# Matthew-Mosior/text-compression

Hardware: AMD Instinct MI355X
Metric: BWT+MTF+RLE encode MB/s on 1 GiB ACGTN (higher is better)
Workload: dtype u8; 1 GPU; 1 x 1073741824-byte iid ACGTN record(s) (splitmix64 counter generator), fused BWT->MTF->RLE encode, in/out resident in HBM; record_bytes=1073741824, records=1, parallelism=record-per-gpu x1

## Files before the change

### include/textcomp_debug.h

```cpp
#ifndef TEXTCOMP_DEBUG_H
#define TEXTCOMP_DEBUG_H
#include "textcomp.h"
#ifdef __cplusplus
extern "C" {
#endif
int tc_dbg_checksum64_dev(tc_ctx *ctx, const void *d_p, uint64_t bytes, uint64_t *out);
int tc_dbg_stream_bench(tc_ctx *ctx, uint64_t bytes, int width, int mode, int iters, double *gbps);
int tc_dbg_sort_bench(tc_ctx *ctx, uint64_t n, int key_bits, int iters, int check, double *ms_per_pass);
int tc_dbg_scatter_bench(tc_ctx *ctx, uint64_t n, uint32_t bins, uint32_t xrun, int iters, double *ms_per_pass);
int tc_dbg_dispatch_probe(tc_ctx *ctx, uint32_t grid, uint32_t lds_bytes, uint32_t spin_cycles, uint32_t *out6);
int tc_dbg_lcp_set_short_cap(tc_ctx *ctx, uint32_t cap);
int tc_dbg_msd_split_used(tc_ctx *ctx, uint32_t *used);
#ifdef __cplusplus
}
#endif
#endif
```

### text-compression_amd/csrc/tc_common.hpp

```cpp
#pragma once
#include <hip/hip_runtime.h>
#include <stdint.h>
#include <stdio.h>
#include <string.h>

#include <string>
#include <vector>

#include "textcomp.h"

typedef uint8_t u8;
typedef uint16_t u16;
typedef uint32_t u32;
typedef uint64_t u64;
typedef int16_t i16;
typedef int32_t i32;
typedef int64_t i64;

#define TC_WAVE 64

struct tc_ctx {
    int device = 0;
    hipStream_t stream = nullptr;
    char *ws = nullptr;
    size_t ws_cap = 0;
    size_t ws_off = 0;
    std::vector<hipMemGenericAllocationHandle_t> ws_chunks;
    size_t ws_chunk_bytes = 0, ws_mapped = 0;
    size_t ws_reserved = 0;
    u32 *d_err = nullptr;
    u64 *d_scalars = nullptr;
    u64 *h_scalars = nullptr;
    u8 *h_hdr = nullptr;
    hipEvent_t ev[8] = {};
    hipEvent_t pev[2 * 16] = {};
    int profile = 0;
    int coding = 0;
    int num_cus = 0;
    int reserved_cus = 0;
    void *hostpipe = nullptr;
    u32 stats_ws_grown = 0;
    u32 lcp_cap = 0;
    int msd_split_used = 0;
    int mtf_fastin_failed = 0;
    int live_comms = 0;
    int safe_tickets = 0;
    u32 ticket_fallbacks = 0;
    int pev_used = 0;
    std::string err;
    tc_stats stats = {};
};

struct TcFail {
    int code;
};

#define TC_HIP(ctx, expr)                                                                  \
    do {                                                                                   \
        hipError_t e__ = (expr);                                                           \
        if (e__ != hipSuccess) {                                                           \
            char b__[512];                                                                 \
            snprintf(b__, sizeof b__, "%s:%d: %s -> %s", __FILE__, __LINE__, #expr,        \
                     hipGetErrorString(e__));                                              \
            (ctx)->err = b__;                                                              \
            throw TcFail{e__ == hipErrorOutOfMemory ? TC_ERR_OOM : TC_ERR_HIP};            \
        }                                                                                  \
    } while (0)

#define TC_FAIL(ctx, code_, ...)                         \
    do {                                                 \
        char b__[512];                                   \
        snprintf(b__, sizeof b__, __VA_ARGS__);          \
        (ctx)->err = b__;                                \
        throw TcFail{code_};                             \
    } while (0)

#define TC_LAUNCH_CHECK(ctx) TC_HIP(ctx, hipGetLastError())

struct Arena {
    char *base;
    size_t off = 0;
    explicit Arena(char *b) : base(b) {}
    template <class T>
    T *get(size_t count) {
        size_t bytes = (count * sizeof(T) + 255) & ~size_t(255);
        T *p = base ? reinterpret_cast<T *>(base + off) : nullptr;
        off += bytes;
        return p;
    }
};

void tc_ws_reserve(tc_ctx *ctx, size_t bytes);
template <class F>
static inline void tc_ws_plan(tc_ctx *ctx, size_t base, F &&fn) {
    Arena dry(nullptr);
    fn(dry, true);
    tc_ws_reserve(ctx, base + dry.off);
    Arena A(ctx->ws + base);
    fn(A, false);
}
u32 tc_persistent_grid(tc_ctx *ctx, int blocks_per_cu);
template <class K>
static inline u32 tc_persistent_grid_for(tc_ctx *ctx, K kernel, int threads, int want_per_cu) {
    int occ = 0;
    if (hipOccupancyMaxActiveBlocksPerMultiprocessor(&occ, kernel, threads, 0) != hipSuccess || occ < 1) {
        (void)hipGetLastError();
        occ = 1;
    }
    return tc_persistent_grid(ctx, occ < want_per_cu ? occ : want_per_cu);
}
void *tc_chunked_alloc(tc_ctx *ctx, size_t bytes, int chunk_log2, void **handle);
void tc_chunked_free(void *handle);
void tc_sync_check(tc_ctx *ctx);

static inline u32 tc_cdiv(u64 a, u64 b) { return (u32)((a + b - 1) / b); }

#ifdef __HIPCC__

__device__ __forceinline__ u32 lane_id() { return __lane_id(); }

__device__ __forceinline__ u64 lanemask_lt() {
    return (1ull << lane_id()) - 1ull;
}

__device__ __forceinline__ u32 wave_incl_sum(u32 v) {
#pragma unroll
    for (int d = 1; d < 64; d <<= 1) {
        u32 t = __shfl_up(v, d, 64);
        if ((int)lane_id() >= d) v += t;
    }
    return v;
}
__device__ __forceinline__ u32 wave_incl_max(u32 v) {
#pragma unroll
    for (int d = 1; d < 64; d <<= 1) {
        u32 t = __shfl_up(v, d, 64);
        if ((int)lane_id() >= d) v = v > t ? v : t;
    }
    return v;
}
__device__ __forceinline__ u64 wave_incl_max64(u64 v) {
#pragma unroll
    for (int d = 1; d < 64; d <<= 1) {
        u64 t = __shfl_up(v, d, 64);
        if ((int)lane_id() >= d) v = v > t ? v : t;
    }
    return v;
}
__device__ __forceinline__ u32 wave_sum(u32 v) {
#pragma unroll
    for (int d = 32; d >= 1; d >>= 1) v += __shfl_xor(v, d, 64);
    return v;
}
__device__ __forceinline__ u64 wave_max64(u64 v) {
#pragma unroll
    for (int d = 32; d >= 1; d >>= 1) {
        u64 t = __shfl_xor(v, d, 64);
        v = v > t ? v : t;
    }
    return v;
}

template <int NT>
__device__ __forceinline__ u32 block_excl_sum(u32 v, u32 *smem, u32 *total) {
    const int w = threadIdx.x >> 6;
    u32 inc = wave_incl_sum(v);
    __syncthreads();
    if (lane_id() == 63) smem[w] = inc;
    __syncthreads();
    u32 base = 0, tot = 0;
#pragma unroll
    for (int i = 0; i < NT / 64; i++) {
        u32 s = smem[i];
        if (i < w) base += s;
        tot += s;
    }
    *total = tot;
    return base + inc - v;
}

template <int NT>
__device__ __forceinline__ u64 block_incl_max64(u64 v, u64 *smem, u64 *total) {
    const int w = threadIdx.x >> 6;
    u64 inc = wave_incl_max64(v);
    __syncthreads();
    if (lane_id() == 63) smem[w] = inc;
    __syncthreads();
    u64 base = 0, tot = 0;
#pragma unroll
    for (int i = 0; i < NT / 64; i++) {
        u64 s = smem[i];
        if (i < w) base = base > s ? base : s;
        tot = tot > s ? tot : s;
    }
    *total = tot;
    return inc > base ? inc : base;
}

#define LB_FLAG_AGG (1ull << 62)
#define LB_FLAG_INC (2ull << 62)
#define LB_VALUE(x) ((x) & ((1ull << 62) - 1))
#define LB_SPIN_LIMIT (1u << 24)

__device__ __forceinline__ void lb_store(u64 *p, u64 v) {
    __hip_atomic_store(p, v, __ATOMIC_RELAXED, __HIP_MEMORY_SCOPE_AGENT);
}
__device__ __forceinline__ u64 lb_load(const u64 *p) {
    return __hip_atomic_load(p, __ATOMIC_RELAXED, __HIP_MEMORY_SCOPE_AGENT);
}

struct OpSum {
    __device__ static u64 apply(u64 a, u64 b) { return a + b; }
    __device__ static u64 identity() { return 0; }
};
struct OpMax {
    __device__ static u64 apply(u64 a, u64 b) { return a > b ? a : b; }
    __device__ static u64 identity() { return 0; }
};
struct OpMaxPair {
    __device__ static u64 apply(u64 a, u64 b) {
        u64 ah = a >> 31, bh = b >> 31, al = a & 0x7fffffffull, bl = b & 0x7fffffffull;
        return ((ah > bh ? ah : bh) << 31) | (al > bl ? al : bl);
    }
    __device__ static u64 identity() { return 0; }
};

template <class Op>
__device__ __forceinline__ u64 lb_exclusive(u64 *status, u32 tile, u64 aggregate, u32 *err) {
    if (tile == 0) {
        if (lane_id() == 0) lb_store(&status[0], LB_FLAG_INC | aggregate);
        return Op::identity();
    }
    if (lane_id() == 0) lb_store(&status[tile], LB_FLAG_AGG | aggregate);
    u64 excl = Op::identity();
    i64 look = (i64)tile - 1;
    u32 spins = 0;
    while (true) {
        i64 idx = look - (i64)lane_id();
        u64 s = LB_FLAG_INC;
        if (idx >= 0) s = lb_load(&status[idx]);
        u64 invalid = __ballot((s >> 62) == 0);
        u64 incmask = __ballot((s >> 62) == 2);
        int first_inc = incmask ? __builtin_ctzll(incmask) : 64;
        if (invalid & (first_inc >= 63 ? ~0ull : ((2ull << first_inc) - 1ull))) {
            if (++spins > LB_SPIN_LIMIT) {
                if (lane_id() == 0) atomicOr(err, 1u);
                break;
            }
            __builtin_amdgcn_s_sleep(1);
            continue;
        }
        u64 v = ((int)lane_id() <= first_inc) ? LB_VALUE(s) : Op::identity();
#pragma unroll
        for (int d = 32; d >= 1; d >>= 1) v = Op::apply(v, __shfl_xor(v, d, 64));
        excl = Op::apply(excl, v);
        if (incmask) break;
        look -= 64;
    }
    if (lane_id() == 0) lb_store(&status[tile], LB_FLAG_INC | Op::apply(excl, aggregate));
    return excl;
}

__device__ __forceinline__ u64 lb_exclusive_last(u64 *status, u32 tile, u64 aggregate, u32 *err) {
    if (lane_id() == 0) lb_store(&status[tile], ((tile == 0 || aggregate != 0) ? LB_FLAG_INC : LB_FLAG_AGG) | aggregate);
    if (tile == 0) return 0;
    i64 look = (i64)tile - 1;
    u32 spins = 0;
    while (true) {
        const i64 idx = look - (i64)lane_id();
        u64 s = LB_FLAG_INC;
        if (idx >= 0) s = lb_load(&status[idx]);
        const u64 ends = __ballot((s >> 62) == 2 || ((s >> 62) == 1 && LB_VALUE(s) != 0));
        const u64 invalid = __ballot((s >> 62) == 0);
        const int first_end = ends ? __builtin_ctzll(ends) : 64;
        const u64 nearer = first_end >= 64 ? ~0ull : ((1ull << first_end) - 1ull);
        if (invalid & nearer) {
            if (++spins > LB_SPIN_LIMIT) {
                if (lane_id() == 0) atomicOr(err, 1u);
                return 0;
            }
            __builtin_amdgcn_s_sleep(1);
            continue;
        }
        if (ends) return LB_VALUE(__shfl(s, first_end, 64));
        look -= 64;
    }
}

__device__ __forceinline__ void lds_barrier() { asm volatile("s_waitcnt lgkmcnt(0)\n\ts_barrier" ::: "memory"); }

#endif
```

### text-compression_amd/csrc/tc_msd.hpp

```cpp
#pragma once
#include "tc_sa.hpp"

#ifndef MSD_NT
#define MSD_NT 1024
#endif
#ifndef MSD_ITEMS
#define MSD_ITEMS 8
#endif
#define MSD_TILE (MSD_NT * MSD_ITEMS)
#ifndef MSD_GROUP
#define MSD_GROUP 16
#endif
#define MSD_GLOG (MSD_GROUP == 32 ? 5 : MSD_GROUP == 16 ? 4 : 3)
#ifndef MSD_SUB
#define MSD_SUB 1
#endif
#ifndef MSD_BPC
#define MSD_BPC 1
#endif
#define MSD_LEVELS 3
#define MSDF_CAP_SMALL 2048
#ifndef MSDF_KO_NT
#define MSDF_KO_NT 256
#endif
#ifndef MSDF_BIG_NT
#define MSDF_BIG_NT 512
#endif
#ifndef MSDF_BIG_ITEMS
#define MSDF_BIG_ITEMS 12
#endif
#define MSDF_CAP_BIG (MSDF_BIG_NT * MSDF_BIG_ITEMS)

struct MsdLevel {
    const u32 *pstart;
    const u32 *pcnt;
    const u32 *tpre;
    u32 nparents;
    int shift;
    u32 *seg;
    u32 *cstart;
    u32 *ccnt;
    int aligned;
    u32 ntot;
    const u32 *cnt_in;
    u32 *flags;
    u64 *dbg;
};

#ifdef __HIPCC__

__device__ __forceinline__ u32 msd_tile_lo(u32 T, u32 b, u32 G) { return (u32)(((u64)T * b) / G); }
__device__ __forceinline__ u32 msd_block_of_tile(u32 T, u32 t, u32 G) {
    return (u32)((((u64)t + 1) * G - 1) / T);
}

__global__ void msd_root_kernel(u32 *pstart, u32 *pcnt, u32 N, u32 *maxchild) {
    pstart[0] = 0;
    pcnt[0] = N;
    *maxchild = 0;
}

__device__ __forceinline__ u32 msd_block_of_parent(const MsdLevel &L, u32 q, u32 G) {
    return (u32)(((u64)L.pstart[q] * G) / L.ntot);
}
__device__ __forceinline__ u32 msd_first_parent(const MsdLevel &L, u32 b, u32 G) {
    if (b == 0) return 0;
    if (b >= G) return L.nparents;
    u32 lo = 0, hi = L.nparents;
    while (lo < hi) {
        const u32 mid = (lo + hi) >> 1;
        if (msd_block_of_parent(L, mid, G) >= b) hi = mid; else lo = mid + 1;
    }
    return lo;
}
__device__ __forceinline__ void msd_block_range(const MsdLevel &L, u32 b, u32 G, u32 *t0, u32 *t1) {
    if (L.aligned) {
        *t0 = L.tpre[msd_first_parent(L, b, G)];
        *t1 = L.tpre[msd_first_parent(L, b + 1, G)];
    } else {
        const u32 T = L.tpre[L.nparents];
        *t0 = (u32)(((u64)T * b) / G);
        *t1 = (u32)(((u64)T * (b + 1)) / G);
    }
}

__global__ __launch_bounds__(1024) void msd_prep_kernel(const u32 *__restrict__ pcnt, u32 nparents,
                                                        u32 *__restrict__ tpre) {
    __shared__ u32 s_scan[1024 / 64 + 1];
    const u32 per = (nparents + 1023) / 1024;
    const u32 lo = threadIdx.x * per;
    u32 sum = 0;
    if (per == 64 && nparents == 65536u) {
        uint4 v[16];
        const uint4 *pv = reinterpret_cast<const uint4 *>(pcnt + lo);
#pragma unroll
        for (int i = 0; i < 16; i++) v[i] = pv[i];
        u32 t[64];
#pragma unroll
        for (int i = 0; i < 16; i++) {
            t[4 * i] = (v[i].x + MSD_TILE - 1) / MSD_TILE; t[4 * i + 1] = (v[i].y + MSD_TILE - 1) / MSD_TILE;
            t[4 * i + 2] = (v[i].z + MSD_TILE - 1) / MSD_TILE; t[4 * i + 3] = (v[i].w + MSD_TILE - 1) / MSD_TILE;
        }
#pragma unroll
        for (int i = 0; i < 64; i++) sum += t[i];
        u32 tot;
        u32 run = block_excl_sum<1024>(sum, s_scan, &tot);
        uint4 *ov = reinterpret_cast<uint4 *>(tpre + lo);
#pragma unroll
        for (int i = 0; i < 16; i++) {
            uint4 o;
            o.x = run; run += t[4 * i];
            o.y = run; run += t[4 * i + 1];
            o.z = run; run += t[4 * i + 2];
            o.w = run; run += t[4 * i + 3];
            ov[i] = o;
        }
        if (threadIdx.x == 0) tpre[nparents] = tot;
        return;
    }
    for (u32 i = 0; i < per; i++) {
        const u32 q = lo + i;
        if (q < nparents) sum += (pcnt[q] + MSD_TILE - 1) / MSD_TILE;
    }
    u32 tot;
    u32 run = block_excl_sum<1024>(sum, s_scan, &tot);
    for (u32 i = 0; i < per; i++) {
        const u32 q = lo + i;
        if (q < nparents) {
            tpre[q] = run;
            run += (pcnt[q] + MSD_TILE - 1) / MSD_TILE;
        }
    }
    if (threadIdx.x == 0) tpre[nparents] = tot;
}

__device__ __forceinline__ u32 msd_find_parent(const u32 *tpre, u32 nparents, u32 t) {
    u32 lo = 0, hi = nparents;
    while (hi - lo > 1) {
        const u32 mid = (lo + hi) >> 1;
        if (tpre[mid] <= t) lo = mid; else hi = mid;
    }
    return lo;
}

struct MsdTileInfo {
    u32 base;
    u32 valid;
    u32 q;
    u32 last;
};
struct MsdCur {
    u32 q, tq0, tq1, ps, pc;
};
__device__ __forceinline__ void msd_cur_init(const MsdLevel &L, MsdCur &c, u32 t) {
    c.q = msd_find_parent(L.tpre, L.nparents, t);
    c.tq0 = L.tpre[c.q]; c.tq1 = L.tpre[c.q + 1]; c.ps = L.pstart[c.q]; c.pc = L.pcnt[c.q];
}
__device__ __forceinline__ void msd_cur_info(const MsdLevel &L, MsdCur &c, u32 t, u32 t_end, MsdTileInfo *out) {
    if (t >= t_end) {
        out->base = 0; out->valid = 0; out->q = 0; out->last = 0;
        return;
    }
    if (t >= c.tq1) {
        u32 q = c.q + 1;
        while (L.tpre[q + 1] <= t) q++;
        c.q = q; c.tq0 = L.tpre[q]; c.tq1 = L.tpre[q + 1]; c.ps = L.pstart[q]; c.pc = L.pcnt[q];
    }
    const u32 off = (t - c.tq0) * MSD_TILE;
    out->base = c.ps + off;
    out->valid = c.pc - off < MSD_TILE ? c.pc - off : MSD_TILE;
    out->q = c.q;
    out->last = (t + 1 >= t_end || t + 1 >= c.tq1) ? 1u : 0u;
}

struct MsdTextDigit {
    const u8 *text;
    u32 n;
    u32 B, s;
    u16 lut[256];
    u32 hash_ok, hsh, tlo, thi;
};

#ifndef MSD_XCD_MAP
#define MSD_XCD_MAP 0
#endif
__device__ __forceinline__ u32 msd_logical_wg(u32 b, u32 G) {
    return (MSD_XCD_MAP && (G & 7u) == 0) ? (b & 7u) * (G >> 3) + (b >> 3) : b;
}

struct MsdJointRows {
    u8 row[256];
    u8 dig[128];
};
template <bool TEXT, bool JOINT, bool HI>
__device__ __forceinline__ void msd_count_body(const MsdLevel &L, const u64 *__restrict__ keys,
                                               const MsdTextDigit &td, u32 *__restrict__ joint_out,
                                               const MsdJointRows &jr) {
    static_assert(!HI || (!TEXT && JOINT), "the high halves serve the joint count of keys only");
    __shared__ u32 s_cnt[256];
    __shared__ u16 s_lut[TEXT ? 256 : 1];
    __shared__ u32 s_seg[4];
    __shared__ u32 s_joint[JOINT ? 32768 : 1];
    const u32 tid = threadIdx.x, G = gridDim.x, b = msd_logical_wg(blockIdx.x, G);
    if (tid < 256) s_cnt[tid] = 0;
    if (TEXT && tid < 256) s_lut[tid] = td.lut[tid];
    __shared__ u8 s_row[JOINT ? 256 : 1];
    if (JOINT) {
        for (u32 i = tid; i < 32768; i += MSD_NT) s_joint[i] = 0;
        if (tid < 256) s_row[tid] = jr.row[tid];
    }
    const u32 T = L.tpre[L.nparents];
    const u32 t0 = msd_tile_lo(T, b, G), t1 = msd_tile_lo(T, b + 1, G);
    if (t0 >= t1) return;
    u32 t = t0;
    u32 q = 0;
    if (tid == 0) q = msd_find_parent(L.tpre, L.nparents, t0);
    while (t < t1) {
        if (tid == 0) {
            while (L.tpre[q + 1] <= t) q++;
            const u32 tq0 = L.tpre[q], tq1 = L.tpre[q + 1];
            const u32 te = tq1 < t1 ? tq1 : t1;
            const u32 ps = L.pstart[q], pc = L.pcnt[q];
            const u32 lo = ps + (t - tq0) * MSD_TILE;
            const u64 hi = (u64)ps + (u64)(te - tq0) * MSD_TILE;
            s_seg[0] = q; s_seg[1] = lo; s_seg[2] = hi < (u64)ps + pc ? (u32)hi : ps + pc; s_seg[3] = te;
        }
        __syncthreads();
        const u32 sq = s_seg[0], lo = s_seg[1], hi = s_seg[2];
        t = s_seg[3];
        if (TEXT) {
            const bool words = td.s <= 5 && (u64)lo + 8 < td.n && ((((uintptr_t)td.text) + lo) & 15) == 0;
            u32 p = lo;
            if (words) {
                const u32 span = (u64)hi + 8 <= td.n ? hi - lo : td.n - 8 - lo;
                const u32 nfull = span / (16 * MSD_NT);
                const u32 *tw = reinterpret_cast<const u32 *>(td.text + lo);
                auto fetch = [&](u32 r, u32 *x) {
                    const u32 wi = (r * MSD_NT + tid) * 4;
#pragma unroll
                    for (int q = 0; q < 5; q++) x[q] = tw[wi + q];
                };
                auto tally = [&](const u32 *x) {
                    u32 cd[20];
                    if (td.hash_ok) {
#pragma unroll
                        for (int q = 0; q < 5; q++) {
                            const u32 y = __builtin_amdgcn_perm(td.thi, td.tlo, (x[q] >> td.hsh) & 0x07070707u);
#pragma unroll
                            for (int j = 0; j < 4; j++) cd[4 * q + j] = (y >> (8 * j)) & 255u;
                        }
                    } else {
#pragma unroll
                        for (int j = 0; j < 20; j++) cd[j] = s_lut[(x[j >> 2] >> (8 * (j & 3))) & 255u];
                    }
#pragma unroll
                    for (int k = 0; k < 16; k++) {
                        u32 g = 0;
#pragma unroll
                        for (int j = 0; j < 5; j++)
                            if (j < (int)td.s) g = g * td.B + cd[k + j];
                        atomicAdd(&s_cnt[g], 1u);
                    }
                };
                u32 r = 0;
                for (; r + 4 <= nfull; r += 4) {
                    u32 xa[5], xb[5], xc[5], xd[5];
                    fetch(r, xa); fetch(r + 1, xb); fetch(r + 2, xc); fetch(r + 3, xd);
                    tally(xa); tally(xb); tally(xc); tally(xd);
                }
                for (; r < nfull; r++) {
                    u32 x[5];
                    fetch(r, x);
                    tally(x);
                }
                p = lo + nfull * 16 * MSD_NT;
            }
            for (u64 i0 = (u64)p + tid; i0 < hi; i0 += MSD_NT) {
                u64 i = i0;
                u32 g = 0;
                for (u32 j = 0; j < td.s; j++, i++) g = g * td.B + (i < td.n ? (u32)s_lut[td.text[i]] : 0u);
                atomicAdd(&s_cnt[g], 1u);
            }
        } else {
            auto add_dd = [&](u32 dd) {
                if (JOINT) {
                    const u32 r = s_row[dd >> 8];
                    if (r != 0xffu) atomicAdd(&s_joint[(r << 8) | (dd & 255u)], 1u);
                    else {
                        atomicAdd(&s_cnt[dd >> 8], 1u);
                        atomicAdd(&joint_out[((size_t)sq * 256 + (dd >> 8)) * 256 + (dd & 255u)], 1u);
                    }
                } else {
                    atomicAdd(&s_cnt[dd >> 8], 1u);
                }
            };
            auto add = [&](u64 k) { add_dd((u32)(k >> (L.shift - 8)) & 0xffffu); };
            if (HI) {
                const u32 *khi = reinterpret_cast<const u32 *>(keys);
                const u32 hs = (u32)L.shift - 40u;
                auto add4 = [&](const uint4 v) {
                    add_dd((v.x >> hs) & 0xffffu); add_dd((v.y >> hs) & 0xffffu);
                    add_dd((v.z >> hs) & 0xffffu); add_dd((v.w >> hs) & 0xffffu);
                };
                const u32 a0 = (lo + 3u) & ~3u, a = a0 < hi ? a0 : hi;
                if (lo + tid < a) add_dd((khi[lo + tid] >> hs) & 0xffffu);
                const u32 nq = (hi - a) >> 2;
                const uint4 *q4 = reinterpret_cast<const uint4 *>(khi + a);
                u32 i = tid;
                for (; i + 3 * MSD_NT < nq; i += 4 * MSD_NT) {
                    const uint4 v0 = q4[i], v1 = q4[i + MSD_NT], v2 = q4[i + 2 * MSD_NT], v3 = q4[i + 3 * MSD_NT];
                    add4(v0); add4(v1); add4(v2); add4(v3);
                }
                for (; i < nq; i += MSD_NT) add4(q4[i]);
                const u32 p = a + 4 * nq + tid;
                if (p < hi) add_dd((khi[p] >> hs) & 0xffffu);
            } else {
                u32 p = lo + tid;
                for (; p + 3 * MSD_NT < hi; p += 4 * MSD_NT) {
                    const u64 k0 = keys[p], k1 = keys[p + MSD_NT], k2 = keys[p + 2 * MSD_NT], k3 = keys[p + 3 * MSD_NT];
                    add(k0); add(k1); add(k2); add(k3);
                }
                for (; p < hi; p += MSD_NT) add(keys[p]);
            }
        }
        __syncthreads();
        if (JOINT) {
            for (u32 w = tid; w < 32768; w += MSD_NT) {
                const u32 v = s_joint[w];
                if (v) {
                    atomicAdd(&joint_out[((size_t)sq * 256 + jr.dig[w >> 8]) * 256 + (w & 255u)], v);
                    atomicAdd(&s_cnt[jr.dig[w >> 8]], v);
                    s_joint[w] = 0;
                }
            }
            __syncthreads();
        }
        if (tid < 256) {
            L.seg[((size_t)sq + b) * 256 + tid] = s_cnt[tid];
            s_cnt[tid] = 0;
        }
    }
}
template <bool TEXT, bool JOINT>
__global__ __launch_bounds__(MSD_NT) void msd_count_kernel(MsdLevel L, const u64 *__restrict__ keys,
                                                           MsdTextDigit td, u32 *__restrict__ joint_out,
                                                           MsdJointRows jr) {
    msd_count_body<TEXT, JOINT, false>(L, keys, td, joint_out, jr);
}
__global__ __launch_bounds__(MSD_NT) void msd_count_hi_kernel(MsdLevel L, const u32 *__restrict__ khi,
                                                              MsdTextDigit td, u32 *__restrict__ joint_out,
                                                              MsdJointRows jr) {
    msd_count_body<false, true, true>(L, reinterpret_cast<const u64 *>(khi), td, joint_out, jr);
}

__global__ __launch_bounds__(256) void msd_scan_kernel(MsdLevel L, u32 G, u32 *maxchild) {
    __shared__ u32 s_scan[256 / 64 + 1];
    const u32 q = blockIdx.x, d = threadIdx.x;
    const u32 cnt = L.pcnt[q];
    const size_t c = (size_t)q * 256 + d;
    if (cnt == 0) {
        L.ccnt[c] = 0;
        L.cstart[c] = L.pstart[q];
        return;
    }
    if (L.aligned) {
        const u32 tot = L.cnt_in[c];
        u32 all;
        const u32 excl = block_excl_sum<256>(tot, s_scan, &all);
        const u32 start = L.pstart[q] + excl;
        L.cstart[c] = start;
        L.ccnt[c] = tot;
        L.seg[((size_t)q + msd_block_of_parent(L, q, G)) * 256 + d] = start;
        if (d == 0 && all != cnt) atomicOr(L.flags, 8u);
        if (maxchild) {
            u32 m = tot;
#pragma unroll
            for (int x = 32; x >= 1; x >>= 1) {
                const u32 o = __shfl_xor(m, x, 64);
                m = m > o ? m : o;
            }
            if ((d & 63) == 0 && m > MSDF_CAP_SMALL) atomicMax(maxchild, m);
        }
        return;
    }
    const u32 T = L.tpre[L.nparents];
    const u32 bf = msd_block_of_tile(T, L.tpre[q], G), bl = msd_block_of_tile(T, L.tpre[q + 1] - 1, G);
    u32 tot = 0;
#pragma unroll 8
    for (u32 b = bf; b <= bl; b++) {
        const u32 v = L.seg[((size_t)q + b) * 256 + d];
        tot += msd_tile_lo(T, b, G) < msd_tile_lo(T, b + 1, G) ? v : 0u;
    }
    u32 all;
    const u32 excl = block_excl_sum<256>(tot, s_scan, &all);
    u32 run = L.pstart[q] + excl;
    L.cstart[c] = run;
    L.ccnt[c] = tot;
#pragma unroll 8
    for (u32 b = bf; b <= bl; b++) {
        const size_t o = ((size_t)q + b) * 256 + d;
        const u32 v = L.seg[o];
        if (msd_tile_lo(T, b, G) >= msd_tile_lo(T, b + 1, G)) continue;
        L.seg[o] = run;
        run += v;
    }
    if (maxchild) {
        u32 m = tot;
#pragma unroll
        for (int x = 32; x >= 1; x >>= 1) {
            const u32 o = __shfl_xor(m, x, 64);
            m = m > o ? m : o;
        }
        if ((d & 63) == 0 && m > MSDF_CAP_SMALL) atomicMax(maxchild, m);
    }
}

typedef u32 msd_u32x4 __attribute__((ext_vector_type(4)));
template <bool KEYGEN, bool VALS, bool SPLIT>
__device__ __forceinline__ void msd_partition_body(const MsdLevel &L, const u64 *kin, const u32 *vin,
                                                   u64 *kout, u32 *vout, u32 *shi, u32 *slo, const u8 *text,
                                                   const RadixKeyGen &kg) {
    static_assert(!SPLIT || !VALS, "the split layout is the key-only levels'");
    __shared__ __attribute__((aligned(16))) u64 s_keys[MSD_TILE];
    __shared__ __attribute__((aligned(16))) u32 s_vals[VALS ? MSD_TILE : 4];
    __shared__ __attribute__((aligned(16))) u64 c_keys[256 * MSD_GROUP];
    __shared__ __attribute__((aligned(16))) u32 c_vals[VALS ? 256 * MSD_GROUP : 4];
    __shared__ u32 s_cnt[256 * MSD_SUB], s_dstart[256 * MSD_SUB], s_r[256], s_cur[256], s_ph[256];
    __shared__ u32 s_scan[16];
    __shared__ u64 s_lmask[4];
#ifdef MSD_PROFILE
    __shared__ u64 s_dbg[2];
    if (threadIdx.x == 0) { s_dbg[0] = 0; s_dbg[1] = 0; }
#endif
    __shared__ u16 s_live[256];
    __shared__ u16 s_klut[KEYGEN ? 256 : 1];
    constexpr bool KG_SPLIT = KEYGEN && !VALS && MSD_ITEMS == 8;
    __shared__ __attribute__((aligned(16))) u8 s_kr[KG_SPLIT ? MSD_TILE + 16 + 80 + 32 : 16];
    __shared__ __attribute__((aligned(16))) u8 s_kg8[KG_SPLIT ? MSD_TILE + 64 : 16];
    __shared__ u32 s_scan2[2];
    static_assert(MSD_GROUP == 8 || MSD_GROUP == 16 || MSD_GROUP == 32, "group = 8, 16 or 32 pairs");
    static_assert(((size_t)MSD_TILE * (VALS ? 12 : 8) + 256 * MSD_GROUP * (VALS ? 12 : 8) + 8192 + (KG_SPLIT ? 2 * MSD_TILE + 256 : 0)) * (VALS ? 1 : MSD_BPC) <= 163840, "LDS budget");
    __shared__ MsdTileInfo s_info[4];

    const u32 tid = threadIdx.x, G = gridDim.x, b = msd_logical_wg(blockIdx.x, G);
    if (KEYGEN && tid < 256) s_klut[tid] = kg.lut[tid];
    if (tid < 256) { s_r[tid] = 0; s_ph[tid] = 0; s_cur[tid] = 0; }
    for (u32 i = tid; i < 256 * MSD_SUB; i += MSD_NT) s_cnt[i] = 0;
    if (tid == 0) {
        u32 ta = 0, tb = 0;
        if (!(L.aligned && (*L.flags & 8u))) msd_block_range(L, b, G, &ta, &tb);
        s_scan2[0] = ta; s_scan2[1] = tb;
    }
    __syncthreads();
    const u32 t0 = s_scan2[0], t1 = s_scan2[1];
    if (t0 >= t1) return;
    MsdCur cs = {};
    if (tid == 0) {
        msd_cur_init(L, cs, t0);
        msd_cur_info(L, cs, t0, t1, &s_info[0]);
        msd_cur_info(L, cs, t0 + 1, t1, &s_info[1]);
        msd_cur_info(L, cs, t0 + 2, t1, &s_info[2]);
    }
    __syncthreads();

    constexpr int KG_PRE = 16, KG_SLOTS = MSD_TILE + KG_PRE + 80;
    u16 *k_c = reinterpret_cast<u16 *>(s_keys);
    u16 *k_g = k_c + KG_SLOTS;
    u8 *k_r = reinterpret_cast<u8 *>(k_g + KG_SLOTS);
    static_assert(KG_SLOTS * 5 <= MSD_TILE * 8, "key-generation image must fit under the staging keys");
    const u32 kg_units = KEYGEN ? (KG_PRE + MSD_TILE + kg.P * kg.s + kg.s + 15) / 16 : 0;

    u64 key[MSD_ITEMS];
    u32 val[MSD_ITEMS];
    msd_u32x4 raw = {0, 0, 0, 0}, nraw = {0, 0, 0, 0};
    auto kg_edge = [&](const MsdTileInfo ti) {
        return ti.base < (u32)KG_PRE || (u64)ti.base - KG_PRE + (u64)kg_units * 16 > (u64)kg.n_text ||
               ((((uintptr_t)text) + ti.base) & 15) != 0;
    };
    auto kg_load_plain = [&](const MsdTileInfo ti) {
        msd_u32x4 rw = {0, 0, 0, 0};
        if (tid < kg_units) {
            const i64 p0 = (i64)ti.base - KG_PRE + (i64)tid * 16;
            const i64 nt = (i64)kg.n_text;
            if (p0 >= 0 && p0 + 16 <= nt && ((((uintptr_t)text) + (u64)p0) & 15) == 0) {
                rw = *reinterpret_cast<const msd_u32x4 *>(text + p0);
            } else {
                u32 x[4] = {0, 0, 0, 0};
#pragma unroll 1
                for (int j = 0; j < 16; j++) {
                    const i64 pp = p0 + j;
                    const u32 c = (pp >= 0 && pp < nt) ? (u32)text[pp] : 0u;
                    x[j >> 2] |= c << (8 * (j & 3));
                }
                rw.x = x[0]; rw.y = x[1]; rw.z = x[2]; rw.w = x[3];
            }
        }
        return rw;
    };
    msd_u32x4 nk4[MSD_ITEMS / 2], nv4[MSD_ITEMS / 4];
    auto pof = [&](int k) -> u32 {
        return KEYGEN ? (u32)k * MSD_NT + tid : (u32)(k >> 2) * (4 * MSD_NT) + 4 * tid + (u32)(k & 3);
    };
    auto tile_safe = [&](const MsdTileInfo x) { return x.valid != 0 && (u64)x.base + MSD_TILE <= (u64)L.ntot; };
    auto load_plain = [&](const MsdTileInfo f) {
#pragma unroll
        for (int k = 0; k < MSD_ITEMS; k++) {
            const u32 p = pof(k);
            key[k] = 0;
            val[k] = 0;
            if (p < f.valid) {
                if (SPLIT) key[k] = (u64)shi[f.base + p] << 32 | slo[f.base + p];
                else key[k] = kin[f.base + p];
                if (VALS) val[k] = vin[f.base + p];
            }
        }
    };
    auto prefetch = [&](const MsdTileInfo cur_ti, const MsdTileInfo nx) {
        if (KEYGEN) {
            const bool use = nx.valid != 0 && !kg_edge(nx);
            const u32 base = use ? nx.base : (cur_ti.base >= (u32)KG_PRE && !kg_edge(cur_ti) ? cur_ti.base : 0u);
            const u32 unit = tid < kg_units ? tid : kg_units - 1;
            const u8 *src = use || base ? text + ((u64)base - KG_PRE + (u64)unit * 16)
                                        : reinterpret_cast<const u8 *>((((uintptr_t)text) + 15) & ~(uintptr_t)15);
            asm volatile("global_load_dwordx4 %0, %1, off" : "=v"(nraw) : "v"(src) : "memory");
        } else {
            const bool safe = tile_safe(nx);
            const u32 nb = safe ? nx.base : 0u;
            const u32 nv = safe ? nx.valid : (L.ntot < (u32)MSD_TILE ? L.ntot & ~3u : (u32)MSD_TILE);
#pragma unroll
            for (int g = 0; g < MSD_ITEMS / 4; g++) {
                u32 gs = (u32)g * (4 * MSD_NT) + 4 * tid;
                gs = gs < nv ? gs : 0u;
                const u32 *vp = vin + nb + gs;
                if (SPLIT) {
                    const u32 *hp = shi + nb + gs, *lp = slo + nb + gs;
                    asm volatile("global_load_dwordx4 %0, %1, off" : "=v"(nk4[2 * g]) : "v"(hp) : "memory");
                    asm volatile("global_load_dwordx4 %0, %1, off" : "=v"(nk4[2 * g + 1]) : "v"(lp) : "memory");
                } else {
                    const u64 *kp = kin + nb + gs;
                    asm volatile("global_load_dwordx4 %0, %1, off" : "=v"(nk4[2 * g]) : "v"(kp) : "memory");
                    asm volatile("global_load_dwordx4 %0, %1, off" : "=v"(nk4[2 * g + 1]) : "v"(kp + 2) : "memory");
                }
                if (VALS) asm volatile("global_load_dwordx4 %0, %1, off" : "=v"(nv4[g]) : "v"(vp) : "memory");
            }
        }
    };
    auto land = [&]() {
        if (KEYGEN) {
            asm volatile("s_waitcnt vmcnt(0)" : "+v"(nraw) : : "memory");
        } else {
            static_assert(MSD_ITEMS == 4 || MSD_ITEMS == 8, "land() lists the prefetch registers");
            if (!VALS) {
                if (MSD_ITEMS == 8)
                    asm volatile("s_waitcnt vmcnt(0)"
                                 : "+v"(nk4[0]), "+v"(nk4[1]), "+v"(nk4[MSD_ITEMS / 2 - 2]), "+v"(nk4[MSD_ITEMS / 2 - 1])
                                 :
                                 : "memory");
                else
                    asm volatile("s_waitcnt vmcnt(0)" : "+v"(nk4[0]), "+v"(nk4[1]) : : "memory");
            } else if (MSD_ITEMS == 8)
                asm volatile("s_waitcnt vmcnt(0)"
                             : "+v"(nk4[0]), "+v"(nk4[1]), "+v"(nk4[MSD_ITEMS / 2 - 2]), "+v"(nk4[MSD_ITEMS / 2 - 1]), "+v"(nv4[0]),
                               "+v"(nv4[MSD_ITEMS / 4 - 1])
                             :
                             : "memory");
            else
                asm volatile("s_waitcnt vmcnt(0)" : "+v"(nk4[0]), "+v"(nk4[1]), "+v"(nv4[0]) : : "memory");
        }
    };
    const u32 B = kg.B;
    (void)B;
    auto gen_group = [&](u8 *k_r, u8 *k_g8, u32 grp) {
        const u32 *rp = reinterpret_cast<const u32 *>(k_r + KG_PRE + 8 * grp);
        const u32 x0 = rp[0], x1 = rp[1], x2 = rp[2];
        u32 c[10];
        if (kg.hash_ok) {
            const u32 y0 = __builtin_amdgcn_perm(kg.thi, kg.tlo, (x0 >> kg.hsh) & 0x07070707u);
            const u32 y1 = __builtin_amdgcn_perm(kg.thi, kg.tlo, (x1 >> kg.hsh) & 0x07070707u);
            const u32 y2 = __builtin_amdgcn_perm(kg.thi, kg.tlo, (x2 >> kg.hsh) & 0x07070707u);
#pragma unroll
            for (int j = 0; j < 4; j++) {
                c[j] = (y0 >> (8 * j)) & 255u;
                c[4 + j] = (y1 >> (8 * j)) & 255u;
            }
            c[8] = y2 & 255u;
            c[9] = (y2 >> 8) & 255u;
        } else {
#pragma unroll
        for (int j = 0; j < 4; j++) {
            c[j] = (u32)s_klut[(x0 >> (8 * j)) & 255u];
            c[4 + j] = (u32)s_klut[(x1 >> (8 * j)) & 255u];
        }
        c[8] = (u32)s_klut[x2 & 255u];
        c[9] = (u32)s_klut[(x2 >> 8) & 255u];
        }
        u32 lo = 0, hi = 0;
#pragma unroll
        for (int j = 0; j < 8; j++) {
            const u32 g = kg.s == 3 ? (c[j] * B + c[j + 1]) * B + c[j + 2] : kg.s == 2 ? c[j] * B + c[j + 1] : c[j];
            if (j < 4) lo |= g << (8 * j);
            else hi |= g << (8 * (j - 4));
        }
        *reinterpret_cast<uint2 *>(k_g8 + 8 * grp) = make_uint2(lo, hi);
    };
    auto kg_fast = [&](const MsdTileInfo x) { return KEYGEN && kg.s <= 3 && MSD_ITEMS == 8 && x.valid != 0 && !kg_edge(x); };
    auto seg_init = [&](u32 qq) {
        const u32 sb = L.seg[((size_t)qq + b) * 256 + tid];
        s_cur[tid] = sb & ~(u32)(MSD_GROUP - 1);
        s_ph[tid] = sb & (MSD_GROUP - 1);
        s_r[tid] = sb & (MSD_GROUP - 1);
        const u64 m = __ballot(L.ccnt[(size_t)qq * 256 + tid] != 0);
        if ((tid & 63) == 0) s_lmask[tid >> 6] = m;
    };
    if (tid < 256) seg_init(s_info[0].q);
    auto detach = [&]() {
        if (KEYGEN) {
            asm volatile("" : "+v"(raw) : : "memory");
        } else if (!VALS) {
            asm volatile("" : "+v"(key[0]), "+v"(key[1]), "+v"(key[2]), "+v"(key[3]) : : "memory");
            if (MSD_ITEMS == 8)
                asm volatile("" : "+v"(key[MSD_ITEMS - 4]), "+v"(key[MSD_ITEMS - 3]), "+v"(key[MSD_ITEMS - 2]), "+v"(key[MSD_ITEMS - 1]) : : "memory");
        } else {
            asm volatile("" : "+v"(key[0]), "+v"(key[1]), "+v"(key[2]), "+v"(key[3]), "+v"(val[0]), "+v"(val[1]), "+v"(val[2]), "+v"(val[3]) : : "memory");
            if (MSD_ITEMS == 8)
                asm volatile("" : "+v"(key[MSD_ITEMS - 4]), "+v"(key[MSD_ITEMS - 3]), "+v"(key[MSD_ITEMS - 2]), "+v"(key[MSD_ITEMS - 1]),
                                  "+v"(val[MSD_ITEMS - 4]), "+v"(val[MSD_ITEMS - 3]), "+v"(val[MSD_ITEMS - 2]), "+v"(val[MSD_ITEMS - 1]) : : "memory");
        }
    };
    if (KEYGEN) {
        if (!kg_edge(s_info[0])) raw = kg_load_plain(s_info[0]);
    } else {
        load_plain(s_info[0]);
    }
    detach();
    if (KG_SPLIT && kg_fast(s_info[0])) {
        if (tid < kg_units) *reinterpret_cast<uint4 *>(s_kr + tid * 16) = make_uint4(raw.x, raw.y, raw.z, raw.w);
        __syncthreads();
        gen_group(s_kr, s_kg8, tid);
        if (tid < 3) gen_group(s_kr, s_kg8, MSD_NT + tid);
    }

    for (u32 t = t0; t < t1; t++) {
        const u32 slot = (t - t0) & 3u;
        const MsdTileInfo ti = s_info[slot];
#ifdef MSD_PROFILE
        u64 tq[8];
        tq[0] = __builtin_readcyclecounter();
#endif
        if (tid == 0) msd_cur_info(L, cs, t + 3, t1, &s_info[(slot + 3) & 3u]);
        __syncthreads();
#ifdef MSD_PROFILE
        const u64 t_b0 = __builtin_readcyclecounter();
#endif
        const MsdTileInfo nx = s_info[(slot + 1) & 3u];
        prefetch(ti, nx);
        if (KEYGEN && kg_edge(ti)) {
            raw = kg_load_plain(ti);
            detach();
        }
        if (!KEYGEN && t != t0 && !tile_safe(ti)) {
            load_plain(ti);
            detach();
        }
        const bool fastkg = KEYGEN && kg.s <= 3 && MSD_ITEMS == 8 && !kg_edge(ti);
        if (fastkg) {
            u8 *kr = KG_SPLIT ? s_kr : k_r;
            u8 *k_g8 = KG_SPLIT ? s_kg8 : reinterpret_cast<u8 *>(k_c);
            if (!KG_SPLIT) {
                if (tid < kg_units) *reinterpret_cast<uint4 *>(kr + tid * 16) = make_uint4(raw.x, raw.y, raw.z, raw.w);
                __syncthreads();
                gen_group(kr, k_g8, tid);
                if (tid < 3) gen_group(kr, k_g8, MSD_NT + tid);
                __syncthreads();
            }
            {
                const u32 *gp = reinterpret_cast<const u32 *>(k_g8 + 8 * tid);
                u32 D[8];
#pragma unroll
                for (int i = 0; i < 8; i++) D[i] = gp[i];
                const u32 *rq = reinterpret_cast<const u32 *>(kr + KG_PRE + 8 * tid - 4);
                const u32 r0 = rq[0], r1 = rq[1], r2 = rq[2];
                const u32 PR[2] = {__builtin_amdgcn_alignbyte(r1, r0, 3), __builtin_amdgcn_alignbyte(r2, r1, 3)};
                auto pick2 = [&](u32 X, int bx, u32 Y, int by, bool upper) -> u32 {
                    const u32 sel = upper ? ((u32)(4 + bx) << 24) | ((u32)by << 16) : ((u32)(4 + bx) << 8) | (u32)by;
                    return __builtin_amdgcn_perm(X, Y, sel);
                };
                auto build = [&](auto S) {
                    constexpr int SS = decltype(S)::value;
#pragma unroll
                    for (int k = 0; k < 8; k++) {
                        const int j0 = k, j1 = k + SS, j2 = k + 2 * SS, j3 = k + 3 * SS, j4 = k + 4 * SS, j5 = k + 5 * SS, j6 = k + 6 * SS;
                        const u32 hA = pick2(D[j0 >> 2], j0 & 3, D[j1 >> 2], j1 & 3, true);
                        const u32 hB = pick2(D[j2 >> 2], j2 & 3, D[j3 >> 2], j3 & 3, false);
                        const u32 lA = pick2(D[j4 >> 2], j4 & 3, D[j5 >> 2], j5 & 3, true);
                        const u32 lB = pick2(D[j6 >> 2], j6 & 3, PR[k >> 2], k & 3, false);
                        const u32 hi = __builtin_amdgcn_perm(hA, hB, 0x07060100u);
                        const u32 lo = __builtin_amdgcn_perm(lA, lB, 0x07060100u);
                        key[k] = ((u64)hi << 32) | (u64)lo;
                    }
                };
                if (kg.s == 3) build(std::integral_constant<int, 3>{});
                else if (kg.s == 2) build(std::integral_constant<int, 2>{});
                else build(std::integral_constant<int, 1>{});
            }
            if (!KG_SPLIT) __syncthreads();
        } else if (KEYGEN) {
            const i64 nt = (i64)kg.n_text;
            if (tid < kg_units) {
                const i64 p0 = (i64)ti.base - KG_PRE + (i64)tid * 16;
                const u32 xx[4] = {raw.x, raw.y, raw.z, raw.w};
                u32 cw[8];
                const bool inside = p0 >= 0 && p0 + 16 <= nt;
#pragma unroll
                for (int j = 0; j < 16; j += 2) {
                    const u32 ba = (xx[j >> 2] >> (8 * (j & 3))) & 255u, bb = (xx[(j + 1) >> 2] >> (8 * ((j + 1) & 3))) & 255u;
                    u32 ca = s_klut[ba], cb = s_klut[bb];
                    if (!inside) {
                        const i64 pa = p0 + j, pb = p0 + j + 1;
                        if (pa < 0 || pa >= nt) ca = 0;
                        if (pb < 0 || pb >= nt) cb = 0;
                    }
                    cw[j >> 1] = ca | (cb << 16);
                }
                uint4 *dc = reinterpret_cast<uint4 *>(k_c + tid * 16);
                dc[0] = make_uint4(cw[0], cw[1], cw[2], cw[3]);
                dc[1] = make_uint4(cw[4], cw[5], cw[6], cw[7]);
                *reinterpret_cast<uint4 *>(k_r + tid * 16) = make_uint4(raw.x, raw.y, raw.z, raw.w);
            }
            __syncthreads();
            const u32 gslots = KG_PRE + MSD_TILE + kg.P * kg.s;
            const u32 B = kg.B;
            if (kg.s == 3) {
                for (u32 x = tid; x < gslots; x += MSD_NT) k_g[x] = (u16)((k_c[x] * B + k_c[x + 1]) * B + k_c[x + 2]);
            } else {
                for (u32 x = tid; x < gslots; x += MSD_NT) {
                    u32 g = 0;
                    for (u32 j = 0; j < kg.s; j++) g = g * B + k_c[x + j];
                    k_g[x] = (u16)g;
                }
            }
            __syncthreads();
#pragma unroll
            for (int k = 0; k < MSD_ITEMS; k++) {
                const u32 p = k * MSD_NT + tid;
                if (p < ti.valid) {
                    const u32 x = KG_PRE + p;
                    u64 kk = 0;
#pragma unroll
                    for (int f = 0; f < 7; f++)
                        if (f < (int)kg.P) kk |= (u64)k_g[x + f * kg.s] << (56 - 8 * f);
                    key[k] = kk | (u64)k_r[x - 1];
                }
            }
            __syncthreads();
        }
#ifdef MSD_PROFILE
        tq[1] = __builtin_readcyclecounter();
#endif
        u32 dig[MSD_ITEMS], rnk[MSD_ITEMS];
#pragma unroll
        for (int k = 0; k < MSD_ITEMS; k++) {
            const u32 p = pof(k);
            dig[k] = (u32)(key[k] >> L.shift) & 255u;
            if (p < ti.valid) rnk[k] = atomicAdd(&s_cnt[dig[k] * MSD_SUB + (tid % MSD_SUB)], 1u);
        }
#ifdef MSD_PROFILE
        const u64 t_s1 = __builtin_readcyclecounter();
        if ((tid & 63) == 0) {
            atomicMax((unsigned long long *)&s_dbg[0], (unsigned long long)(t_s1 - t_b0));
            atomicMax((unsigned long long *)&s_dbg[1], (unsigned long long)(tq[1] - t_b0));
        }
#endif
        __syncthreads();
#ifdef MSD_PROFILE
        tq[2] = __builtin_readcyclecounter();
        if (b == 0 && L.dbg && (tid == 0 || tid == MSD_NT - 64)) L.dbg[tid == 0 ? 8 : 9] += t_s1 - tq[1];
        if (b == 0 && L.dbg && tid == 0) { L.dbg[10] += s_dbg[0]; L.dbg[11] += s_dbg[1]; s_dbg[0] = 0; s_dbg[1] = 0; }
#endif
        {
            constexpr u32 NC = 256 * MSD_SUB;
            if (tid < NC) {
                const u32 c = s_cnt[tid];
                const u32 inc = wave_incl_sum(c);
                if ((tid & 63) == 63) s_scan[tid >> 6] = inc;
                s_dstart[tid] = inc - c;
            }
            __syncthreads();
            if (tid < NC) {
                u32 base = 0;
                for (u32 i = 0; i < (tid >> 6); i++) base += s_scan[i];
                s_dstart[tid] += base;
            }
            if (tid < 256) {
                const u32 w = tid >> 6;
                const u64 mine = s_lmask[w];
                if ((mine >> (tid & 63)) & 1ull) {
                    u32 pos = (u32)__popcll(mine & ((1ull << (tid & 63)) - 1ull));
                    for (u32 i = 0; i < w; i++) pos += (u32)__popcll(s_lmask[i]);
                    s_live[pos] = (u16)tid;
                }
            }
        }
        __syncthreads();
#ifdef MSD_PROFILE
        tq[3] = __builtin_readcyclecounter();
#endif
#pragma unroll
        for (int k = 0; k < MSD_ITEMS; k++) {
            const u32 p = pof(k);
            if (p < ti.valid) {
                const u32 o = s_dstart[dig[k] * MSD_SUB + (tid % MSD_SUB)] + rnk[k];
                s_keys[o] = key[k];
                if (VALS) s_vals[o] = KEYGEN ? ti.base + (fastkg ? 8 * tid + k : p) : val[k];
            }
        }
#ifdef MSD_PROFILE
        tq[4] = __builtin_readcyclecounter();
#endif
        land();
#ifdef MSD_PROFILE
        tq[5] = __builtin_readcyclecounter();
#endif
        const bool kg_next = KG_SPLIT && kg_fast(nx);
        if (KEYGEN) {
            raw = nraw;
            if (kg_next && tid < kg_units) *reinterpret_cast<uint4 *>(s_kr + tid * 16) = make_uint4(raw.x, raw.y, raw.z, raw.w);
        } else {
#pragma unroll
            for (int k = 0; k < MSD_ITEMS; k++) {
                if (SPLIT) {
                    const msd_u32x4 h4 = nk4[2 * (k >> 2)], l4 = nk4[2 * (k >> 2) + 1];
                    const u32 h = (k & 3) == 0 ? h4.x : (k & 3) == 1 ? h4.y : (k & 3) == 2 ? h4.z : h4.w;
                    const u32 l = (k & 3) == 0 ? l4.x : (k & 3) == 1 ? l4.y : (k & 3) == 2 ? l4.z : l4.w;
                    key[k] = (u64)h << 32 | l;
                } else {
                    const msd_u32x4 q4 = nk4[k >> 1];
                    key[k] = (k & 1) ? ((u64)q4.w << 32 | q4.z) : ((u64)q4.y << 32 | q4.x);
                }
                if (VALS) {
                    const msd_u32x4 v4 = nv4[k >> 2];
                    val[k] = (k & 3) == 0 ? v4.x : (k & 3) == 1 ? v4.y : (k & 3) == 2 ? v4.z : v4.w;
                }
            }
        }
        __syncthreads();
#ifdef MSD_PROFILE
        tq[6] = __builtin_readcyclecounter();
#endif
        if (kg_next) {
            gen_group(s_kr, s_kg8, tid);
            if (tid < 3) gen_group(s_kr, s_kg8, MSD_NT + tid);
        }
        {
            constexpr u32 NG = MSD_NT / MSD_GROUP;
            const u32 lg = tid / MSD_GROUP, l = tid % MSD_GROUP;
            const u32 nlive = (u32)(__popcll(s_lmask[0]) + __popcll(s_lmask[1]) + __popcll(s_lmask[2]) + __popcll(s_lmask[3]));
            for (u32 j = lg; j < nlive; j += NG) {
                const u32 d = s_live[j];
                u32 c = 0;
#pragma unroll
                for (int x = 0; x < MSD_SUB; x++) c += s_cnt[d * MSD_SUB + x];
                if (c == 0) continue;
                const u32 r = s_r[d], ds = s_dstart[d * MSD_SUB], cur = s_cur[d], ph = s_ph[d];
                const u32 ng = (r + c) >> MSD_GLOG;
                for (u32 k = 0; k < ng; k++) {
                    const u32 e = k * MSD_GROUP + l;
                    u64 kk;
                    u32 vv = 0;
                    if (e < r) {
                        kk = c_keys[d * MSD_GROUP + e];
                        if (VALS) vv = c_vals[d * MSD_GROUP + e];
                    } else {
                        kk = s_keys[ds + e - r];
                        if (VALS) vv = s_vals[ds + e - r];
                    }
                    if (k > 0 || l >= ph) {
                        if (KEYGEN && SPLIT) {
                            shi[cur + e] = (u32)(kk >> 32);
                            slo[cur + e] = (u32)kk;
                        } else {
                            kout[cur + e] = kk;
                        }
                        if (VALS) vout[cur + e] = vv;
                    }
                }
                const u32 newr = ng ? ((r + c) & (MSD_GROUP - 1)) : r + c;
                if (ng) {
                    if (l < newr) {
                        const u32 o = ds + (ng * MSD_GROUP - r) + l;
                        c_keys[d * MSD_GROUP + l] = s_keys[o];
                        if (VALS) c_vals[d * MSD_GROUP + l] = s_vals[o];
                    }
                } else if (l >= r && l < newr) {
                    c_keys[d * MSD_GROUP + l] = s_keys[ds + l - r];
                    if (VALS) c_vals[d * MSD_GROUP + l] = s_vals[ds + l - r];
                }
                if (l == 0) {
                    s_r[d] = newr;
                    if (ng) {
                        s_cur[d] = cur + ng * MSD_GROUP;
                        s_ph[d] = 0;
                    }
#pragma unroll
                    for (int x = 0; x < MSD_SUB; x++) s_cnt[d * MSD_SUB + x] = 0;
                }
            }
        }
#ifdef MSD_PROFILE
        tq[7] = __builtin_readcyclecounter();
        if (b == 0 && tid == 0 && L.dbg) {
            L.dbg[0] += tq[1] - tq[0]; L.dbg[2] += tq[2] - tq[1]; L.dbg[3] += tq[3] - tq[2]; L.dbg[4] += tq[4] - tq[3];
            L.dbg[5] += tq[5] - tq[4]; L.dbg[6] += tq[6] - tq[5]; L.dbg[7] += tq[7] - tq[6]; L.dbg[1] += 1;
        }
#endif
        if (ti.last) {
            __syncthreads();
            for (u32 x = tid; x < 256 * MSD_GROUP; x += MSD_NT) {
                const u32 d = x / MSD_GROUP, j = x % MSD_GROUP;
                if (j >= s_ph[d] && j < s_r[d]) {
                    const u32 pos = s_cur[d] + j;
                    if (KEYGEN && SPLIT) {
                        const u64 kk = c_keys[x];
                        shi[pos] = (u32)(kk >> 32);
                        slo[pos] = (u32)kk;
                    } else {
                        kout[pos] = c_keys[x];
                    }
                    if (VALS) vout[pos] = c_vals[x];
                }
            }
            __syncthreads();
            if (t + 1 < t1 && tid < 256) seg_init(s_info[(slot + 1) & 3u].q);
        }
    }
}
template <bool KEYGEN, bool VALS = true>
__global__ __launch_bounds__(MSD_NT) void msd_partition_kernel(MsdLevel L, const u64 *kin, const u32 *vin,
                                                               u64 *kout, u32 *vout, const u8 *text,
                                                               RadixKeyGen kg) {
    msd_partition_body<KEYGEN, VALS, false>(L, kin, vin, kout, vout, nullptr, nullptr, text, kg);
}
template <bool KEYGEN>
__global__ __launch_bounds__(MSD_NT) void msd_partition_split_kernel(MsdLevel L, u32 *khi, u32 *klo, u64 *kout,
                                                                     const u8 *text, RadixKeyGen kg) {
    msd_partition_body<KEYGEN, false, true>(L, nullptr, nullptr, kout, nullptr, khi, klo, text, kg);
}
static inline size_t msd_split_npad(size_t N) { return (N + 31) & ~(size_t)31; }

struct MsdFinishLut {
    u32 a[256];
    u32 w[256];
    u32 c[256];
};
#define MSDK_BPC 1024
__global__ __launch_bounds__(256) void msd_finish_lut_kernel(const u32 *__restrict__ cnt, MsdFinishLut *out) {
    __shared__ u64 s_x[257];
    __shared__ u64 s_tot;
    const u32 t = threadIdx.x;
    s_x[t] = cnt[t];
    __syncthreads();
    if (t == 0) {
        u64 run = 0;
        for (int i = 0; i < 256; i++) { const u64 c = s_x[i]; s_x[i] = run; run += c; }
        s_x[256] = run;
        s_tot = run ? run : 1;
    }
    __syncthreads();
    const u64 tot = s_tot;
    const u32 lo = (u32)(s_x[t] * (u64)(MSDK_BPC * 64 - 1) / tot), hi = t == 255 ? (u32)(MSDK_BPC * 64 - 1) : (u32)(s_x[t + 1] * (u64)(MSDK_BPC * 64 - 1) / tot);
    out->a[t] = lo;
    out->w[t] = hi - lo;
    const u64 c16 = s_x[t] * 65536ull / tot;
    out->c[t] = c16 > 65535 ? 65535u : (u32)c16;
}


struct MsdFinishArgs {
    const u64 *keys;
    const u32 *vals;
    const u32 *pcnt;
    const u32 *cstart;
    const u32 *ccnt;
    u32 *sa_out;
    u8 *L;
    u32 *out_slot, *out_idx, *out_grp;
    u32 *rcount;
    u32 rcap;
    u32 *counters;
    u64 *kout;
    u32 *whole_list;
    u32 whole_cap;
    u32 *out_khi;
    const MsdFinishLut *lut;
};

#define MSDW_NT 512
__global__ __launch_bounds__(MSDW_NT) void msd_whole_kernel(MsdFinishArgs a) {
    __shared__ u32 s_o;
    const u32 tid = threadIdx.x;
    const u32 nlist = a.counters[2] < a.whole_cap ? a.counters[2] : a.whole_cap;
    for (u32 e = blockIdx.x; e < nlist; e += gridDim.x) {
        const u32 start = a.whole_list[2 * e], tot = a.whole_list[2 * e + 1];
        for (u32 base = 0; base < tot; base += MSDW_NT * 4) {
            const u32 cnt = tot - base < MSDW_NT * 4 ? tot - base : MSDW_NT * 4;
            const u32 reg = (e + base / (MSDW_NT * 4)) % FIN_REGIONS;
            const u32 rbase = reg * a.rcap;
            __syncthreads();
            if (tid == 0) s_o = atomicAdd(a.rcount + reg * FIN_RSTRIDE, cnt);
            __syncthreads();
            const u32 o0 = s_o;
            for (u32 i = tid; i < cnt; i += MSDW_NT) {
                const u32 p = start + base + i;
                const u64 k = a.keys[p];
                const u32 v = a.vals[p];
                a.sa_out[p] = v;
                a.L[p] = (u8)(k & 0xff);
                a.kout[p] = k;
                if (o0 + i < a.rcap) {
                    a.out_slot[rbase + o0 + i] = p;
                    a.out_idx[rbase + o0 + i] = v;
                    a.out_grp[rbase + o0 + i] = start;
                }
            }
        }
    }
}

template <int MSDF_NT, int MSDF_ITEMS, int MSDF_CH, int MSDF_XB, bool SORTEDKEYS, bool VALS = true>
__global__ __launch_bounds__(MSDF_NT) void msd_finish_kernel(MsdFinishArgs a) {
    constexpr u32 MSDF_TILE = MSDF_NT * MSDF_ITEMS;
    constexpr u32 BINS_PER_CHILD = 256u << MSDF_XB;
    constexpr u32 MAXBINS = MSDF_CH * BINS_PER_CHILD;
    constexpr int BPT = MAXBINS / MSDF_NT;
    static_assert(BPT * MSDF_NT == MAXBINS && BPT % 2 == 0, "bins must divide among the threads in pairs");
    static_assert(MSDF_TILE < 65536, "16-bit bin counters");
    __shared__ u32 s_off[MAXBINS / 2 + 2];
    __shared__ u32 s_low[MSDF_TILE];
    __shared__ u32 s_idx[VALS ? MSDF_TILE : 4];
    __shared__ __attribute__((aligned(16))) u8 s_L[MSDF_TILE + 8];
    __shared__ u32 s_cc[256], s_cs[256];
    __shared__ u32 s_chunk[5];
    __shared__ u32 s_scan[MSDF_NT / 64 + 1];
    const u32 q = blockIdx.x;
    if (a.pcnt[q] == 0 || (a.counters[1] & 8u)) return;
    const u32 tid = threadIdx.x, l = tid & 63;
    for (u32 i = tid; i < 256; i += MSDF_NT) {
        s_cc[i] = a.ccnt[(size_t)q * 256 + i];
        s_cs[i] = a.cstart[(size_t)q * 256 + i];
    }
    const u32 region = blockIdx.x % FIN_REGIONS;
    u32 *rctr = a.rcount + region * FIN_RSTRIDE;
    const u32 rbase = region * a.rcap;
    __shared__ u32 s_aw[256];
    __shared__ u16 s_cq[256];
    const bool use_lut = a.lut != nullptr;
    if (use_lut)
        for (u32 i = tid; i < 256; i += MSDF_NT) {
            s_aw[i] = a.lut->a[i] | (a.lut->w[i] << 16);
            s_cq[i] = (u16)a.lut->c[i];
        }
    auto bin_of = [&](u64 key, u32 c0) -> u32 {
        if (use_lut) {
            const u32 aw = s_aw[(u32)(key >> 32) & 255u];
            const u32 c = s_cq[(u32)(key >> 24) & 255u];
            const u32 inner = ((aw & 0xffffu) + ((u32)__umul24(aw >> 16, c) >> 16)) >> (8 - MSDF_XB);
            return (((u32)(key >> 40) & 255u) - c0) * BINS_PER_CHILD + inner;
        }
        return ((u32)(key >> (32 - MSDF_XB)) & ((0x10000u << MSDF_XB) - 1u)) - c0 * BINS_PER_CHILD;
    };
    auto off_at = [&](u32 bin) { return (s_off[bin >> 1] >> (16 * (bin & 1))) & 0xffffu; };
    u32 ch = 0;
    while (true) {
        __syncthreads();
        if (tid == 0) {
            while (ch < 256 && s_cc[ch] == 0) ch++;
            u32 c0 = ch, tot = 0, span = 0;
            if (ch < 256 && s_cc[ch] > MSDF_TILE) {
                if (SORTEDKEYS) {
                    const u32 e = atomicAdd(&a.counters[2], 1u);
                    if (e < a.whole_cap) {
                        a.whole_list[2 * e] = s_cs[ch];
                        a.whole_list[2 * e + 1] = s_cc[ch];
                    }
                    atomicOr(&a.counters[1], e < a.whole_cap ? 2u : 4u);
                } else {
                    atomicOr(&a.counters[1], 4u);
                }
                ch++;
                span = 1;
            } else {
                while (ch < 256 && span < MSDF_CH && tot + s_cc[ch] <= MSDF_TILE) {
                    tot += s_cc[ch];
                    ch++;
                    span++;
                }
            }
            s_chunk[0] = c0; s_chunk[1] = span; s_chunk[2] = c0 < 256 ? s_cs[c0] : 0; s_chunk[3] = tot; s_chunk[4] = ch;
        }
        __syncthreads();
        const u32 c0 = s_chunk[0], span = s_chunk[1], start = s_chunk[2], tot = s_chunk[3];
        ch = s_chunk[4];
        if (c0 >= 256) break;
        if (tot == 0) continue;
        const u32 nbins = span * BINS_PER_CHILD;
        const u32 lsh = (u32)((uintptr_t)(a.L + start) & 3u);
        for (u32 i = tid; i <= nbins / 2; i += MSDF_NT) s_off[i] = 0;
        __syncthreads();
        u64 key[MSDF_ITEMS];
        u32 val[MSDF_ITEMS], pos[MSDF_ITEMS];
        const u64 *kp = a.keys + start;
        const u32 *vp = a.vals + start;
#pragma unroll
        for (int k = 0; k < MSDF_ITEMS; k++) {
            const u32 i = k * MSDF_NT + tid;
            if (i < tot) {
                key[k] = kp[i];
                if (VALS) val[k] = vp[i];
            }
        }
#pragma unroll
        for (int k = 0; k < MSDF_ITEMS; k++) {
            const u32 i = k * MSDF_NT + tid;
            if (i < tot) {
                const u32 bin = bin_of(key[k], c0);
                pos[k] = atomicAdd(&s_off[bin >> 1], (bin & 1) ? 0x10000u : 1u);
            }
        }
        __syncthreads();
        {
            const u32 w0 = tid * (BPT / 2);
            u32 wv[BPT / 2], sum = 0;
#pragma unroll
            for (int j = 0; j < BPT / 2; j++) {
                wv[j] = (w0 + j) * 2 < nbins ? s_off[w0 + j] : 0u;
                sum += (wv[j] & 0xffffu) + (wv[j] >> 16);
            }
            u32 all;
            u32 ex = block_excl_sum<MSDF_NT>(sum, s_scan, &all);
#pragma unroll
            for (int j = 0; j < BPT / 2; j++) {
                const u32 lo = wv[j] & 0xffffu, hi = wv[j] >> 16;
                if ((w0 + j) * 2 < nbins) s_off[w0 + j] = ex | ((ex + lo) << 16);
                ex += lo + hi;
            }
            if (tid == 0) s_off[nbins / 2] = tot;
        }
        __syncthreads();
#pragma unroll
        for (int k = 0; k < MSDF_ITEMS; k++) {
            const u32 i = k * MSDF_NT + tid;
            if (i < tot) {
                const u32 bin = bin_of(key[k], c0);
                pos[k] = ((pos[k] >> (16 * (bin & 1))) & 0xffffu) + off_at(bin);
                s_low[pos[k]] = (u32)(key[k] >> 8);
            }
        }
        __syncthreads();
#pragma unroll
        for (int k = 0; k < MSDF_ITEMS; k++) {
            if (k * MSDF_NT < tot) {
                const u32 i = k * MSDF_NT + tid;
                const bool in = i < tot;
                u32 s = 0, e = 0, lt = 0, eq = 0;
                const u32 mine = (u32)(key[k] >> 8);
                if (in) {
                    const u32 bin = bin_of(key[k], c0);
                    s = off_at(bin);
                    e = off_at(bin + 1);
                }
                for (u32 u = s; __any(u < e); u++) {
                    if (u < e) {
                        const u32 y = s_low[u];
                        lt += y < mine;
                        eq += y == mine;
                    }
                }
                u32 rank = s + lt;
                const bool td = in && eq > 1;
                const u64 tb = __ballot(td);
                if (tb) {
                    if (td)
                        for (u32 u = s; u < pos[k]; u++) rank += s_low[u] == mine;
                    u32 base = 0;
                    if (l == 0) base = atomicAdd(rctr, (u32)__popcll(tb));
                    base = __shfl(base, 0, 64);
                    if (td) {
                        const u32 o = base + (u32)__popcll(tb & lanemask_lt());
                        if (o < a.rcap) {
                            a.out_slot[rbase + o] = start + rank;
                            a.out_idx[rbase + o] = VALS ? val[k] : mine;
                            if (!VALS) a.out_khi[rbase + o] = (u32)(key[k] >> 40);
                            a.out_grp[rbase + o] = start + s + lt;
                        }
                    }
                }
                if (in) {
                    if (VALS) s_idx[rank] = val[k];
                    s_L[rank + (VALS ? 0u : lsh)] = (u8)(key[k] & 0xff);
                    if (SORTEDKEYS) a.kout[start + rank] = key[k];
                }
            }
        }
        __syncthreads();
        if (VALS) {
            for (u32 i = tid; i < tot; i += MSDF_NT) {
                a.sa_out[start + i] = s_idx[i];
                a.L[start + i] = s_L[i];
            }
        } else {
            const u32 sh = lsh, nw = (sh + tot + 3u) >> 2;
            u8 *Lw = a.L + (start - sh);
            const u32 *sw = reinterpret_cast<const u32 *>(s_L);
            for (u32 w = tid; w < nw; w += MSDF_NT) {
                const u32 lo = 4u * w, hi = lo + 4u;
                if (lo >= sh && hi <= sh + tot) {
                    reinterpret_cast<u32 *>(Lw)[w] = sw[w];
                } else {
                    for (u32 q = lo; q < hi; q++)
                        if (q >= sh && q < sh + tot) Lw[q] = s_L[q];
                }
            }
        }
    }
}

template <int CH>
__global__ __launch_bounds__(256, 6) void msd_finish_ko_kernel(MsdFinishArgs a, const MsdFinishLut *__restrict__ lut) {
    constexpr u32 NT = 256, ITEMS = 8, TILE = NT * ITEMS, MAXBINS = CH * MSDK_BPC;
    constexpr int BPT = MAXBINS / NT;
    static_assert(CH == 3, "the chunk's live children are c0, l1, l2");
    static_assert(TILE == MSDF_CAP_SMALL && TILE <= 2048 && MAXBINS <= 4096 && BPT * NT == MAXBINS && BPT % 4 == 0,
                  "chunk of the small instance; bin | byte | slot in one word; whole 16-byte groups of bins per thread");
    __shared__ __attribute__((aligned(16))) u32 s_off[MAXBINS + 4];
    __shared__ u32 s_low[TILE + 4];
    __shared__ __attribute__((aligned(16))) u8 s_L[TILE + 8];
    __shared__ u32 s_aw[256];
    __shared__ u16 s_c[256];
    __shared__ u32 s_live[256 + 4];
    __shared__ u32 s_scan[NT / 64 + 1];
    const u32 q = blockIdx.x;
    if (a.pcnt[q] == 0 || (a.counters[1] & 8u)) return;
    const u32 tid = threadIdx.x, l = tid & 63;
    u32 nlive;
    {
        const u32 c = a.ccnt[(size_t)q * 256 + tid];
        s_aw[tid] = lut->a[tid] | (lut->w[tid] << 16);
        s_c[tid] = (u16)lut->c[tid];
        const u64 m = __ballot(c != 0);
// ... 220 lines not shown
```

### text-compression_amd/csrc/tc_sa_host.hpp

```cpp
#pragma once
#include <chrono>

#include "tc_sa_plan.hpp"

#ifndef SA_KDIR_BITS
#define SA_KDIR_BITS 26
#endif
struct SaBuffers {
    u64 *k0, *k1;
    u32 *v0, *v1;
    u32 *isa;
    u32 *v2;
    u32 *act[2][4];
    u64 *sk[2];
    u32 *sv[2];
    u32 *t_idx, *t_rank;
    u64 *t_bits;
    u32 *t_dir;
    u32 *t_bsum;
    u32 *fin_rc;
    u32 *kdir;
    u64 sparse_cap;
    u32 *hist;
    u64 *rstatus;
    u64 *gstatus;
    u32 *counts;
    u32 *msd_pstart[MSD_LEVELS + 1], *msd_pcnt[MSD_LEVELS + 1];
    u32 *msd_tpre[MSD_LEVELS], *msd_seg[MSD_LEVELS];
    u32 *msd_joint;
    u32 msd_grid;
    TiedTable tp;
    SegBuffers seg;
    u32 *chain_ref, *chain_code, *chain_summ;
};

static inline u64 msd_min_n() { return (u64)env_int("TC_SA_MSD_MIN_LOG2", 27) >= 40 ? ~0ull : 1ull << env_int("TC_SA_MSD_MIN_LOG2", 27); }
static inline bool msd_wanted(u64 N) { return env_int("TC_SA_MSD", 1) != 0 && N >= msd_min_n() && N >= 1024; }

static size_t sa_carve(Arena &A, u64 N, SaBuffers &b, bool own_v1) {
    b.k0 = A.get<u64>(N + 32);
    b.k1 = A.get<u64>(N);
    b.v0 = A.get<u32>(N);
    b.v1 = own_v1 ? A.get<u32>(N) : nullptr;
    b.isa = A.get<u32>(N + 1);
    b.v2 = A.get<u32>(N);
    b.sparse_cap = N / 8 + 1024;
    for (int s = 0; s < 2; s++) {
        for (int q = 0; q < 3; q++) b.act[s][q] = A.get<u32>(N);
        b.act[s][3] = A.get<u32>(b.sparse_cap);
        b.sk[s] = A.get<u64>(b.sparse_cap);
        b.sv[s] = A.get<u32>(b.sparse_cap);
    }
    b.t_idx = A.get<u32>(b.sparse_cap);
    b.t_rank = A.get<u32>(b.sparse_cap);
    b.t_bits = A.get<u64>(N / 64 + 2);
    b.t_dir = A.get<u32>(N / 64 + 2);
    b.t_bsum = A.get<u32>(N / 64 / BDIR_TILE + 2);
    b.fin_rc = A.get<u32>(FIN_REGIONS * FIN_RSTRIDE + 128);
    b.kdir = A.get<u32>(((size_t)1 << SA_KDIR_BITS) + 2 + ((size_t)1 << SA_KDIR_BITS) / KDF_CHUNK + 64);
    b.hist = A.get<u32>(RDX_MAX_PASSES * RDX_BINS);
    b.rstatus = A.get<u64>(radix_status_words(N));
    b.gstatus = A.get<u64>(2 * (size_t)tc_cdiv(N, GRP_TILE) + 4);
    b.counts = A.get<u32>(260);
    {
        SegBuffers &g = b.seg;
        g.cap_runs = (size_t)(N / SEG_CAP + 2);
        g.cap_tiles = (size_t)(N / SEG_PT + 2) + g.cap_runs;
        g.segbits = A.get<u64>(seg_bit_words(N));
        g.ybits = A.get<u64>(seg_bit_words(N));
        for (int q = 0; q < 2; q++) {
            g.lstart[q] = A.get<u32>(g.cap_runs);
            g.lsize[q] = A.get<u32>(g.cap_runs);
            g.ltbase[q] = A.get<u32>(g.cap_runs);
            g.lshift[q] = A.get<u32>(g.cap_runs);
        }
        g.tile_seg = A.get<u32>(g.cap_tiles);
        g.hist = A.get<u32>(g.cap_runs * 256);
        g.mm = A.get<u32>(g.cap_runs * 2);
        g.counters = A.get<u32>(64);
    }
    for (int l = 0; l <= MSD_LEVELS; l++) b.msd_pstart[l] = b.msd_pcnt[l] = nullptr;
    if (msd_wanted(N)) {
        b.msd_grid = 256 * MSD_BPC;
        size_t np = 1;
        for (int l = 0; l <= MSD_LEVELS; l++, np *= 256) {
            b.msd_pstart[l] = A.get<u32>(np);
            b.msd_pcnt[l] = A.get<u32>(np);
            if (l < MSD_LEVELS) {
                b.msd_tpre[l] = A.get<u32>(np + 1);
                b.msd_seg[l] = A.get<u32>((np + b.msd_grid) * 256);
            }
        }
        b.msd_joint = A.get<u32>((size_t)256 * 256 * 256);
        b.tp.key = A.get<u64>((size_t)1 << TP_SLOT_BITS);
        b.tp.grp = A.get<u32>((size_t)1 << TP_SLOT_BITS);
        b.tp.cnt = A.get<u32>((size_t)1 << TP_SLOT_BITS);
        b.tp.bloom = A.get<u32>(((size_t)1 << TP_BLOOM_LOG2) / 32);
    }
    b.chain_ref = A.get<u32>(N + 1);
    b.chain_code = A.get<u32>(N + 1);
    b.chain_summ = A.get<u32>(chain_summ_words());
    return A.off;
}

enum SaSlot {
    SA_SLOT_PRIMARY = 0,
    SA_SLOT_ACTIVE = 1,
    SA_SLOT_PROBE = 11,
    SA_SLOT_TIED = 12,
    SA_SLOT_DROPPED = 13,
    SA_SLOT_SAMPLE = 14,
    SA_SLOT_MAXCHILD = 15,
    SA_SLOT_SEG = 24,
    SA_SLOT_ERR = 62,
    SA_SLOT_MSD_PROF = 64,
    SA_SLOT_MSDK_PROF = 112,
};
static inline u32 sa_slot_lo(const tc_ctx *ctx, int slot) { return (u32)(ctx->h_scalars[slot] & 0xffffffffu); }
static inline u32 sa_slot_hi(const tc_ctx *ctx, int slot) { return (u32)(ctx->h_scalars[slot] >> 32); }
static inline u32 *sa_dev_slot(tc_ctx *ctx, int slot) { return reinterpret_cast<u32 *>(ctx->d_scalars + slot); }

#ifdef SEG_PROFILE
static void seg_profile_dump(tc_ctx *ctx, u32 m) {
    u64 h[16];
    TC_HIP(ctx, hipStreamSynchronize(ctx->stream));
    TC_HIP(ctx, hipMemcpyFromSymbol(h, HIP_SYMBOL(seg_prof), sizeof h));
    const double w = (double)(h[7] | 1);
    fprintf(stderr, "seg_small: %llu members, %llu windows (that sort), mid members per window %.0f | cycles per window: bits %.0f attr+masks %.0f (prefix) %.0f image %.0f tiny+compact %.0f tiny store %.0f network %.0f store %.0f\n",
            (unsigned long long)m, (unsigned long long)h[7], h[8] / w, h[0] / w, h[1] / w, 0.0, h[2] / w, h[3] / w, h[4] / w, h[5] / w, h[6] / w);
    memset(h, 0, sizeof h);
    TC_HIP(ctx, hipMemcpyToSymbol(HIP_SYMBOL(seg_prof), h, sizeof h));
}
#else
static inline void seg_profile_dump(tc_ctx *, u32) {}
#endif

static void seg_sort_pairs(tc_ctx *ctx, SegBuffers &g, u64 *kx, u32 *vx, u64 *ky, u32 *vy, u32 m, int rbits) {
    hipStream_t s = ctx->stream;
    const u32 nwords = (u32)seg_bit_words(m);
    TC_HIP(ctx, hipMemsetAsync(g.ybits, 0, (size_t)nwords * sizeof(u64), s));
    TC_HIP(ctx, hipMemsetAsync(g.counters, 0, 8 * sizeof(u32), s));
    u32 igrid = tc_cdiv((u64)nwords * 64, 256);
    if (igrid > 16384) igrid = 16384;
    seg_init_kernel<<<igrid, 256, 0, s>>>(kx, m, g.segbits, nwords, g.lstart[0], g.lsize[0], g.ltbase[0], g.lshift[0],
                                          (u32)(rbits > 8 ? rbits - 8 : 0), g.counters, (u32)g.cap_runs);
    TC_LAUNCH_CHECK(ctx);
    const int nlev = 8;
    int cur = 0;
    for (int L = 0;; L++) {
        TC_HIP(ctx, hipMemcpyAsync(&ctx->h_scalars[SA_SLOT_SEG], g.counters + 2 * cur, 2 * sizeof(u32), hipMemcpyDeviceToHost, s));
        TC_HIP(ctx, hipStreamSynchronize(s));
        const u32 S = sa_slot_lo(ctx, SA_SLOT_SEG), T = sa_slot_hi(ctx, SA_SLOT_SEG);
        if (S == 0) break;
        if (L >= nlev) TC_FAIL(ctx, TC_ERR_INTERNAL, "segmented sort: %u runs still unsorted after %d levels", S, nlev);
        if (S > g.cap_runs || T > g.cap_tiles) TC_FAIL(ctx, TC_ERR_INTERNAL, "segmented sort: %u long runs / %u tiles exceed the tables", S, T);
        const int nxt = cur ^ 1;
        TC_HIP(ctx, hipMemsetAsync(g.hist, 0, (size_t)S * 256 * sizeof(u32), s));
        seg_mm_init_kernel<<<tc_cdiv(S, 256), 256, 0, s>>>(g.mm, S);
        TC_LAUNCH_CHECK(ctx);
        TC_HIP(ctx, hipMemsetAsync(g.counters + 2 * nxt, 0, 2 * sizeof(u32), s));
        u32 wgrid = tc_cdiv(S, 4);
        if (wgrid > 8192) wgrid = 8192;
        seg_tilemap_kernel<<<wgrid, 256, 0, s>>>(g.lsize[cur], g.ltbase[cur], S, g.tile_seg, (u32)g.cap_tiles);
        TC_LAUNCH_CHECK(ctx);
        seg_count_kernel<<<T, 256, 0, s>>>(kx, ky, g.lstart[cur], g.lsize[cur], g.ltbase[cur], g.lshift[cur], g.tile_seg, g.counters + 2 * cur, g.hist, g.mm);
        TC_LAUNCH_CHECK(ctx);
        seg_scan_kernel<<<wgrid, 256, 0, s>>>(g.lstart[cur], g.lsize[cur], g.lshift[cur], g.counters + 2 * cur, g.hist, g.mm, g.segbits, 0,
                                              g.lstart[nxt], g.lsize[nxt], g.ltbase[nxt], g.lshift[nxt], g.counters + 2 * nxt, (u32)g.cap_runs);
        TC_LAUNCH_CHECK(ctx);
        seg_scatter_kernel<<<T, 256, 0, s>>>(kx, vx, ky, vy, g.lstart[cur], g.lsize[cur], g.ltbase[cur], g.lshift[cur], g.tile_seg, g.counters + 2 * cur,
                                             g.hist, g.mm, g.ybits);
        TC_LAUNCH_CHECK(ctx);
        cur = nxt;
    }
    seg_small_kernel<<<tc_cdiv(m, SEG_SPAN), SEG_NT, 0, s>>>(kx, vx, ky, vy, m, g.segbits, g.ybits);
    TC_LAUNCH_CHECK(ctx);
    seg_profile_dump(ctx, m);
}

static void sa_choose_config(const u32 *counts, u64 n, int forced_fields, SaConfig &c) {
    u32 sig = 0;
    double H = 0;
    for (int v = 0; v < 256; v++) {
        c.lut[v] = 0;
        if (counts[v]) {
            c.lut[v] = (u16)(++sig);
            double p = (double)counts[v] / (double)n;
            H -= p * log2(p);
        }
    }
    c.sigma_text = sig;
    c.B = sig + 1;
    if (c.B <= 16) {
        c.w = 8;
        c.s = 1;
        u32 pw = c.B;
        while (pw * c.B <= 256) {
            pw *= c.B;
            c.s++;
        }
    } else {
        c.s = 1;
        c.w = (u32)ceil_log2_u64(c.B);
    }
    u32 pmax = 56 / c.w;
    double need = (double)ceil_log2_u64(n + 1) + 8.0;
    double per_field = H * c.s;
    u32 P = pmax;
    if (per_field > 1e-9) {
        double pf = ceil(need / per_field);
        if (pf < (double)pmax) P = (u32)pf;
    }
    if (P < 1) P = 1;
    if (forced_fields > 0) P = (u32)forced_fields;
    if (P > pmax) P = pmax;
    c.P = P;
    c.h0 = P * c.s;
    c.entropy = H;
}

static void sa_run(tc_ctx *ctx, SaBuffers &b, const u8 *d_text, u64 n, u32 *d_sa, u8 *d_L,
                   u64 *primary, u32 *counts256_out);

struct TicketTrip {};
__global__ void err_or_kernel(u32 *err, u32 bits) { atomicOr(err, bits); }
static void ticket_check(tc_ctx *ctx) {
    if (env_int("TC_DBG_TICKET_TRIP", 0) != 0) {
        err_or_kernel<<<1, 1, 0, ctx->stream>>>(ctx->d_err, 2u);
        TC_LAUNCH_CHECK(ctx);
    }
    TC_HIP(ctx, hipMemcpyAsync(&ctx->h_scalars[SA_SLOT_ERR], ctx->d_err, sizeof(u32), hipMemcpyDeviceToHost,
                               ctx->stream));
    TC_HIP(ctx, hipStreamSynchronize(ctx->stream));
    if (sa_slot_lo(ctx, SA_SLOT_ERR) & 2u) throw TicketTrip{};
}

static void sa_build(tc_ctx *ctx, Arena &A, const u8 *d_text, u64 n, u32 *d_sa, u8 *d_L,
                     u64 *primary, u32 *counts256_out, bool dry) {
    const u64 N = n + 1;
    SaBuffers b;
    sa_carve(A, N, b, d_sa == nullptr);
    if (dry) return;
    try {
        sa_run(ctx, b, d_text, n, d_sa, d_L, primary, counts256_out);
    } catch (const TicketTrip &) {
        tc_memset_async(ctx, ctx->d_err, 0, sizeof(u32));
        ctx->safe_tickets = 1;
        ctx->ticket_fallbacks++;
        sa_run(ctx, b, d_text, n, d_sa, d_L, primary, counts256_out);
    }
    ctx->stats.ticket_fallbacks = ctx->ticket_fallbacks;
}

struct SaRun {
    tc_ctx *ctx;
    SaBuffers &b;
    const u8 *text;
    u64 n, N;
    int rbits;
    u32 *d_sa;
    u32 *sa;
    u8 *d_L;
    SaKnobs K;
    SaConfig cfg;
    int rshift;
    u64 bin_min;
    u64 *part_act1;
    bool part_act1_ok;
    u64 m = 0;
    u64 h_start = 0;
    const u64 *skeys = nullptr;
    const u64 *tkeys = nullptr;
    int tkeys_shift = 0;
    bool isa_ready = false;
    bool dense = false;
    RankLookup rl = {};
    std::chrono::steady_clock::time_point trace_t0;

    hipStream_t stream() const { return ctx->stream; }
    tc_stats &st() const { return ctx->stats; }
};

template <class X>
static inline void sa_fill(const SaConfig &c, X &x) {
    x.B = c.B; x.w = c.w; x.s = c.s; x.P = c.P;
    memcpy(x.lut, c.lut, sizeof x.lut);
}
static inline void sa_fill(const SaConfig &c, MsdTextDigit &x) {
    x.B = c.B; x.s = c.s;
    memcpy(x.lut, c.lut, sizeof x.lut);
}
static RadixKeyGen sa_keygen(const SaRun &R) {
    RadixKeyGen kg;
    sa_fill(R.cfg, kg);
    kg.n_text = (u32)R.n;
    kg.hash_ok = 0; kg.hsh = 0; kg.tlo = 0; kg.thi = 0;
    return kg;
}
static RadixBuffers sa_radix_buffers(const SaRun &R, u64 *keys, u64 *keys_alt, u32 *vals, u32 *vals_alt) {
    RadixBuffers rb;
    rb.keys = keys; rb.keys_alt = keys_alt; rb.vals = vals; rb.vals_alt = vals_alt;
    rb.hist = R.b.hist; rb.status = R.b.rstatus; rb.status_cap = radix_status_words(R.N);
    return rb;
}
static RadixBuffers sa_sparse_buffers(const SaRun &R) {
    return sa_radix_buffers(R, R.b.sk[0], R.b.sk[1], R.b.sv[0], R.b.sv[1]);
}

static void sa_trace_buffers(const SaRun &R) {
    if (R.K.trace != 2) return;
    fprintf(stderr, "textcomp: buffers text %p k0 %p k1 %p v0 %p v1 %p sa %p L %p\n", (const void *)R.text, (void *)R.b.k0,
            (void *)R.b.k1, (void *)R.b.v0, (void *)R.b.v1, (void *)R.d_sa, (void *)R.d_L);
}
static void sa_trace_step(SaRun &R, const char *what, u64 count) {
    if (!R.K.trace) return;
    (void)hipStreamSynchronize(R.stream());
    auto t1 = std::chrono::steady_clock::now();
    fprintf(stderr, "textcomp:   %-28s %10llu  %8.3f ms\n", what, (unsigned long long)count,
            std::chrono::duration<double, std::milli>(t1 - R.trace_t0).count());
    R.trace_t0 = t1;
}
static void sa_trace_tied_checksums(SaRun &R, u32 fm) {
    if (R.K.trace < 2 || fm == 0) return;
    tc_ctx *ctx = R.ctx;
    std::vector<u32> hk(fm), hh(fm), hs(fm), hg(fm);
    tc_d2h(ctx, hk.data(), R.b.act[0][1], fm * sizeof(u32));
    tc_d2h(ctx, hh.data(), R.b.act[0][3], fm * sizeof(u32));
    tc_d2h(ctx, hs.data(), R.b.act[0][0], fm * sizeof(u32));
    tc_d2h(ctx, hg.data(), R.b.act[0][2], fm * sizeof(u32));
    TC_HIP(ctx, hipStreamSynchronize(R.stream()));
    u64 a1 = 0, a2 = 0, a3 = 0, a4 = 0;
    for (u32 i = 0; i < fm; i++) { a1 += hk[i]; a2 += hh[i]; a3 += hs[i]; a4 += hg[i]; }
    fprintf(stderr, "textcomp: tied members: sum klo %llx khi %llx slot %llx grp %llx\n", (unsigned long long)a1, (unsigned long long)a2, (unsigned long long)a3, (unsigned long long)a4);
    for (u32 i = 0; i < fm && i < 6; i++) fprintf(stderr, "textcomp:   member %u: klo %08x khi %06x slot %u grp %u\n", i, hk[i], hh[i], hs[i], hg[i]);
}
static void sa_trace_group_sizes(SaRun &R, int cur, u32 mm) {
    if (!R.K.trace) return;
    tc_ctx *ctx = R.ctx;
    u64 *gh = reinterpret_cast<u64 *>(R.b.hist);
    tc_memset_async(ctx, gh, 0, 32 * sizeof(u64));
    group_size_hist_kernel<<<tc_cdiv(mm, 256), 256, 0, R.stream()>>>(R.b.act[cur][0], R.b.act[cur][2], mm, gh);
    u64 hh32[32];
    tc_d2h(ctx, hh32, gh, sizeof hh32);
    (void)hipStreamSynchronize(R.stream());
    fprintf(stderr, "textcomp:   members by group size 2^c:");
    for (int c = 0; c < 32; c++) if (hh32[c]) fprintf(stderr, " %d:%.1f%%", c, 100.0 * (double)hh32[c] / (double)mm);
    fprintf(stderr, "\n");
    R.trace_t0 = std::chrono::steady_clock::now();
}
static void sa_trace_chain_tables(SaRun &R, int cur, u32 mm, u32 hh, const ChainDims &cd, const u64 *chain_path, const u64 *chain_sign) {
    if (!R.K.trace) return;
    tc_ctx *ctx = R.ctx;
    unsigned long long *dg = reinterpret_cast<unsigned long long *>(R.b.hist);
    tc_memset_async(ctx, dg, 0, 8 * sizeof(u64));
    chain_diag_kernel<<<4096, 256, 0, R.stream()>>>(R.b.act[cur][1], R.b.act[cur][2], mm, chain_path, chain_sign, R.b.chain_code, dg);
    u64 hd[8];
    tc_d2h(ctx, hd, dg, sizeof hd);
    (void)hipStreamSynchronize(R.stream());
    fprintf(stderr, "textcomp:   chain tables (h = %u, %u x %u cells of %u rows, %s ranks): members %u, on path %llu, k = 0: %llu, largest k %llu\n",
            hh, cd.nb, cd.h, cd.bk, R.dense ? "dense" : "sparse", mm, (unsigned long long)hd[0], (unsigned long long)hd[1], (unsigned long long)hd[2]);
    R.trace_t0 = std::chrono::steady_clock::now();
}
#ifdef MSDK_PROFILE
static void msdk_profile_dump(tc_ctx *ctx) {
    u64 h[10];
    tc_d2h(ctx, h, ctx->d_scalars + SA_SLOT_MSDK_PROF, sizeof h);
    TC_HIP(ctx, hipStreamSynchronize(ctx->stream));
    const double c = (double)(h[8] | 1);
    fprintf(stderr, "finish (key-only): chunks %llu, keys per chunk %.0f | cycles per chunk: land %.0f B %.0f zero+B %.0f bins+B %.0f scan+B %.0f scatter+B %.0f walk+prefetch+rank+B %.0f copy-out %.0f\n",
            (unsigned long long)h[8], h[9] / c, h[0] / c, h[1] / c, h[2] / c, h[3] / c, h[4] / c, h[5] / c, h[6] / c, h[7] / c);
    tc_memset_async(ctx, ctx->d_scalars + SA_SLOT_MSDK_PROF, 0, sizeof h);
}
#else
static inline void msdk_profile_dump(tc_ctx *) {}
#endif
#ifdef MSD_PROFILE
static void msd_profile_dump(tc_ctx *ctx) {
    u64 h[48];
    tc_d2h(ctx, h, ctx->d_scalars + SA_SLOT_MSD_PROF, sizeof h);
    TC_HIP(ctx, hipStreamSynchronize(ctx->stream));
    for (int l = 0; l < MSD_LEVELS; l++)
        fprintf(stderr, "msd level %d: tiles %llu | cursor+B0 %llu keygen/S1+B1 %llu S2 %llu S3 %llu land %llu B3 %llu S4 %llu (cycles per tile)\n", l + 1,
                (unsigned long long)h[16 * l + 1], (unsigned long long)(h[16 * l] / (h[16 * l + 1] | 1)), (unsigned long long)(h[16 * l + 2] / (h[16 * l + 1] | 1)),
                (unsigned long long)(h[16 * l + 3] / (h[16 * l + 1] | 1)), (unsigned long long)(h[16 * l + 4] / (h[16 * l + 1] | 1)), (unsigned long long)(h[16 * l + 5] / (h[16 * l + 1] | 1)),
                (unsigned long long)(h[16 * l + 6] / (h[16 * l + 1] | 1)), (unsigned long long)(h[16 * l + 7] / (h[16 * l + 1] | 1)));
    for (int l = 0; l < MSD_LEVELS; l++)
        fprintf(stderr, "   level %d, S1 alone per tile: wave 0 %llu, last wave %llu cycles; slowest wave B0 -> before B1 %llu, B0 -> prefetch issued %llu\n", l + 1,
                (unsigned long long)(h[16 * l + 8] / (h[16 * l + 1] | 1)), (unsigned long long)(h[16 * l + 9] / (h[16 * l + 1] | 1)),
                (unsigned long long)(h[16 * l + 10] / (h[16 * l + 1] | 1)), (unsigned long long)(h[16 * l + 11] / (h[16 * l + 1] | 1)));
    tc_memset_async(ctx, ctx->d_scalars + SA_SLOT_MSD_PROF, 0, sizeof h);
}
#else
static inline void msd_profile_dump(tc_ctx *) {}
#endif

static void sa_run_group(SaRun &R, bool init, GroupArgs ga) {
    tc_ctx *ctx = R.ctx;
    hipStream_t s = R.stream();
    const u32 gtiles = tc_cdiv(R.N, GRP_TILE);
    u32 tiles = tc_cdiv(ga.count, GRP_TILE);
    tc_memset_async(ctx, R.b.gstatus, 0, (2 * (size_t)gtiles + 4) * sizeof(u64));
    ga.text = R.text; ga.sa = R.sa; ga.L = R.d_L;
    ga.status_max = R.b.gstatus; ga.status_sum = R.b.gstatus + gtiles;
    ga.ticket = reinterpret_cast<u32 *>(R.b.gstatus + 2 * (size_t)gtiles);
    ga.scalars = ctx->d_scalars; ga.err = ctx->d_err;
    u32 grid = init ? tc_persistent_grid_for(ctx, group_kernel<true>, GRP_NT, 2)
                    : tc_persistent_grid_for(ctx, group_kernel<false>, GRP_NT, 2);
    if (grid > tiles) grid = tiles;
    if (init) group_kernel<true><<<grid, GRP_NT, 0, s>>>(ga);
    else group_kernel<false><<<grid, GRP_NT, 0, s>>>(ga);
    TC_LAUNCH_CHECK(ctx);
}
static u64 sa_fetch_m(SaRun &R) {
    tc_d2h(R.ctx, R.ctx->h_scalars, R.ctx->d_scalars, 2 * sizeof(u64));
    TC_HIP(R.ctx, hipStreamSynchronize(R.stream()));
    return R.ctx->h_scalars[SA_SLOT_ACTIVE];
}
static void sa_apply_pairs(SaRun &R, const u64 *pairs, u32 count, u64 *part) {
    tc_ctx *ctx = R.ctx;
    hipStream_t s = R.stream();
    u32 *cursor = R.b.hist;
    rank_cursor_kernel<<<1, 256, 0, s>>>(cursor, R.rshift);
    TC_LAUNCH_CHECK(ctx);
    rank_bin_kernel<<<tc_cdiv(count, RBIN_TILE), RBIN_NT, 0, s>>>(pairs, count, R.rshift, cursor, part, R.N);
    TC_LAUNCH_CHECK(ctx);
    rank_scatter_kernel<<<tc_cdiv(R.N, RSCAT_NT * RSCAT_ITEMS), RSCAT_NT, 0, s>>>(part, R.N, R.rshift, cursor, R.b.isa);
    TC_LAUNCH_CHECK(ctx);
}

static RadixBuffers sa_build_keys_and_sort(SaRun &R, const RadixPlan &plan, bool sa_in_alt_at_end) {
    tc_ctx *ctx = R.ctx;
    SaBuffers &b = R.b;
    const SaConfig &cfg = R.cfg;
    hipStream_t s = R.stream();
    const u32 n = (u32)R.n;
    KeyBuildParams kp;
    sa_fill(cfg, kp);
    kp.plan.npass = plan.npass;
    for (int p = 0; p < plan.npass; p++) {
        kp.plan.shift[p] = plan.shift[p];
        kp.plan.mask[p] = plan.mask[p];
    }
    tc_memset_async(ctx, b.hist, 0, sizeof(u32) * RDX_MAX_PASSES * RDX_BINS);
    bool onehist = cfg.w == 8 && plan.npass < RDX_MAX_PASSES && R.K.kb_onehist != 0;
    for (int p = 0; p < plan.npass; p++)
        if (plan.mask[p] != 255u || plan.shift[p] % 8 != 0) onehist = false;
    const u32 kgrid = tc_cdiv(R.N, SA_TILE);
    const bool fuse = onehist && RDX_TILE == SA_TILE && R.K.keygen_fused != 0;
    R.st().keygen_fused = fuse ? 1u : 0u;
    const RadixKeyGen kg = sa_keygen(R);
    if (fuse) {
        u32 ggrid = tc_cdiv(R.N, 256 * 16 * 4);
        if (ggrid > 2048) ggrid = 2048;
        if (cfg.s == 3) ghist_kernel<3><<<ggrid, 256, 0, s>>>(R.text, n, kp, b.hist);
        else ghist_kernel<0><<<ggrid, 256, 0, s>>>(R.text, n, kp, b.hist);
        TC_LAUNCH_CHECK(ctx);
        keyhist_fix_kernel<<<1, 256, 0, s>>>(R.text, n, kp, b.hist);
    } else if (onehist) {
        if (cfg.s == 3 && cfg.P == 6) keybuild_kernel<true, 3, 6><<<kgrid, SA_NT, 0, s>>>(R.text, n, kp, b.k0, b.hist);
        else if (cfg.s == 3 && cfg.P == 5) keybuild_kernel<true, 3, 5><<<kgrid, SA_NT, 0, s>>>(R.text, n, kp, b.k0, b.hist);
        else keybuild_kernel<true, 0, 0><<<kgrid, SA_NT, 0, s>>>(R.text, n, kp, b.k0, b.hist);
        TC_LAUNCH_CHECK(ctx);
        keyhist_fix_kernel<<<1, 256, 0, s>>>(R.text, n, kp, b.hist);
    } else {
        keybuild_kernel<false, 0, 0><<<kgrid, SA_NT, 0, s>>>(R.text, n, kp, b.k0, b.hist);
    }
    TC_LAUNCH_CHECK(ctx);
    const bool even = plan.npass % 2 == 0;
    const bool start_in_sa = sa_in_alt_at_end ? !even : even;
    RadixBuffers rb = start_in_sa ? sa_radix_buffers(R, b.k0, b.k1, R.sa, b.v0) : sa_radix_buffers(R, b.k0, b.k1, b.v0, R.sa);
    ctx->pev_used = 0;
    const bool xcd_group = !ctx->safe_tickets && R.K.xcd_group != 0;
    radix_sort_pairs(ctx, rb, (u32)R.N, plan, true, true, true,
                     R.text, fuse ? &kg : nullptr, xcd_group);
    if (xcd_group) ticket_check(ctx);
    return rb;
}

static bool sa_alphabet(SaRun &R, u32 *counts256_out, u64 *primary) {
    tc_ctx *ctx = R.ctx;
    hipStream_t s = R.stream();
    tc_memset_async(ctx, R.b.counts, 0, 256 * sizeof(u32));
    {
        u32 grid = tc_cdiv(R.n, 256 * 64);
        if (grid > 2048) grid = 2048;
        if (grid < 1) grid = 1;
        hist256_kernel<<<grid, 256, 0, s>>>(R.text, R.n, R.b.counts);
        TC_LAUNCH_CHECK(ctx);
    }
    u32 counts[256];
    tc_d2h(ctx, counts, R.b.counts, sizeof counts);
    TC_HIP(ctx, hipStreamSynchronize(s));
    if (counts256_out) memcpy(counts256_out, counts, sizeof counts);
    sa_choose_config(counts, R.n, R.K.fields, R.cfg);
    if (R.cfg.sigma_text != 1 || R.n == 0) return false;
    unary_sa_kernel<<<tc_cdiv(R.N, 256), 256, 0, s>>>(R.text, (u32)R.n, R.sa, R.d_L);
    TC_LAUNCH_CHECK(ctx);
    *primary = R.n;
    tc_stats &st = R.st();
    st.sigma = 2; st.rounds = 0; st.radix_launches = 0; st.ms_radix = 0;
    return true;
}


static void sa_sample(SaRun &R, int topbits) {
    tc_ctx *ctx = R.ctx;
    sample_dup_kernel<<<1, 1024, 0, R.stream()>>>(R.text, (u32)R.n, sa_keygen(R), topbits, sa_dev_slot(ctx, SA_SLOT_SAMPLE));
    TC_LAUNCH_CHECK(ctx);
    tc_d2h(ctx, &ctx->h_scalars[SA_SLOT_SAMPLE], ctx->d_scalars + SA_SLOT_SAMPLE, sizeof(u64));
    TC_HIP(ctx, hipStreamSynchronize(R.stream()));
    R.st().sample_dups = sa_slot_lo(ctx, SA_SLOT_SAMPLE);
}

struct Round0Out {
    bool msd, msd_big, keyonly;
    int tb;
    FinishArgs fa;
    const u64 *keys;
    const u64 *keys_sorted;
    int npass;
};
static void sa_round0_begin(SaRun &R, int tb, Round0Out &o) {
    tc_ctx *ctx = R.ctx;
    SaBuffers &b = R.b;
    const int keybits = (int)(R.cfg.P * R.cfg.w);
    FinishArgs &fa = o.fa;
    o.tb = tb;
    o.keys_sorted = nullptr;
    fa.N = (u32)R.N; fa.tshift = 64 - tb;
    fa.lshift = 64 - keybits; fa.lbits = keybits - tb;
    fa.sa_out = R.sa; fa.L = R.d_L;
    fa.out_slot = b.act[1][0]; fa.out_idx = b.act[1][1]; fa.out_grp = b.act[1][2];
    fa.act_cap = (u32)R.N; fa.counters = sa_dev_slot(ctx, SA_SLOT_TIED);
    fa.rcount = b.fin_rc; fa.rcap = (u32)(R.N / FIN_REGIONS);
    fa.fix_cap = (u32)(b.sparse_cap - 1024);
    fa.ovbits = b.act[1][0];
    tc_memset_async(ctx, ctx->d_scalars + SA_SLOT_TIED, 0, 2 * sizeof(u64));
    tc_memset_async(ctx, b.fin_rc, 0, (FIN_REGIONS * FIN_RSTRIDE + 128) * sizeof(u32));
}

static Round0Out sa_round0_lsd(SaRun &R, const Round0Plan &pl) {
    Round0Out o;
    o.msd = o.msd_big = o.keyonly = false;
    sa_round0_begin(R, pl.topbits, o);
    R.st().msd_path = 0;
    RadixPlan plan;
    plan.add_range(64 - pl.topbits, 64);
    RadixBuffers rb = sa_build_keys_and_sort(R, plan, true);
    o.npass = plan.npass;
    o.keys = rb.keys;
    o.fa.keys = rb.keys; o.fa.sa_in = rb.vals;
    const u32 waves = tc_cdiv(R.N, 64 * FIN_WPW);
    finish_kernel<<<tc_cdiv(waves, FIN_NT / 64), FIN_NT, 0, R.stream()>>>(o.fa);
    TC_LAUNCH_CHECK(R.ctx);
    return o;
}

static Round0Out sa_round0_msd(SaRun &R, const Round0Plan &pl, bool keyonly) {
    tc_ctx *ctx = R.ctx;
    SaBuffers &b = R.b;
    const SaConfig &cfg = R.cfg;
    hipStream_t s = R.stream();
    tc_stats &st = R.st();
    const u32 n = (u32)R.n, N = (u32)R.N;
    Round0Out o;
    o.msd = true; o.msd_big = pl.msd_big; o.keyonly = keyonly;
    sa_round0_begin(R, 8 * MSD_LEVELS, o);
    u32 *counters = o.fa.counters;
    RadixKeyGen kg = sa_keygen(R);
    radix_keygen_hash(kg);
    if (R.K.keygen_hash == 0) kg.hash_ok = 0;
    MsdTextDigit td;
    sa_fill(cfg, td);
    td.text = R.text; td.n = n;
    td.hash_ok = kg.hash_ok; td.hsh = kg.hsh; td.tlo = kg.tlo; td.thi = kg.thi;
    u32 G = b.msd_grid < (u32)ctx->num_cus * MSD_BPC ? b.msd_grid : (u32)ctx->num_cus * MSD_BPC;
    if (ctx->reserved_cus > 0 && G > (u32)(ctx->num_cus - ctx->reserved_cus) * MSD_BPC)
        G = (u32)(ctx->num_cus - ctx->reserved_cus) * MSD_BPC;
    if (R.K.msd_grid > 0 && (u32)R.K.msd_grid < G) G = (u32)R.K.msd_grid;
    u32 *maxchild = sa_dev_slot(ctx, SA_SLOT_MAXCHILD);
    msd_root_kernel<<<1, 1, 0, s>>>(b.msd_pstart[0], b.msd_pcnt[0], N, maxchild);
    TC_LAUNCH_CHECK(ctx);
    u64 *kbuf[2] = {b.k0, b.k1};
    u32 *vbuf[2] = {keyonly ? nullptr : b.v0, keyonly ? nullptr : R.sa};
    st.msd_keyonly = keyonly ? 1u : 0u;
    ctx->pev_used = 0;
    st.keygen_fused = 1;
    MsdJointRows jr;
    u32 nrows = 0;
    {
        memset(jr.row, 0xff, sizeof jr.row);
        memset(jr.dig, 0, sizeof jr.dig);
        u32 nd = 1;
        for (u32 j = 0; j < cfg.s; j++) nd *= cfg.B;
        for (u32 d = 0; d < nd && d < 256; d++) {
            bool real = true;
            for (u32 v = d, j = 0; j < cfg.s; j++, v /= cfg.B) real = real && (v % cfg.B) != 0;
            if (real) {
                if (nrows < 128) { jr.row[d] = (u8)nrows; jr.dig[nrows] = (u8)d; }
                nrows++;
            }
        }
    }
    const bool joint = R.K.msd_joint != 0 && nrows <= 128;
    const bool split = keyonly && joint && R.K.msd_split != 0 && MSD_LEVELS == 3;
    u32 *khi = reinterpret_cast<u32 *>(b.k0), *klo = khi + msd_split_npad(N);
    ctx->msd_split_used = split ? 1 : 0;
    if (joint) tc_memset_async(ctx, b.msd_joint, 0, (size_t)256 * 256 * 256 * sizeof(u32));
    u32 np = 1;
    for (int l = 0; l < MSD_LEVELS; l++, np *= 256) {
        MsdLevel ML;
        ML.pstart = b.msd_pstart[l]; ML.pcnt = b.msd_pcnt[l]; ML.tpre = b.msd_tpre[l];
        ML.nparents = np; ML.shift = 56 - 8 * l; ML.seg = b.msd_seg[l];
        ML.cstart = b.msd_pstart[l + 1]; ML.ccnt = b.msd_pcnt[l + 1];
        ML.aligned = (joint && l == MSD_LEVELS - 1) ? 1 : 0;
        ML.ntot = N; ML.cnt_in = b.msd_joint; ML.flags = counters + 1;
        ML.dbg = ctx->d_scalars + SA_SLOT_MSD_PROF + 16 * l;
        const u64 *kin = l ? kbuf[(l - 1) & 1] : nullptr;
        const u32 *vin = l ? vbuf[(l - 1) & 1] : nullptr;
        msd_prep_kernel<<<1, 1024, 0, s>>>(ML.pcnt, np, b.msd_tpre[l]);
        TC_LAUNCH_CHECK(ctx);
        if (l == 0) msd_count_kernel<true, false><<<G, MSD_NT, 0, s>>>(ML, nullptr, td, nullptr, jr);
        else if (ML.aligned) {  }
        else if (joint && l == MSD_LEVELS - 2 && split) msd_count_hi_kernel<<<G, MSD_NT, 0, s>>>(ML, khi, td, b.msd_joint, jr);
        else if (joint && l == MSD_LEVELS - 2) msd_count_kernel<false, true><<<G, MSD_NT, 0, s>>>(ML, kin, td, b.msd_joint, jr);
        else msd_count_kernel<false, false><<<G, MSD_NT, 0, s>>>(ML, kin, td, nullptr, jr);
        TC_LAUNCH_CHECK(ctx);
        msd_scan_kernel<<<np, 256, 0, s>>>(ML, G, l == MSD_LEVELS - 1 ? maxchild : nullptr);
        TC_LAUNCH_CHECK(ctx);
        const bool ev = ctx->profile && ctx->pev_used < 16;
        if (ev) TC_HIP(ctx, hipEventRecord(ctx->pev[2 * ctx->pev_used], s));
        if (split && l <= 1) {
            if (l == 0) msd_partition_split_kernel<true><<<G, MSD_NT, 0, s>>>(ML, khi, klo, nullptr, R.text, kg);
            else msd_partition_split_kernel<false><<<G, MSD_NT, 0, s>>>(ML, khi, klo, kbuf[1], R.text, kg);
        } else if (keyonly) {
            if (l == 0) msd_partition_kernel<true, false><<<G, MSD_NT, 0, s>>>(ML, nullptr, nullptr, kbuf[0], nullptr, R.text, kg);
            else msd_partition_kernel<false, false><<<G, MSD_NT, 0, s>>>(ML, kin, nullptr, kbuf[l & 1], nullptr, R.text, kg);
        } else if (l == 0) msd_partition_kernel<true><<<G, MSD_NT, 0, s>>>(ML, nullptr, nullptr, kbuf[0], vbuf[0], R.text, kg);
        else msd_partition_kernel<false><<<G, MSD_NT, 0, s>>>(ML, kin, vin, kbuf[l & 1], vbuf[l & 1], R.text, kg);
        TC_LAUNCH_CHECK(ctx);
        if (ev) {
            TC_HIP(ctx, hipEventRecord(ctx->pev[2 * ctx->pev_used + 1], s));
            ctx->pev_used++;
        }
    }
    o.keys = kbuf[(MSD_LEVELS - 1) & 1];
    MsdFinishArgs mf;
    mf.keys = o.keys; mf.vals = vbuf[(MSD_LEVELS - 1) & 1];
    mf.pcnt = b.msd_pcnt[MSD_LEVELS - 1];
    mf.cstart = b.msd_pstart[MSD_LEVELS]; mf.ccnt = b.msd_pcnt[MSD_LEVELS];
    mf.sa_out = R.sa; mf.L = R.d_L;
    mf.out_slot = o.fa.out_slot; mf.out_idx = o.fa.out_idx; mf.out_grp = o.fa.out_grp;
    mf.rcount = o.fa.rcount; mf.rcap = o.fa.rcap; mf.counters = counters;
    mf.kout = kbuf[MSD_LEVELS & 1];
    o.keys_sorted = mf.kout;
    mf.whole_list = b.msd_seg[MSD_LEVELS - 1];
    mf.whole_cap = 1u << 20;
    mf.out_khi = b.v0;
    MsdFinishLut *flut = reinterpret_cast<MsdFinishLut *>(b.msd_seg[MSD_LEVELS - 1] + 2 * (size_t)mf.whole_cap);
    msd_finish_lut_kernel<<<1, 256, 0, s>>>(b.msd_pcnt[1], flut);
    TC_LAUNCH_CHECK(ctx);
    mf.lut = R.K.msd_finish_lut != 0 ? flut : nullptr;
    if (pl.msd_big && keyonly) {
        msd_finish_kernel<MSDF_BIG_NT, MSDF_BIG_ITEMS, 1, 5, true, false><<<np / 256, MSDF_BIG_NT, 0, s>>>(mf);
    } else if (pl.msd_big) {
        msd_finish_kernel<MSDF_BIG_NT, MSDF_BIG_ITEMS, 1, 5, true><<<np / 256, MSDF_BIG_NT, 0, s>>>(mf);
        TC_LAUNCH_CHECK(ctx);
        msd_whole_kernel<<<1024, MSDW_NT, 0, s>>>(mf);
    } else if (keyonly && R.K.msd_finish_ko != 0) {
        msd_finish_ko_kernel<3><<<np / 256, 256, 0, s>>>(mf, flut);
        msdk_profile_dump(ctx);
    } else if (keyonly) {
        msd_finish_kernel<MSDF_KO_NT, MSDF_CAP_SMALL / MSDF_KO_NT, 4, 1, false, false><<<np / 256, MSDF_KO_NT, 0, s>>>(mf);
    } else {
        msd_finish_kernel<256, 8, 4, 1, false><<<np / 256, 256, 0, s>>>(mf);
    }
    TC_LAUNCH_CHECK(ctx);
    o.npass = MSD_LEVELS;
    st.msd_path = 1;
    msd_profile_dump(ctx);
    return o;
}

static bool sa_keyonly_recover(SaRun &R, u32 fm, u32 flags) {
    tc_ctx *ctx = R.ctx;
    SaBuffers &b = R.b;
    const SaConfig &cfg = R.cfg;
    hipStream_t s = R.stream();
    const u32 n = (u32)R.n;
    bool ok = fm <= TP_MAX_TIED && (u64)fm + 1024 <= b.sparse_cap && !(flags & 2u);
    if (ok) sa_trace_tied_checksums(R, fm);
    if (ok && fm > 0) {
        tc_memset_async(ctx, b.tp.key, 0, sizeof(u64) << TP_SLOT_BITS);
        tc_memset_async(ctx, b.tp.cnt, 0, sizeof(u32) << TP_SLOT_BITS);
        tc_memset_async(ctx, b.tp.bloom, 0, ((size_t)1 << TP_BLOOM_LOG2) / 8);
        u32 *d_total = sa_dev_slot(ctx, SA_SLOT_PROBE);
        tc_memset_async(ctx, d_total, 0, sizeof(u64));
        tied_table_kernel<<<tc_cdiv(fm, 256), 256, 0, s>>>(b.act[0][1], b.act[0][3], b.act[0][2], fm, cfg.B, cfg.s, cfg.P, b.tp);
        TC_LAUNCH_CHECK(ctx);
        const RadixKeyGen kgp = sa_keygen(R);
        u32 pgrid = (u32)ctx->num_cus * 3;
        if (pgrid > tc_cdiv(n, TPK_TILE)) pgrid = tc_cdiv(n, TPK_TILE);
        switch (cfg.s) {
#define TC_PROBE(S) case S: tied_probe_kernel<S><<<pgrid, TPK_NT, 0, s>>>(R.text, n, kgp, b.tp, b.act[0][0], b.act[0][1], b.act[0][2], d_total, fm); break;
            TC_PROBE(1) TC_PROBE(2) TC_PROBE(3) TC_PROBE(4) TC_PROBE(5) TC_PROBE(6) TC_PROBE(7) TC_PROBE(8)
#undef TC_PROBE
            default: TC_FAIL(ctx, TC_ERR_INTERNAL, "key-only levels: %u symbols per field", cfg.s);
        }
        TC_LAUNCH_CHECK(ctx);
        tc_d2h(ctx, &ctx->h_scalars[SA_SLOT_PROBE], ctx->d_scalars + SA_SLOT_PROBE, sizeof(u64));
        TC_HIP(ctx, hipStreamSynchronize(s));
        ok = sa_slot_lo(ctx, SA_SLOT_PROBE) == fm;
    }
    if (R.K.trace)
        fprintf(stderr, "textcomp: key-only levels: %u tied suffixes %s (the pass over the text met %u)\n", fm,
                ok ? "found again in the text" : "-- NOT recoverable: the levels run again with suffix starts", sa_slot_lo(ctx, SA_SLOT_PROBE));
    return ok;
}

static void sa_tier2_fix(SaRun &R, const FinishArgs &fa, u32 &fm, u32 &flags, u32 &fm_dropped) {
    tc_ctx *ctx = R.ctx;
    hipStream_t s = R.stream();
    const u32 fm_lean = fm;
    u32 *flagword = sa_dev_slot(ctx, SA_SLOT_TIED) + 1;
    u32 *ndropped = sa_dev_slot(ctx, SA_SLOT_DROPPED);
    tc_memset_async(ctx, flagword, 0, sizeof(u32));
    tc_memset_async(ctx, ndropped, 0, sizeof(u64));
    tc_memset_async(ctx, fa.ovbits, 0, ((size_t)tc_cdiv(R.N, 64) + 1) * sizeof(u64));
    const u32 fwaves = tc_cdiv(R.N, 64 * FIX_WIN);
    finish_fix_kernel<<<tc_cdiv(fwaves, FIN_NT / 64), FIN_NT, 0, s>>>(fa);
    TC_LAUNCH_CHECK(ctx);
    if (fm_lean) {
        finish_filter_kernel<<<tc_cdiv(fm_lean, 256) < 4096u ? tc_cdiv(fm_lean, 256) : 4096u, 256, 0, s>>>(fa.out_slot, fm_lean, fa.ovbits, ndropped);
        TC_LAUNCH_CHECK(ctx);
    }
    tc_d2h(ctx, &ctx->h_scalars[SA_SLOT_TIED], ctx->d_scalars + SA_SLOT_TIED, 2 * sizeof(u64));
    TC_HIP(ctx, hipStreamSynchronize(s));
    fm = sa_slot_lo(ctx, SA_SLOT_TIED);
    flags = sa_slot_hi(ctx, SA_SLOT_TIED);
    fm_dropped = sa_slot_lo(ctx, SA_SLOT_DROPPED);
}

static void sa_order_tied(SaRun &R, u32 fm, u32 slot_bits) {
    tc_ctx *ctx = R.ctx;
    SaBuffers &b = R.b;
    hipStream_t s = R.stream();
    if (fm <= SEG_W && R.K.tiny != 0) {
        tied_small_kernel<0><<<1, SEG_NT, 0, s>>>(b.act[0][0], b.act[0][1], b.act[0][2], fm, nullptr, nullptr, nullptr);
        TC_LAUNCH_CHECK(ctx);
        return;
    }
    pack_active_kernel<<<tc_cdiv(fm, 256), 256, 0, s>>>(b.act[0][0], b.act[0][2], fm, b.sk[0]);
    TC_LAUNCH_CHECK(ctx);
    TC_HIP(ctx, hipMemcpyAsync(b.sv[0], b.act[0][1], fm * sizeof(u32), hipMemcpyDeviceToDevice, s));
    RadixPlan ps;
    ps.add_range(32, 32 + (int)slot_bits);
    RadixBuffers rs = sa_sparse_buffers(R);
    radix_sort_pairs(ctx, rs, fm, ps, false, false);
    unpack_active_kernel<<<tc_cdiv(fm, 256), 256, 0, s>>>(rs.keys, fm, b.act[0][0], b.act[0][2]);
    TC_LAUNCH_CHECK(ctx);
    TC_HIP(ctx, hipMemcpyAsync(b.act[0][1], rs.vals, fm * sizeof(u32), hipMemcpyDeviceToDevice, s));
}

static void sa_key_round(SaRun &R, u64 *kall) {
    tc_ctx *ctx = R.ctx;
    SaBuffers &b = R.b;
    hipStream_t s = R.stream();
    tc_stats &st = R.st();
    const u32 mm = (u32)R.m;
    key_round_kernel<<<tc_cdiv(mm, 256), 256, 0, s>>>(b.act[0][0], b.act[0][2], kall, mm, b.sk[0], b.sv[0]);
    TC_LAUNCH_CHECK(ctx);
    seg_sort_pairs(ctx, b.seg, b.sk[0], b.sv[0], b.sk[1], b.sv[1], mm, 32);
    key_round_store_kernel<<<tc_cdiv(mm, 256), 256, 0, s>>>(b.sk[0], b.act[0][0], mm, kall);
    TC_LAUNCH_CHECK(ctx);
    GroupArgs gk = {};
    gk.keys = b.sk[0]; gk.count = mm; gk.vals = b.sv[0]; gk.vals_are_idx = 0; gk.norank = 1;
    gk.in_slot = b.act[0][0]; gk.in_idx = b.act[0][1];
    gk.out_slot = b.act[1][0]; gk.out_idx = b.act[1][1]; gk.out_grp = b.act[1][2];
    sa_run_group(R, false, gk);
    const u64 m2 = sa_fetch_m(R);
    for (int q = 0; q < 3; q++)
        if (m2) TC_HIP(ctx, hipMemcpyAsync(b.act[0][q], b.act[1][q], m2 * sizeof(u32), hipMemcpyDeviceToDevice, s));
    st.m[st.rounds] = R.m; st.key_bytes[st.rounds] = 8; st.passes[st.rounds] = 1; st.h[st.rounds] = (u32)R.h_start;
    st.rounds++;
    st.seg_rounds++;
    if (R.K.trace)
        fprintf(stderr, "textcomp: key round: %u members of whole buckets ordered by the key's remaining 32 bits, %llu stay tied\n", mm, (unsigned long long)m2);
    R.m = m2;
    R.h_start = R.cfg.h0;
}

enum Round0Result {
    R0_ACCEPTED,
    R0_GIVE_WAY,
    R0_NEED_STARTS,
};
static Round0Result sa_round0_collect(SaRun &R, Round0Out &o, bool keyround, bool &many_ties) {
    tc_ctx *ctx = R.ctx;
    SaBuffers &b = R.b;
    hipStream_t s = R.stream();
    tc_stats &st = R.st();
    FinishArgs &fa = o.fa;
    u32 *roff = b.fin_rc + FIN_REGIONS * FIN_RSTRIDE;
    finish_regions_kernel<<<1, 64, 0, s>>>(fa.rcount, fa.rcap, roff, fa.counters);
    TC_LAUNCH_CHECK(ctx);
    if (o.msd && o.keyonly)
        finish_compact_kernel<<<1024, 256, 0, s>>>(roff, fa.rcap, b.act[1][0], b.act[1][1], b.act[1][2],
                                                  b.act[0][0], b.act[0][1], b.act[0][2], b.v0, b.act[0][3], (u32)b.sparse_cap);
    else
        finish_compact_kernel<<<1024, 256, 0, s>>>(roff, fa.rcap, b.act[1][0], b.act[1][1], b.act[1][2],
                                                  b.act[0][0], b.act[0][1], b.act[0][2]);
    TC_LAUNCH_CHECK(ctx);
    fa.out_slot = b.act[0][0]; fa.out_idx = b.act[0][1]; fa.out_grp = b.act[0][2];
    tc_d2h(ctx, &ctx->h_scalars[SA_SLOT_TIED], ctx->d_scalars + SA_SLOT_TIED, sizeof(u64));
    TC_HIP(ctx, hipStreamSynchronize(s));
    u32 fm = sa_slot_lo(ctx, SA_SLOT_TIED), over = sa_slot_hi(ctx, SA_SLOT_TIED);
    if (R.K.trace)
        fprintf(stderr, "textcomp: round 0 %s way%s: tied %u, flags 0x%x (1 over-long bucket left to the fix pass, 2 whole buckets tied, 4 bucket above the finish chunk, 8 joint counts off)\n",
                o.msd ? "MSD" : "LSD", o.msd && o.msd_big ? " (big finish)" : "", fm, over);
    if (o.msd && (over & (4u | 8u))) return R0_GIVE_WAY;
    if (o.msd && o.keyonly && !sa_keyonly_recover(R, fm, over)) return R0_NEED_STARTS;
    u32 slot_bits = (u32)R.rbits, fm_dropped = 0;
    if (!o.msd && (over & 1u) && fm <= fa.fix_cap && R.K.tier2 != 0) {
        sa_tier2_fix(R, fa, fm, over, fm_dropped);
        slot_bits = (u32)R.rbits + 1;
    }
    if (o.msd && !o.msd_big && fm > (1u << 18)) return R0_GIVE_WAY;
    if ((over & 1u) || fm > b.sparse_cap - 1024) {
        if (!o.msd && fm > b.sparse_cap - 1024) many_ties = true;
        return R0_GIVE_WAY;
    }
    R.m = fm - fm_dropped;
    if (over & 2u) R.h_start = (u64)(o.tb / (int)R.cfg.w) * R.cfg.s;
    if (o.msd && o.msd_big) {
        R.skeys = o.keys_sorted;
    } else {
        R.tkeys = o.keys;
        R.tkeys_shift = 64 - o.tb;
    }
    st.finish_pass = 1;
    st.rounds = 1;
    st.m[0] = R.N; st.key_bytes[0] = 8; st.passes[0] = (u32)o.npass; st.h[0] = 0;
    if (R.m > 0) sa_order_tied(R, fm, slot_bits);
    if (o.msd && o.msd_big && (over & 2u) && keyround && R.m >= (u64)R.K.seg_min && R.K.seg != 0)
        sa_key_round(R, const_cast<u64 *>(o.keys_sorted));
    return R0_ACCEPTED;
}

static bool sa_round0(SaRun &R, bool &hopeless, bool &many_ties) {
    SaConfig &cfg = R.cfg;
    Round0In in;
    in.entropy = cfg.entropy; in.w = cfg.w; in.s = cfg.s; in.P = cfg.P;
    in.N = R.N;
    in.msd_carved = R.b.msd_pstart[0] != nullptr && msd_wanted(R.N);
    in.want_sa = R.d_sa != nullptr;
    in.sample_dups = 0;
    in.msd_levels = MSD_LEVELS; in.cap_small = MSDF_CAP_SMALL; in.cap_big = MSDF_CAP_BIG;
    in.samp_n = SAMP_N; in.tied_max = TP_MAX_TIED;
    Round0Plan pl;
    sa_round0_depth(in, R.K, pl);
    const bool finish_fits = (int)(cfg.P * cfg.w) - pl.topbits <= 32;
    if (finish_fits && R.n >= (1u << 20) && R.K.sample != 0) {
        sa_sample(R, pl.topbits);
        hopeless = R.st().sample_dups > SAMP_N / 10;
    }
    if (!finish_fits || hopeless) return false;
    in.sample_dups = R.st().sample_dups;
    sa_round0_plan(in, R.K, pl);
    if (pl.P != cfg.P) {
        cfg.P = pl.P;
        cfg.h0 = cfg.P * cfg.s;
        R.h_start = cfg.h0;
    }
    Round0Result res = R0_GIVE_WAY;
    if (pl.try_msd) {
        Round0Out o = sa_round0_msd(R, pl, pl.keyonly);
        res = sa_round0_collect(R, o, pl.keyround, many_ties);
        if (res == R0_NEED_STARTS) {
            o = sa_round0_msd(R, pl, false);
            res = sa_round0_collect(R, o, pl.keyround, many_ties);
        }
    }
    if (res == R0_GIVE_WAY) {
        R.ctx->msd_split_used = 0;
        Round0Out o = sa_round0_lsd(R, pl);
        res = sa_round0_collect(R, o, pl.keyround, many_ties);
    }
    return res == R0_ACCEPTED;
}

static void sa_full_path(SaRun &R, u32 P_full, bool hopeless, bool many_ties) {
    SaBuffers &b = R.b;
    SaConfig &cfg = R.cfg;
    tc_stats &st = R.st();
    cfg.P = P_full;
    if ((hopeless || st.finish_pass == 0) && R.K.fields == 0 && R.K.deep != 0 && R.K.finish != 0)
        cfg.P = 56 / cfg.w;
    cfg.h0 = cfg.P * cfg.s;
    R.h_start = cfg.h0;
    RadixPlan plan;
    plan.add_range(64 - (int)(cfg.P * cfg.w), 64);
    RadixBuffers rb = sa_build_keys_and_sort(R, plan, false);
    R.skeys = rb.keys;
    GroupArgs g0 = {};
    g0.keys = R.skeys; g0.count = (u32)R.N; g0.vals = R.sa;
    g0.out_slot = b.act[0][0]; g0.out_idx = b.act[0][1]; g0.out_grp = b.act[0][2]; g0.out_tpos = b.act[0][3];
    const bool ties = hopeless || many_ties;
    if (ties) { g0.isa = b.isa; R.isa_ready = true; }
    const bool g0_pairs = ties && R.N >= R.bin_min && R.part_act1_ok;
    if (g0_pairs) g0.pairs = rb.keys_alt;
    sa_run_group(R, true, g0);
    if (g0_pairs) sa_apply_pairs(R, rb.keys_alt, (u32)R.N, R.part_act1);
    R.m = sa_fetch_m(R);
    st.rounds = 1;
    st.m[0] = R.N; st.key_bytes[0] = 8; st.passes[0] = (u32)plan.npass; st.h[0] = 0;
}

static void sa_rank_accel(SaRun &R) {
    tc_ctx *ctx = R.ctx;
    SaBuffers &b = R.b;
    hipStream_t s = R.stream();
    RankLookup &rl = R.rl;
    const u64 N = R.N;
    const u32 nwords = (u32)(N / 64 + 1);
    const u32 nb = tc_cdiv(nwords, BDIR_TILE);
    bitdir_sum_kernel<<<nb, 256, 0, s>>>(b.t_bits, nwords, b.t_bsum);
    TC_LAUNCH_CHECK(ctx);
    bitdir_spine_kernel<<<1, 1024, 0, s>>>(b.t_bsum, nb);
    TC_LAUNCH_CHECK(ctx);
    bitdir_down_kernel<<<nb, 256, 0, s>>>(b.t_bits, nwords, b.t_bsum, b.t_dir);
    TC_LAUNCH_CHECK(ctx);
    rl.t_bits = b.t_bits; rl.t_dir = b.t_dir;
    const u64 *dkeys = R.tkeys ? R.tkeys : ((R.skeys == b.k0 || R.skeys == b.k1) ? R.skeys : nullptr);
    if (!dkeys) return;
    int kb = R.tkeys ? (64 - R.tkeys_shift < SA_KDIR_BITS ? 64 - R.tkeys_shift : SA_KDIR_BITS) : SA_KDIR_BITS;
    while (kb > 16 && (1ull << kb) > N / 16) kb--;
    if (R.K.kdir_search != 0) {
        kdir_build_kernel<<<tc_cdiv((1ull << kb) + 1, 256), 256, 0, s>>>(dkeys, (u32)N, kb, b.kdir);
        TC_LAUNCH_CHECK(ctx);
    } else {
        const u64 entries = (1ull << kb) + 1;
        const u32 nbk = tc_cdiv(entries, KDF_CHUNK);
        u32 *bmin = b.kdir + ((size_t)1 << SA_KDIR_BITS) + 2;
        tc_memset_async(ctx, b.kdir, 0xff, entries * sizeof(u32));
        kdir_mark_kernel<<<tc_cdiv(N, 256), 256, 0, s>>>(dkeys, (u32)N, kb, b.kdir);
        TC_LAUNCH_CHECK(ctx);
        kdir_fill_min_kernel<<<nbk, 256, 0, s>>>(b.kdir, entries, bmin);
        TC_LAUNCH_CHECK(ctx);
        kdir_fill_spine_kernel<<<1, 1024, 0, s>>>(bmin, nbk);
        TC_LAUNCH_CHECK(ctx);
        kdir_fill_apply_kernel<<<nbk, 256, 0, s>>>(b.kdir, entries, bmin);
        TC_LAUNCH_CHECK(ctx);
    }
    rl.kdir = b.kdir; rl.kdir_bits = kb;
}

static void sa_rank_tables(SaRun &R) {
    tc_ctx *ctx = R.ctx;
    SaBuffers &b = R.b;
    hipStream_t s = R.stream();
    RankLookup &rl = R.rl;
    const u64 m = R.m, N = R.N;
    R.dense = m > b.sparse_cap - 1024 || R.K.dense != 0;
    sa_fill(R.cfg, rl);
    rl.text = R.text; rl.n = (u32)R.n; rl.N = (u32)N; rl.h0 = R.cfg.h0;
    if (R.dense && !R.skeys) TC_FAIL(ctx, TC_ERR_INTERNAL, "dense mode needs the sorted keys");
    if (R.dense) {
        if (!R.isa_ready) {
            GroupArgs gi = {};
            gi.keys = R.skeys; gi.count = (u32)N; gi.vals = R.sa;
            gi.isa = b.isa; gi.isa_only = 1;
            u64 *kfree = R.skeys == b.k0 ? b.k1 : b.k0;
            const bool gi_pairs = N >= R.bin_min && R.part_act1_ok && (R.skeys == b.k0 || R.skeys == b.k1);
            if (gi_pairs) gi.pairs = kfree;
            sa_run_group(R, true, gi);
            if (gi_pairs) sa_apply_pairs(R, kfree, (u32)N, R.part_act1);
        }
        rl.isa = b.isa;
        return;
    }
    rl.skeys = R.skeys; rl.tkeys = R.tkeys; rl.tshift = R.tkeys_shift; rl.sa = R.sa; rl.t_idx = b.t_idx; rl.t_rank = b.t_rank; rl.t_n = (u32)m;
    if (m == 0) return;
    const u32 mm = (u32)m;
    if (m <= SEG_W && R.K.tiny != 0) {
        tied_small_kernel<1><<<1, SEG_NT, 0, s>>>(b.act[0][0], b.act[0][1], b.act[0][2], mm, b.t_idx, b.t_rank, b.act[0][3]);
        TC_LAUNCH_CHECK(ctx);
        return;
    }
    widen_u32_kernel<<<tc_cdiv(mm, 256), 256, 0, s>>>(b.act[0][1], b.sk[0], mm);
    TC_LAUNCH_CHECK(ctx);
    RadixPlan pt;
    pt.add_range(0, R.rbits);
    RadixBuffers rt = sa_sparse_buffers(R);
    radix_sort_pairs(ctx, rt, mm, pt, true, false);
    const bool accel = m >= (u64)R.K.accel_min;
    if (accel) tc_memset_async(ctx, b.t_bits, 0, (size_t)(u32)(N / 64 + 1) * sizeof(u64));
    table_build_kernel<<<tc_cdiv(mm, 256), 256, 0, s>>>(rt.keys, rt.vals, b.act[0][2], mm,
                                                       b.t_idx, b.t_rank, b.act[0][3],
                                                       accel ? b.t_bits : nullptr);
    TC_LAUNCH_CHECK(ctx);
    if (accel) sa_rank_accel(R);
}

static void sa_chain_codes(SaRun &R, int cur, u32 mm, u32 hh, u64 *chain_path, u64 *chain_sign, u32 chain_words) {
    tc_ctx *ctx = R.ctx;
    SaBuffers &b = R.b;
    hipStream_t s = R.stream();
    const u64 N = R.N;
    const ChainDims cd = chain_dims(N, hh);
    u64 *pathbits = b.seg.segbits, *signbits = b.seg.ybits;
    u32 *any = b.chain_summ + chain_any_offset();
    tc_memset_async(ctx, b.chain_ref, 0xff, (size_t)N * sizeof(u32));
    chain_ref_kernel<<<tc_cdiv(mm, 256), 256, 0, s>>>(b.act[cur][0], b.act[cur][1], b.act[cur][2], R.rl, mm, hh, b.chain_ref);
    TC_LAUNCH_CHECK(ctx);
    if (R.dense) {
        u32 fgrid = tc_cdiv(chain_words, 4);
        if (fgrid > 16384) fgrid = 16384;
        chain_flags_kernel<<<fgrid, 256, 0, s>>>(b.isa, b.chain_ref, (u32)N, hh, pathbits, signbits, chain_words);
    } else {
        tc_memset_async(ctx, pathbits, 0, (size_t)chain_words * sizeof(u64));
        tc_memset_async(ctx, signbits, 0, (size_t)chain_words * sizeof(u64));
        u32 fgrid = tc_cdiv(mm, 256);
        if (fgrid > 16384) fgrid = 16384;
        chain_flags_members_kernel<<<fgrid, 256, 0, s>>>(b.act[cur][1], b.act[cur][2], R.rl, mm, hh, b.chain_ref, pathbits, signbits);
    }
    TC_LAUNCH_CHECK(ctx);
    TC_HIP(ctx, hipMemcpyAsync(chain_path, pathbits, (size_t)chain_words * sizeof(u64), hipMemcpyDeviceToDevice, s));
    TC_HIP(ctx, hipMemcpyAsync(chain_sign, signbits, (size_t)chain_words * sizeof(u64), hipMemcpyDeviceToDevice, s));
    {
        tc_memset_async(ctx, any, 0, (size_t)cd.nb * sizeof(u32));
        u64 parts = ((u64)cd.bk * cd.h / 64) / 4096 + 1;
        if (parts > 1024) parts = 1024;
        chain_blockany_kernel<<<dim3(cd.nb, (u32)parts), 256, 0, s>>>(chain_path, cd, any);
        TC_LAUNCH_CHECK(ctx);
    }
    const u32 cgrid = (u32)tc_cdiv((u64)cd.nb * cd.h, 256);
    if (cd.nb > 1) {
        chain_scan_a_kernel<<<cgrid, 256, 0, s>>>(chain_path, chain_sign, cd, any, b.chain_summ);
        TC_LAUNCH_CHECK(ctx);
        chain_scan_b_kernel<<<tc_cdiv(cd.h, 256), 256, 0, s>>>(b.chain_summ, cd);
        TC_LAUNCH_CHECK(ctx);
    }
    chain_scan_c_kernel<<<cgrid, 256, 0, s>>>(chain_path, chain_sign, cd, any, b.chain_summ, b.chain_code);
    TC_LAUNCH_CHECK(ctx);
    R.st().chain_rounds++;
    sa_trace_step(R, "chain round: codes", N);
    sa_trace_chain_tables(R, cur, mm, hh, cd, chain_path, chain_sign);
}

static void sa_doubling_round(SaRun &R, ChainPolicy &chain, int &cur, u64 &h) {
    tc_ctx *ctx = R.ctx;
    SaBuffers &b = R.b;
    hipStream_t s = R.stream();
    tc_stats &st = R.st();
    const RankLookup &rl = R.rl;
    const bool dense = R.dense;
    const u64 N = R.N, m = R.m;
    const int rbits = R.rbits;
    const u32 mm = (u32)m;
    const u32 hh = h > N ? (u32)N : (u32)h;
    sa_trace_group_sizes(R, cur, mm);
    u64 *k2 = dense ? b.k0 : b.sk[0], *k2alt = dense ? b.k1 : b.sk[1];
    u32 *kv = dense ? b.v0 : b.sv[0], *kvalt = dense ? b.v2 : b.sv[1];
    RadixPlan p2;
    p2.add_range(0, rbits);
    p2.add_range(32, 32 + rbits);
    RadixPlanDev pd2;
    pd2.npass = p2.npass;
    for (int p = 0; p < p2.npass; p++) { pd2.shift[p] = p2.shift[p]; pd2.mask[p] = p2.mask[p]; }
    const bool seg_round = R.K.seg != 0 && mm >= (u32)R.K.seg_min;
    const bool fuse_hist = mm >= (1u << 20) && !seg_round && chain.keymode == 0;
    const bool vals_idx = dense;
    if (fuse_hist) tc_memset_async(ctx, b.hist, 0, sizeof(u32) * RDX_MAX_PASSES * RDX_BINS);
    const u32 chain_words = (u32)(N / 64 + 1);
    u64 *chain_path = reinterpret_cast<u64 *>(b.chain_ref), *chain_sign = chain_path + chain_words;
    if (chain.start(seg_round, hh, h, N, m)) sa_chain_codes(R, cur, mm, hh, chain_path, chain_sign, chain_words);
    const int keymode = chain.keymode;
    if (keymode == 1) {
        chain_key1_kernel<<<tc_cdiv(mm, 256), 256, 0, s>>>(b.act[cur][1], b.act[cur][2], chain_path, chain_sign, b.chain_code, mm, k2, vals_idx ? kv : nullptr);
    } else if (keymode == 2) {
        u32 kgrid = tc_cdiv(mm, 256);
        if (kgrid > 65536) kgrid = 65536;
        chain_key2_kernel<<<kgrid, 256, 0, s>>>(b.act[cur][1], b.act[cur][2], chain_path, chain_sign, b.chain_code, rl, mm, hh, k2, vals_idx ? kv : nullptr);
    } else {
        u32 kgrid = fuse_hist ? tc_cdiv(mm, 256 * 8) : tc_cdiv(mm, 256);
        if (fuse_hist && kgrid > 8192) kgrid = 8192;
        if (!fuse_hist && !vals_idx && !rl.isa && !rl.skeys && rl.tkeys && mm <= 65536u) kgrid = tc_cdiv(mm, 4);
        if (fuse_hist) key2_kernel<true><<<kgrid, 256, 0, s>>>(b.act[cur][1], b.act[cur][2], rl, mm, hh, k2, vals_idx ? kv : nullptr, pd2, b.hist);
        else key2_kernel<false><<<kgrid, 256, 0, s>>>(b.act[cur][1], b.act[cur][2], rl, mm, hh, k2, vals_idx ? kv : nullptr, pd2, b.hist);
    }
    TC_LAUNCH_CHECK(ctx);
    sa_trace_step(R, "round: keys (rank lookups)", mm);
    RadixBuffers r2 = sa_radix_buffers(R, k2, k2alt, kv, kvalt);
    if (seg_round) {
        if (!vals_idx) {
            seg_iota_kernel<<<tc_cdiv(mm, 256), 256, 0, s>>>(kv, mm);
            TC_LAUNCH_CHECK(ctx);
        }
        seg_sort_pairs(ctx, b.seg, k2, kv, k2alt, kvalt, mm, keymode == 1 ? 32 : rbits);
        st.seg_rounds++;
    } else {
        radix_sort_pairs(ctx, r2, mm, p2, !vals_idx, fuse_hist);
    }
    sa_trace_step(R, seg_round ? "round: segmented sort" : "round: radix passes", mm);
    GroupArgs gr = {};
    gr.keys = r2.keys; gr.count = mm; gr.vals = r2.vals; gr.vals_are_idx = vals_idx ? 1 : 0;
    gr.in_slot = b.act[cur][0]; gr.in_idx = b.act[cur][1]; gr.in_tpos = b.act[cur][3];
    gr.isa = dense ? b.isa : nullptr; gr.t_rank = dense ? nullptr : b.t_rank;
    gr.out_slot = b.act[cur ^ 1][0]; gr.out_idx = b.act[cur ^ 1][1];
    gr.out_grp = b.act[cur ^ 1][2]; gr.out_tpos = b.act[cur ^ 1][3];
    const bool gr_pairs = dense && mm >= R.bin_min;
    if (gr_pairs) gr.pairs = r2.keys_alt;
    sa_run_group(R, false, gr);
    if (gr_pairs) sa_apply_pairs(R, r2.keys_alt, mm, r2.keys);
    if (keymode != 2) {
        st.m[st.rounds] = m; st.key_bytes[st.rounds] = 8; st.passes[st.rounds] = seg_round ? 1u : (u32)p2.npass;
        st.h[st.rounds] = hh;
        st.rounds++;
    } else {
        st.passes[st.rounds - 1]++;
    }
    R.m = sa_fetch_m(R);
    sa_trace_step(R, "round: groups", mm);
    cur ^= 1;
    if (chain.finish(mm, R.m)) h *= 2;
}

static void sa_run(tc_ctx *ctx, SaBuffers &b, const u8 *d_text, u64 n, u32 *d_sa, u8 *d_L,
                   u64 *primary, u32 *counts256_out) {
    const u64 N = n + 1;
    hipStream_t s = ctx->stream;
    tc_stats &st = ctx->stats;
    SaRun R{ctx, b, d_text, n, N, ceil_log2_u64(N), d_sa, d_sa ? d_sa : b.v1, d_L, SaKnobs{}};
    R.rshift = R.rbits > 8 ? R.rbits - 8 : 0;
    R.bin_min = 1ull << R.K.bin_min_log2;
    R.part_act1 = reinterpret_cast<u64 *>(b.act[1][0]);
    R.part_act1_ok = (size_t)((char *)b.act[1][2] - (char *)b.act[1][0]) >= N * sizeof(u64) &&
                     ((uintptr_t)b.act[1][0] & 7) == 0;
    sa_trace_buffers(R);
    ctx->msd_split_used = 0;
    if (sa_alphabet(R, counts256_out, primary)) return;

    const u32 P_full = R.cfg.P;
    R.h_start = R.cfg.h0;
    bool hopeless = false;
    bool many_ties = false;
    tc_memset_async(ctx, ctx->d_scalars, 0, 16 * sizeof(u64));
    const bool fast = R.K.finish != 0 && R.K.dense == 0 && sa_round0(R, hopeless, many_ties);
    if (!fast) sa_full_path(R, P_full, hopeless, many_ties);

    R.trace_t0 = std::chrono::steady_clock::now();
    sa_trace_step(R, "(sync before the rank table)", R.m);
    sa_rank_tables(R);
    sa_trace_step(R, R.dense ? "ranks: dense ISA" : "ranks: sparse table", R.m);

    if (R.K.h_start > 0) R.h_start = (u64)R.K.h_start;
    ChainPolicy chain(R.K.chain);
    int cur = 0;
    u64 h = R.h_start;
    while (R.m > 0) {
        if (st.rounds >= TC_MAX_ROUNDS) TC_FAIL(ctx, TC_ERR_INTERNAL, "suffix sort did not converge");
        sa_doubling_round(R, chain, cur, h);
    }
    primary_kernel<<<1, 64, 0, s>>>(R.rl, ctx->d_scalars);
    TC_LAUNCH_CHECK(ctx);
    tc_d2h(ctx, ctx->h_scalars, ctx->d_scalars, sizeof(u64));
    TC_HIP(ctx, hipStreamSynchronize(s));
    *primary = ctx->h_scalars[SA_SLOT_PRIMARY];
    st.sigma = R.cfg.sigma_text + 1;
    st.radix_launches = 0;
    st.ms_radix = 0;
    for (int i = 0; i < ctx->pev_used; i++) {
        float ms = 0;
        if (hipEventElapsedTime(&ms, ctx->pev[2 * i], ctx->pev[2 * i + 1]) == hipSuccess) {
            st.ms_radix += ms;
            st.radix_launches++;
        }
    }
}
```

### text-compression_amd/csrc/tc_sa_plan.hpp

```cpp
#pragma once
#include <math.h>
#include <stdint.h>

struct SaKnobs {
    int trace = env_int("TC_SA_TRACE", 0);
    int fields = env_int("TC_SA_FIELDS", 0);
    int bin_min_log2 = env_int("TC_SA_BIN_MIN_LOG2", 25);
    int kb_onehist = env_int("TC_KB_ONEHIST", 1);
    int keygen_fused = env_int("TC_KEYGEN_FUSED", 1);
    int xcd_group = env_int("TC_XCD_GROUP", 1);
    int finish = env_int("TC_SA_FINISH", 1);
    int dense = env_int("TC_SA_DENSE", 0);
    int global_passes = env_int("TC_SA_GLOBAL_PASSES", 0);
    int sample = env_int("TC_SA_SAMPLE", 1);
    int msd = env_int("TC_SA_MSD", 1);
    int msd_big = env_int("TC_SA_MSD_BIG", 0);
    int msd_max_dups = env_int("TC_SA_MSD_MAX_DUPS", 8);
    int keyround = env_int("TC_SA_KEYROUND", 1);
    int msd_keyonly = env_int("TC_SA_MSD_KEYONLY", 1);
    int keygen_hash = env_int("TC_KEYGEN_HASH", 1);
    int msd_grid = env_int("TC_MSD_GRID", 0);
    int msd_joint = env_int("TC_SA_MSD_JOINT", 1);
    int msd_split = env_int("TC_MSD_SPLIT", 1);
    int msd_finish_lut = env_int("TC_MSD_FINISH_LUT", 1);
    int msd_finish_ko = env_int("TC_MSD_FINISH_KO", 1);
    int tier2 = env_int("TC_SA_TIER2", 1);
    int tiny = env_int("TC_SA_TINY", 1);
    int seg = env_int("TC_SA_SEG", 1);
    int seg_min = env_int("TC_SA_SEG_MIN", 1 << 16);
    int deep = env_int("TC_SA_DEEP", 1);
    int accel_min = env_int("TC_SA_ACCEL_MIN", 1 << 20);
    int kdir_search = env_int("TC_SA_KDIR_SEARCH", 0);
    int h_start = env_int("TC_SA_H_START", 0);
    int chain = env_int("TC_SA_CHAIN", 1);
};

struct Round0In {
    double entropy;
    uint32_t w, s, P;
    uint64_t N;
    bool msd_carved;
    bool want_sa;
    uint32_t sample_dups;
    int msd_levels;
    uint32_t cap_small, cap_big;
    uint32_t samp_n, tied_max;
};
struct Round0Plan {
    int G, topbits;
    bool msd_cand;
    uint32_t P;
    bool try_msd, msd_big, keyonly, keyround;
};

static inline void sa_round0_depth(const Round0In &in, const SaKnobs &K, Round0Plan &pl) {
    const int keybits = (int)(in.P * in.w);
    double e8 = in.w == 8 ? in.entropy * in.s : in.entropy * 8.0 / in.w;
    int G = e8 > 1e-9 ? (int)ceil((log2((double)in.N) - 4.0) / e8) : 64;
    if (G < (keybits - 32 + 7) / 8) G = (keybits - 32 + 7) / 8;
    if (G < 1) G = 1;
    if (K.global_passes > 0) G = K.global_passes;
    pl.msd_cand = in.w == 8 && in.msd_carved && K.fields == 0 && K.global_passes == 0;
    if (pl.msd_cand && G < in.msd_levels) G = in.msd_levels;
    pl.G = G;
    pl.topbits = 8 * G < keybits ? 8 * G : keybits;
    pl.P = in.P;
}

static inline void sa_round0_plan(const Round0In &in, const SaKnobs &K, Round0Plan &pl) {
    if (K.fields == 0) {
        uint32_t pf = (uint32_t)((pl.topbits + 32) / (int)in.w);
        if (pf > 56 / in.w) pf = 56 / in.w;
        if (pf > pl.P) pl.P = pf;
    }
    const double field_bits = in.entropy * in.s < 8.0 ? in.entropy * in.s : 8.0;
    const double lvl_bits = field_bits * in.msd_levels;
    const double msd_bucket = (double)in.N / exp2(lvl_bits);
    pl.msd_big = msd_bucket > (double)in.cap_small / 3.0 || K.msd_big != 0;
    const bool msd_fits = msd_bucket <= (double)in.cap_big * 0.8;
    const double iid_dups = (double)in.samp_n * in.samp_n / 2.0 / exp2(field_bits * (pl.topbits / 8));
    const bool msd_iid = (double)in.sample_dups <= (double)K.msd_max_dups + 3.0 * iid_dups;
    pl.keyround = K.keyround != 0;
    pl.try_msd = pl.msd_cand && pl.P == 7 &&
                 (K.msd == 2 || (msd_fits && (msd_iid || (pl.msd_big && pl.keyround && K.msd == 3))));
    const double tied_est = (double)in.N * (double)in.N / exp2(in.entropy * (double)(pl.P * in.s));
    pl.keyonly = !in.want_sa && (tied_est < (double)in.tied_max / 4.0 || K.msd_keyonly == 2) && K.msd_keyonly != 0;
}

struct ChainPolicy {
    int mode;
    int keymode = 0;
    uint64_t prev_mm = 0;
    int chain_fail = 0, chain_wait = 0;
    uint64_t chain_m0 = 0;

    explicit ChainPolicy(int mode_) : mode(mode_) {}

    bool start(bool seg_round, uint32_t hh, uint64_t h, uint64_t N, uint64_t m) {
        if (keymode != 0 || !seg_round || hh < 4 || h >= N || mode == 0) return false;
        if (mode != 2 && !(m >= (1u << 20) && prev_mm > 0 && (prev_mm - m) * 256 < prev_mm && chain_wait == 0 && chain_fail < 3))
            return false;
        keymode = 1;
        chain_m0 = m;
        return true;
    }
    bool finish(uint64_t m, uint64_t m_left) {
        if (keymode == 1) {
            keymode = 2;
            return false;
        }
        if (keymode == 2) {
            if ((chain_m0 - m_left) * 8 < chain_m0) chain_wait = 1 << ++chain_fail;
        } else if (chain_wait > 0) chain_wait--;
        prev_mm = keymode == 2 ? 0 : m;
        keymode = 0;
        return true;
    }
};
```

### text-compression_amd/csrc/textcomp.hip

```cpp
#include "tc_common.hpp"
#include "tc_encode_host.hpp"
#include "tc_decode_host.hpp"
#include "tc_ws_host.hpp"
#include "tc_fm_host.hpp"
#include "tc_lcp_host.hpp"
#include "tc_container_host.hpp"
#include "tc_hostio_host.hpp"
#include "tc_generate.hpp"
#include "tc_dbg_host.hpp"
#include "tc_comm.hpp"
#include "textcomp_debug.h"

#define TC_API_BEGIN(ctx)                                  \
    if (!(ctx)) return TC_ERR_ARG;                         \
    try {                                                  \
        if (hipSetDevice((ctx)->device) != hipSuccess) {   \
            (ctx)->err = "hipSetDevice failed";            \
            return TC_ERR_HIP;                             \
        }
#define TC_API_END(ctx)                                    \
        return TC_OK;                                      \
    } catch (const TcFail &f) {                            \
        (void)hipGetLastError();                           \
        return f.code;                                     \
// ... 287 lines not shown
        if (!container || bytes < TC_CONTAINER_HEADER) TC_FAIL(ctx, TC_ERR_MALFORMED, "container shorter than its header");
        const ContainerHeader h = container_header_parse(ctx, container, bytes, HDR_MAGIC);
        if (n) *n = h.n;
        if (nruns) *nruns = h.nruns;
        return TC_OK;
    } catch (const TcFail &f) {
        return f.code;
    }
}

int tc_container_coding(tc_ctx *ctx, const uint8_t *container, uint64_t bytes, int *coding) {
    if (!ctx) return TC_ERR_ARG;
    try {
        if (!coding) TC_FAIL(ctx, TC_ERR_ARG, "bad argument");
        if (!container || bytes < TC_CONTAINER_HEADER) TC_FAIL(ctx, TC_ERR_MALFORMED, "container shorter than its header");
        const ContainerHeader h = container_header_parse(ctx, container, bytes, HDR_MAGIC);
        if (h.format == HF_FORMAT) *coding = TC_CODING_HUFFMAN;
        else if (h.sigma <= TC_MAX_SIGMA && h.format == (u32)pack_format(h.sigma)) *coding = TC_CODING_PACKED;
        else TC_FAIL(ctx, TC_ERR_MALFORMED, "container header names no known body format");
        return TC_OK;
    } catch (const TcFail &f) {
        return f.code;
    }
}

int tc_encode_container(tc_ctx *ctx, const uint8_t *text, uint64_t n, uint8_t *out, uint64_t *bytes) {
    TC_API_BEGIN(ctx)
    encode_container_entry(ctx, text, n, out, bytes);
    TC_API_END(ctx)
}

int tc_decode_container(tc_ctx *ctx, const uint8_t *container, uint64_t bytes, uint8_t *text, uint64_t *n_out) {
    TC_API_BEGIN(ctx)
    decode_container_entry(ctx, container, bytes, text, n_out);
    TC_API_END(ctx)
}

uint64_t tc_stream_bound(uint64_t n, uint64_t block_bytes) {
    if (block_bytes == 0) block_bytes = TC_STREAM_BLOCK_DEFAULT;
    if (block_bytes > TC_MAX_N) block_bytes = TC_MAX_N;
    const u64 nb = stream_blocks(n, block_bytes);
    const u64 last = n - (nb - 1) * block_bytes;
    return (nb - 1) * container_bound_any(block_bytes) + container_bound_any(last);
}

int tc_encode_stream(tc_ctx *ctx, const uint8_t *text, uint64_t n, uint64_t block_bytes, uint8_t *out,
                     uint64_t *bytes) {
    TC_API_BEGIN(ctx)
    encode_stream_entry(ctx, text, n, block_bytes, out, bytes);
    TC_API_END(ctx)
}

int tc_stream_info(tc_ctx *ctx, const uint8_t *stream, uint64_t bytes, uint64_t *n_total, uint64_t *nblocks) {
    if (!ctx) return TC_ERR_ARG;
    try {
        const StreamIndex ix = stream_index(ctx, stream, bytes);
        if (n_total) *n_total = ix.n_total;
        if (nblocks) *nblocks = ix.off.size();
        return TC_OK;
    } catch (const TcFail &f) {
        return f.code;
    }
}

int tc_decode_stream(tc_ctx *ctx, const uint8_t *stream, uint64_t bytes, uint8_t *text, uint64_t *n_out) {
    TC_API_BEGIN(ctx)
    decode_stream_entry(ctx, stream, bytes, text, n_out);
    TC_API_END(ctx)
}

int tc_fm_build(tc_ctx *ctx, const uint8_t *text, uint64_t n, tc_fm **out) {
    TC_API_BEGIN(ctx)
    fm_build_entry(ctx, text, nullptr, n, 1, 0, 0, out);
    TC_API_END(ctx)
}

int tc_fm_build_dev(tc_ctx *ctx, const uint8_t *d_text, uint64_t n, tc_fm **out) {
    TC_API_BEGIN(ctx)
    fm_build_entry(ctx, nullptr, d_text, n, 1, 0, 0, out);
    TC_API_END(ctx)
}

int tc_fm_build_sampled(tc_ctx *ctx, const uint8_t *text, uint64_t n, uint32_t sa_rate, tc_fm **out) {
    TC_API_BEGIN(ctx)
    fm_build_entry(ctx, text, nullptr, n, sa_rate, 0, 1, out);
    TC_API_END(ctx)
}

int tc_fm_build_sampled_dev(tc_ctx *ctx, const uint8_t *d_text, uint64_t n, uint32_t sa_rate, tc_fm **out) {
    TC_API_BEGIN(ctx)
    fm_build_entry(ctx, nullptr, d_text, n, sa_rate, 0, 1, out);
    TC_API_END(ctx)
}

int tc_fm_build_self(tc_ctx *ctx, const uint8_t *text, uint64_t n, uint32_t sa_rate, uint32_t text_rate, tc_fm **out) {
    TC_API_BEGIN(ctx)
    fm_build_entry(ctx, text, nullptr, n, sa_rate, text_rate, 2, out);
    TC_API_END(ctx)
}

int tc_fm_build_self_dev(tc_ctx *ctx, const uint8_t *d_text, uint64_t n, uint32_t sa_rate, uint32_t text_rate, tc_fm **out) {
    TC_API_BEGIN(ctx)
    fm_build_entry(ctx, nullptr, d_text, n, sa_rate, text_rate, 2, out);
    TC_API_END(ctx)
}

uint32_t tc_fm_sa_rate(const tc_fm *fm) { return fm ? fm->sa_rate : 0; }
uint32_t tc_fm_text_rate(const tc_fm *fm) { return fm ? fm->text_rate : 0; }
uint64_t tc_fm_device_bytes(const tc_fm *fm, int part) { return fm_device_bytes(fm, part); }
void tc_fm_free(tc_fm *fm) { fm_release(fm); }

uint64_t tc_fm_export_bound(const tc_fm *fm, int with_locate) { return fm_export_bound(fm, with_locate); }

int tc_fm_export_dev(tc_ctx *ctx, const tc_fm *fm, int with_locate, uint8_t *d_out, uint64_t *bytes) {
    TC_API_BEGIN(ctx)
    fm_export_device(ctx, fm, with_locate, d_out, bytes);
    TC_API_END(ctx)
}

int tc_fm_import_dev(tc_ctx *ctx, const uint8_t *d_in, uint64_t bytes, tc_fm **out) {
    TC_API_BEGIN(ctx)
    fm_import_device(ctx, d_in, bytes, out);
    TC_API_END(ctx)
}

int tc_fm_count_dev(tc_ctx *ctx, const tc_fm *fm, const uint8_t *d_pats, const uint64_t *d_offs,
                    uint64_t npat, int64_t *d_out) {
    TC_API_BEGIN(ctx)
    fm_count_entry(ctx, fm, d_pats, d_offs, npat, true, 0, d_out, true);
    TC_API_END(ctx)
}

int tc_fm_count(tc_ctx *ctx, const tc_fm *fm, const uint8_t *pats, const uint64_t *offs,
                uint64_t npat, int64_t *out) {
    TC_API_BEGIN(ctx)
    fm_count_entry(ctx, fm, pats, offs, npat, true, 0, out, false);
    TC_API_END(ctx)
}

int tc_fm_locate(tc_ctx *ctx, const tc_fm *fm, const uint8_t *pats, const uint64_t *offs,
                 uint64_t npat, uint64_t *hit_offs, uint64_t *hits, uint64_t *nhits) {
    TC_API_BEGIN(ctx)
    fm_locate_entry(ctx, fm, pats, offs, npat, true, 0, hit_offs, hits, nullptr, nhits, false);
    TC_API_END(ctx)
}

int tc_fm_locate_dev(tc_ctx *ctx, const tc_fm *fm, const uint8_t *d_pats, const uint64_t *d_offs,
                     uint64_t npat, uint64_t *d_hit_offs, uint64_t *d_hits, uint64_t *nhits) {
    TC_API_BEGIN(ctx)
    fm_locate_entry(ctx, fm, d_pats, d_offs, npat, true, 0, d_hit_offs, d_hits, nullptr, nhits, true);
    TC_API_END(ctx)
}

int tc_fm_count_mm_dev(tc_ctx *ctx, const tc_fm *fm, const uint8_t *d_pats, const uint64_t *d_offs, uint64_t npat, uint32_t k,
                       int64_t *d_out) {
    TC_API_BEGIN(ctx)
    fm_count_entry(ctx, fm, d_pats, d_offs, npat, false, k, d_out, true);
    TC_API_END(ctx)
}

int tc_fm_count_mm(tc_ctx *ctx, const tc_fm *fm, const uint8_t *pats, const uint64_t *offs, uint64_t npat, uint32_t k,
                   int64_t *out) {
    TC_API_BEGIN(ctx)
    fm_count_entry(ctx, fm, pats, offs, npat, false, k, out, false);
    TC_API_END(ctx)
}

int tc_fm_locate_mm(tc_ctx *ctx, const tc_fm *fm, const uint8_t *pats, const uint64_t *offs, uint64_t npat, uint32_t k,
                    uint64_t *hit_offs, uint64_t *hits, uint8_t *hit_mm, uint64_t *nhits) {
    TC_API_BEGIN(ctx)
    fm_locate_entry(ctx, fm, pats, offs, npat, false, k, hit_offs, hits, hit_mm, nhits, false);
    TC_API_END(ctx)
}

int tc_fm_locate_mm_dev(tc_ctx *ctx, const tc_fm *fm, const uint8_t *d_pats, const uint64_t *d_offs, uint64_t npat, uint32_t k,
                        uint64_t *d_hit_offs, uint64_t *d_hits, uint8_t *d_hit_mm, uint64_t *nhits) {
    TC_API_BEGIN(ctx)
    fm_locate_entry(ctx, fm, d_pats, d_offs, npat, false, k, d_hit_offs, d_hits, d_hit_mm, nhits, true);
    TC_API_END(ctx)
}

int tc_fm_extract_dev(tc_ctx *ctx, const tc_fm *fm, const uint64_t *d_starts, const uint64_t *d_lens, uint64_t nq,
                      uint64_t *d_out_offs, uint8_t *d_out, uint64_t *nbytes) {
    TC_API_BEGIN(ctx)
    fm_extract_entry(ctx, fm, d_starts, d_lens, nq, d_out_offs, d_out, nbytes, true);
    TC_API_END(ctx)
}

int tc_fm_extract(tc_ctx *ctx, const tc_fm *fm, const uint64_t *starts, const uint64_t *lens, uint64_t nq,
                  uint64_t *out_offs, uint8_t *out, uint64_t *nbytes) {
    TC_API_BEGIN(ctx)
    fm_extract_entry(ctx, fm, starts, lens, nq, out_offs, out, nbytes, false);
    TC_API_END(ctx)
}

int tc_fm_factorize(tc_ctx *ctx, const tc_fm *fm, const uint8_t *pats, const uint64_t *offs, uint64_t npat, uint64_t *fac_offs,
                    uint64_t *fac_pos, uint32_t *fac_len, uint64_t *nfac) {
    TC_API_BEGIN(ctx)
    fm_factor_entry(ctx, fm, pats, offs, npat, fac_offs, fac_pos, fac_len, nfac, false);
    TC_API_END(ctx)
}

int tc_fm_factorize_dev(tc_ctx *ctx, const tc_fm *fm, const uint8_t *d_pats, const uint64_t *d_offs, uint64_t npat,
                        uint64_t *d_fac_offs, uint64_t *d_fac_pos, uint32_t *d_fac_len, uint64_t *nfac) {
    TC_API_BEGIN(ctx)
    fm_factor_entry(ctx, fm, d_pats, d_offs, npat, d_fac_offs, d_fac_pos, d_fac_len, nfac, true);
    TC_API_END(ctx)
}

int tc_fm_unfactorize(tc_ctx *ctx, const tc_fm *fm, const uint64_t *fac_offs, const uint64_t *fac_pos, const uint32_t *fac_len,
                      uint64_t npat, uint64_t *out_offs, uint8_t *out, uint64_t *nbytes) {
    TC_API_BEGIN(ctx)
    fm_unfactor_entry(ctx, fm, fac_offs, fac_pos, fac_len, npat, out_offs, out, nbytes, false);
    TC_API_END(ctx)
}

int tc_fm_unfactorize_dev(tc_ctx *ctx, const tc_fm *fm, const uint64_t *d_fac_offs, const uint64_t *d_fac_pos,
                          const uint32_t *d_fac_len, uint64_t npat, uint64_t *d_out_offs, uint8_t *d_out, uint64_t *nbytes) {
    TC_API_BEGIN(ctx)
    fm_unfactor_entry(ctx, fm, d_fac_offs, d_fac_pos, d_fac_len, npat, d_out_offs, d_out, nbytes, true);
    TC_API_END(ctx)
}

int tc_fm_info(const tc_fm *fm, uint64_t *N, uint32_t *sigma, int16_t *c_sym, uint64_t *c_val,
               uint64_t *primary) {
    return fm_info(fm, N, sigma, c_sym, c_val, primary);
}

int tc_comm_unique_id(tc_ctx *ctx, uint8_t *id) {
    TC_API_BEGIN(ctx)
    comm_unique_id_entry(ctx, id);
    TC_API_END(ctx)
}

int tc_comm_create(tc_ctx *ctx, const uint8_t *id, int rank, int world, tc_comm **out) {
    TC_API_BEGIN(ctx)
    comm_create_entry(ctx, id, rank, world, out);
    TC_API_END(ctx)
}

void tc_comm_destroy(tc_comm *comm) { comm_destroy_entry(comm); }

int tc_comm_reserved_cus(const tc_comm *comm) { return comm ? comm->cus : 0; }

int tc_comm_wait(tc_comm *c) {
    if (!c) return TC_ERR_ARG;
    tc_ctx *ctx = c->ctx;
    TC_API_BEGIN(ctx)
    comm_wait_entry(ctx, c);
    TC_API_END(ctx)
}

int tc_comm_gather(tc_comm *c, int root, const uint8_t *d_container, uint64_t bytes, uint8_t *d_recv,
                   uint64_t slot_bytes, uint64_t *sizes) {
    if (!c) return TC_ERR_ARG;
    tc_ctx *ctx = c->ctx;
    TC_API_BEGIN(ctx)
    comm_gather_entry(ctx, c, root, d_container, bytes, d_recv, slot_bytes, sizes);
    TC_API_END(ctx)
}

int tc_comm_broadcast(tc_comm *c, int root, uint8_t *d_buf, uint64_t bytes) {
    if (!c) return TC_ERR_ARG;
    tc_ctx *ctx = c->ctx;
    TC_API_BEGIN(ctx)
    comm_broadcast_entry(ctx, c, root, d_buf, bytes);
    TC_API_END(ctx)
}

int tc_dbg_checksum64_dev(tc_ctx *ctx, const void *d_p, uint64_t bytes, uint64_t *out) {
    TC_API_BEGIN(ctx)
    dbg_checksum64_entry(ctx, d_p, bytes, out);
    TC_API_END(ctx)
}

int tc_dbg_stream_bench(tc_ctx *ctx, uint64_t bytes, int width, int mode, int iters, double *gbps) {
    TC_API_BEGIN(ctx)
    dbg_stream_bench_entry(ctx, bytes, width, mode, iters, gbps);
    TC_API_END(ctx)
}

int tc_dbg_scatter_bench(tc_ctx *ctx, uint64_t n, uint32_t bins, uint32_t xrun, int iters, double *ms_per_pass) {
    TC_API_BEGIN(ctx)
    dbg_scatter_bench_entry(ctx, n, bins, xrun, iters, ms_per_pass);
    TC_API_END(ctx)
}

int tc_dbg_lcp_set_short_cap(tc_ctx *ctx, uint32_t cap) {
    if (!ctx) return TC_ERR_ARG;
    if (cap != 0 && (cap < 16 || cap > 65536 || cap % 16 != 0)) {
        ctx->err = "the short cap is a multiple of 16 in 16 .. 65536, or 0";
        return TC_ERR_ARG;
    }
    ctx->lcp_cap = cap;
    return TC_OK;
}

int tc_dbg_msd_split_used(tc_ctx *ctx, uint32_t *used) {
    if (!ctx || !used) return TC_ERR_ARG;
    *used = ctx->msd_split_used ? 1u : 0u;
    return TC_OK;
}

int tc_dbg_dispatch_probe(tc_ctx *ctx, uint32_t grid, uint32_t lds_bytes, uint32_t spin_cycles, uint32_t *out6) {
    TC_API_BEGIN(ctx)
    dbg_dispatch_probe_entry(ctx, grid, lds_bytes, spin_cycles, out6);
    TC_API_END(ctx)
}

int tc_dbg_sort_bench(tc_ctx *ctx, uint64_t n, int key_bits, int iters, int check, double *ms_per_pass) {
    TC_API_BEGIN(ctx)
    dbg_sort_bench_entry(ctx, n, key_bits, iters, check, ms_per_pass);
    TC_API_END(ctx)
}

}
```

Baseline: 56260 MB/s.

## Walk aligned MSD levels via an LDS directory of nonempty parents

Adds a directory-driven tile walk for aligned MSD partition levels. Each workgroup compacts the nonempty parents (q, start, count) into an LDS directory with a ballot scan and generates tile descriptors from it, replacing the per-tile binary-search and linear tpre scans. It also prefetches the next segment's seg/ccnt row during the current tile so segment initialisation can read a shadow copy. The cost is extra LDS, refill barriers when the directory runs out, an atomic fill counter, and a forced plain load after a refill.

Result: faster. 57920 MB/s (median of 6 runs) (+3.0%).

```diff
diff --git a/include/textcomp_debug.h b/include/textcomp_debug.h
--- a/include/textcomp_debug.h
+++ b/include/textcomp_debug.h
@@ -11,6 +11,7 @@
 int tc_dbg_dispatch_probe(tc_ctx *ctx, uint32_t grid, uint32_t lds_bytes, uint32_t spin_cycles, uint32_t *out6);
 int tc_dbg_lcp_set_short_cap(tc_ctx *ctx, uint32_t cap);
 int tc_dbg_msd_split_used(tc_ctx *ctx, uint32_t *used);
+int tc_dbg_msd_dir(tc_ctx *ctx, uint32_t out[2]);
 #ifdef __cplusplus
 }
 #endif
diff --git a/text-compression_amd/csrc/tc_common.hpp b/text-compression_amd/csrc/tc_common.hpp
--- a/text-compression_amd/csrc/tc_common.hpp
+++ b/text-compression_amd/csrc/tc_common.hpp
@@ -41,6 +41,7 @@
     void *hostpipe = nullptr;
     u32 stats_ws_grown = 0;
     u32 lcp_cap = 0;
+    int msd_dir_used = 0;
     int msd_split_used = 0;
     int mtf_fastin_failed = 0;
     int live_comms = 0;
diff --git a/text-compression_amd/csrc/tc_msd.hpp b/text-compression_amd/csrc/tc_msd.hpp
--- a/text-compression_amd/csrc/tc_msd.hpp
+++ b/text-compression_amd/csrc/tc_msd.hpp
@@ -1,5 +1,6 @@
 #pragma once
 #include "tc_sa.hpp"
+#include "tc_msd_dir.hpp"
 
 #ifndef MSD_NT
 #define MSD_NT 1024
@@ -45,6 +46,7 @@
     const u32 *cnt_in;
     u32 *flags;
     u64 *dbg;
+    u32 *dirfills;
 };
 
 #ifdef __HIPCC__
@@ -54,10 +56,11 @@
     return (u32)((((u64)t + 1) * G - 1) / T);
 }
 
-__global__ void msd_root_kernel(u32 *pstart, u32 *pcnt, u32 N, u32 *maxchild) {
+__global__ void msd_root_kernel(u32 *pstart, u32 *pcnt, u32 N, u32 *maxchild, u32 *dirfills) {
     pstart[0] = 0;
     pcnt[0] = N;
     *maxchild = 0;
+    *dirfills = 0;
 }
 
 __device__ __forceinline__ u32 msd_block_of_parent(const MsdLevel &L, u32 q, u32 G) {
@@ -416,11 +419,12 @@
 }
 
 typedef u32 msd_u32x4 __attribute__((ext_vector_type(4)));
-template <bool KEYGEN, bool VALS, bool SPLIT>
+template <bool KEYGEN, bool VALS, bool SPLIT, bool DIR = false>
 __device__ __forceinline__ void msd_partition_body(const MsdLevel &L, const u64 *kin, const u32 *vin,
                                                    u64 *kout, u32 *vout, u32 *shi, u32 *slo, const u8 *text,
                                                    const RadixKeyGen &kg) {
     static_assert(!SPLIT || !VALS, "the split layout is the key-only levels'");
+    static_assert(!DIR || (!KEYGEN && !SPLIT), "the directory is the aligned level's");
     __shared__ __attribute__((aligned(16))) u64 s_keys[MSD_TILE];
     __shared__ __attribute__((aligned(16))) u32 s_vals[VALS ? MSD_TILE : 4];
     __shared__ __attribute__((aligned(16))) u64 c_keys[256 * MSD_GROUP];
@@ -439,14 +443,30 @@
     __shared__ __attribute__((aligned(16))) u8 s_kg8[KG_SPLIT ? MSD_TILE + 64 : 16];
     __shared__ u32 s_scan2[2];
     static_assert(MSD_GROUP == 8 || MSD_GROUP == 16 || MSD_GROUP == 32, "group = 8, 16 or 32 pairs");
-    static_assert(((size_t)MSD_TILE * (VALS ? 12 : 8) + 256 * MSD_GROUP * (VALS ? 12 : 8) + 8192 + (KG_SPLIT ? 2 * MSD_TILE + 256 : 0)) * (VALS ? 1 : MSD_BPC) <= 163840, "LDS budget");
+    constexpr u32 DIRCAP = DIR ? (VALS ? 128 : 1024) : 1;
+    __shared__ MsdDirEnt s_dir[DIRCAP];
+    __shared__ u32 s_rseg[DIR ? 256 : 1];
+    __shared__ u64 s_rmask[4];
+    __shared__ u32 s_nq[4], s_dst[6];
+    static_assert(((size_t)MSD_TILE * (VALS ? 12 : 8) + 256 * MSD_GROUP * (VALS ? 12 : 8) + 8192 + (KG_SPLIT ? 2 * MSD_TILE + 256 : 0) + (DIR ? DIRCAP * sizeof(MsdDirEnt) + 1024 + 128 : 0)) * (VALS ? 1 : MSD_BPC) <= 163840, "LDS budget");
     __shared__ MsdTileInfo s_info[4];
 
     const u32 tid = threadIdx.x, G = gridDim.x, b = msd_logical_wg(blockIdx.x, G);
     if (KEYGEN && tid < 256) s_klut[tid] = kg.lut[tid];
     if (tid < 256) { s_r[tid] = 0; s_ph[tid] = 0; s_cur[tid] = 0; }
     for (u32 i = tid; i < 256 * MSD_SUB; i += MSD_NT) s_cnt[i] = 0;
-    if (tid == 0) {
+    if (DIR) {
+        if (tid == 0 || tid == 64) {
+            const u32 w = tid >> 6;
+            u32 q = 0, tq = 0;
+            if (!(*L.flags & 8u)) {
+                q = msd_first_parent(L, b + w, G);
+                tq = L.tpre[q];
+            }
+            s_scan2[w] = tq; s_dst[1 + w] = q;
+        }
+        if (tid == 0) { s_dst[0] = 0; s_dst[3] = 0; s_dst[4] = MSD_DIR_NONE; }
+    } else if (tid == 0) {
         u32 ta = 0, tb = 0;
         if (!(L.aligned && (*L.flags & 8u))) msd_block_range(L, b, G, &ta, &tb);
         s_scan2[0] = ta; s_scan2[1] = tb;
@@ -455,7 +475,51 @@
     const u32 t0 = s_scan2[0], t1 = s_scan2[1];
     if (t0 >= t1) return;
     MsdCur cs = {};
-    if (tid == 0) {
+    u32 dir_e = 0, dir_k = 0;
+    auto dir_refill = [&]() {
+        u32 n = 0, qn = s_dst[1];
+        const u32 qe = s_dst[2];
+        while (n == 0 && qn < qe) {
+            const u32 q = qn + tid;
+            const bool in = q < qe;
+            const u32 pc = in ? L.pcnt[q] : 0u, ps = in ? L.pstart[q] : 0u;
+            const u64 m = __ballot(pc != 0);
+            if ((tid & 63) == 0) s_scan[tid >> 6] = (u32)__popcll(m);
+            __syncthreads();
+            u32 before = 0, tot = 0;
+#pragma unroll
+            for (u32 i = 0; i < MSD_NT / 64; i++) {
+                const u32 c = s_scan[i];
+                tot += c;
+                before += i < (tid >> 6) ? c : 0u;
+            }
+            const u32 rank = before + (u32)__popcll(m & ((1ull << (tid & 63)) - 1ull));
+            if (pc != 0 && rank < DIRCAP) { s_dir[rank].q = q; s_dir[rank].ps = ps; s_dir[rank].pc = pc; }
+            if (pc != 0 && rank == DIRCAP) s_dst[5] = q;
+            __syncthreads();
+            if (tot > DIRCAP) { n = DIRCAP; qn = s_dst[5]; }
+            else { n = tot; qn = qe - qn < (u32)MSD_NT ? qe : qn + MSD_NT; }
+            if (tid == 0) atomicAdd(L.dirfills, 1u);
+        }
+        __syncthreads();
+        if (tid == 0) { s_dst[0] = n; s_dst[1] = qn; s_dst[3] = 0; }
+        dir_e = 0; dir_k = 0;
+    };
+    auto dir_gen = [&](u32 x) {
+        MsdDirCur c = {dir_e, dir_k, s_dst[0], s_dst[1], s_dst[2], s_dst[3]};
+        MsdDirTile d;
+        u32 nq;
+        msd_dir_next(s_dir, c, MSD_TILE, &d, &nq);
+        dir_e = c.e; dir_k = c.k; s_dst[3] = c.pend;
+        MsdTileInfo *o = &s_info[(x - t0) & 3u];
+        o->base = d.base; o->valid = d.valid; o->q = d.q; o->last = d.last;
+        s_nq[(x - t0) & 3u] = nq;
+    };
+    if (DIR) {
+        dir_refill();
+        __syncthreads();
+        if (tid == 0) { dir_gen(t0); dir_gen(t0 + 1); dir_gen(t0 + 2); }
+    } else if (tid == 0) {
         msd_cur_init(L, cs, t0);
         msd_cur_info(L, cs, t0, t1, &s_info[0]);
         msd_cur_info(L, cs, t0 + 1, t1, &s_info[1]);
@@ -612,6 +676,13 @@
         const u64 m = __ballot(L.ccnt[(size_t)qq * 256 + tid] != 0);
         if ((tid & 63) == 0) s_lmask[tid >> 6] = m;
     };
+    auto seg_init_shadow = [&]() {
+        const u32 sb = s_rseg[tid];
+        s_cur[tid] = sb & ~(u32)(MSD_GROUP - 1);
+        s_ph[tid] = sb & (MSD_GROUP - 1);
+        s_r[tid] = sb & (MSD_GROUP - 1);
+        if ((tid & 63) == 0) s_lmask[tid >> 6] = s_rmask[tid >> 6];
+    };
     if (tid < 256) seg_init(s_info[0].q);
     auto detach = [&]() {
         if (KEYGEN) {
@@ -640,6 +711,8 @@
         if (tid < 3) gen_group(s_kr, s_kg8, MSD_NT + tid);
     }
 
+    u32 row_s = 0, row_c = 0;
+    bool seg_first = true, plain_next = false;
     for (u32 t = t0; t < t1; t++) {
         const u32 slot = (t - t0) & 3u;
         const MsdTileInfo ti = s_info[slot];
@@ -647,18 +720,31 @@
         u64 tq[8];
         tq[0] = __builtin_readcyclecounter();
 #endif
-        if (tid == 0) msd_cur_info(L, cs, t + 3, t1, &s_info[(slot + 3) & 3u]);
+        if (tid == 0) {
+            if (DIR) dir_gen(t + 3);
+            else msd_cur_info(L, cs, t + 3, t1, &s_info[(slot + 3) & 3u]);
+        }
         __syncthreads();
 #ifdef MSD_PROFILE
         const u64 t_b0 = __builtin_readcyclecounter();
 #endif
         const MsdTileInfo nx = s_info[(slot + 1) & 3u];
+        const u32 dpend = DIR ? s_dst[3] : 0u;
+        const u32 rq = DIR && seg_first ? s_nq[slot] : MSD_DIR_NONE;
+        const bool rows = DIR && rq != MSD_DIR_NONE && tid < 256;
         prefetch(ti, nx);
+        if (rows) {
+            const u32 *ps = L.seg + ((size_t)rq + b) * 256 + tid, *pc = L.ccnt + (size_t)rq * 256 + tid;
+            asm volatile("global_load_dword %0, %2, off\n\tglobal_load_dword %1, %3, off"
+                         : "+v"(row_s), "+v"(row_c)
+                         : "v"(ps), "v"(pc)
+                         : "memory");
+        }
         if (KEYGEN && kg_edge(ti)) {
             raw = kg_load_plain(ti);
             detach();
         }
-        if (!KEYGEN && t != t0 && !tile_safe(ti)) {
+        if (!KEYGEN && t != t0 && (!tile_safe(ti) || (DIR && plain_next))) {
             load_plain(ti);
             detach();
         }
@@ -821,6 +907,13 @@
 #ifdef MSD_PROFILE
         tq[5] = __builtin_readcyclecounter();
 #endif
+        if (rows) {
+            asm volatile("" : "+v"(row_s), "+v"(row_c) : : "memory");
+            s_rseg[tid] = row_s;
+            const u64 m = __ballot(row_c != 0);
+            if ((tid & 63) == 0) s_rmask[tid >> 6] = m;
+            if (tid == 0) s_dst[4] = rq;
+        }
         const bool kg_next = KG_SPLIT && kg_fast(nx);
         if (KEYGEN) {
             raw = nraw;
@@ -913,6 +1006,9 @@
             L.dbg[5] += tq[5] - tq[4]; L.dbg[6] += tq[6] - tq[5]; L.dbg[7] += tq[7] - tq[6]; L.dbg[1] += 1;
         }
 #endif
+#ifdef MSD_PROFILE
+        const u64 t_end0 = __builtin_readcyclecounter();
+#endif
         if (ti.last) {
             __syncthreads();
             for (u32 x = tid; x < 256 * MSD_GROUP; x += MSD_NT) {
@@ -930,8 +1026,30 @@
                 }
             }
             __syncthreads();
-            if (t + 1 < t1 && tid < 256) seg_init(s_info[(slot + 1) & 3u].q);
-        }
+            if (DIR) {
+                plain_next = false;
+                if (dpend) {
+                    dir_refill();
+                    __syncthreads();
+                    if (tid == 0)
+                        for (u32 x = t + 4 - dpend; x <= t + 3; x++) dir_gen(x);
+                    __syncthreads();
+                    plain_next = dpend == 3;
+                }
+                if (t + 1 < t1 && tid < 256) {
+                    const u32 q2 = s_info[(slot + 1) & 3u].q;
+                    if (s_dst[4] == q2) seg_init_shadow();
+                    else seg_init(q2);
+                }
+            } else if (t + 1 < t1 && tid < 256) seg_init(s_info[(slot + 1) & 3u].q);
+        }
+#ifdef MSD_PROFILE
+        if (b == 0 && tid == 0 && L.dbg && ti.last) {
+            L.dbg[12] += __builtin_readcyclecounter() - t_end0;
+            L.dbg[13] += 1;
+        }
+#endif
+        seg_first = ti.last != 0;
     }
 }
 template <bool KEYGEN, bool VALS = true>
@@ -944,6 +1062,11 @@
 __global__ __launch_bounds__(MSD_NT) void msd_partition_split_kernel(MsdLevel L, u32 *khi, u32 *klo, u64 *kout,
                                                                      const u8 *text, RadixKeyGen kg) {
     msd_partition_body<KEYGEN, false, true>(L, nullptr, nullptr, kout, nullptr, khi, klo, text, kg);
+}
+template <bool VALS>
+__global__ __launch_bounds__(MSD_NT) void msd_partition_dir_kernel(MsdLevel L, const u64 *kin, const u32 *vin, u64 *kout,
+                                                                   u32 *vout, RadixKeyGen kg) {
+    msd_partition_body<false, VALS, false, true>(L, kin, vin, kout, vout, nullptr, nullptr, nullptr, kg);
 }
 static inline size_t msd_split_npad(size_t N) { return (N + 31) & ~(size_t)31; }
 
diff --git a/text-compression_amd/csrc/tc_msd_dir.hpp b/text-compression_amd/csrc/tc_msd_dir.hpp
--- /dev/null
+++ b/text-compression_amd/csrc/tc_msd_dir.hpp
@@ -0,0 +1,92 @@
+#pragma once
+#include <stdint.h>
+
+#if defined(__HIPCC__)
+#define MSD_DIR_FN __host__ __device__ __forceinline__
+#else
+#define MSD_DIR_FN static inline
+#endif
+
+#define MSD_DIR_NONE 0xffffffffu
+#define MSD_DIR_PENDING 2u
+#define MSD_DIR_BATCH 1024u
+
+struct MsdDirEnt {
+    uint32_t q, ps, pc;
+};
+struct MsdDirTile {
+    uint32_t base, valid, q, last;
+};
+struct MsdDirCur {
+    uint32_t e, k;
+    uint32_t n;
+    uint32_t qnext, qend;
+    uint32_t pend;
+};
+
+MSD_DIR_FN void msd_dir_next(const MsdDirEnt *dir, MsdDirCur &c, const uint32_t tile, MsdDirTile *out, uint32_t *nq) {
+    *nq = MSD_DIR_NONE;
+    if (c.e >= c.n) {
+        out->base = 0; out->valid = 0; out->q = 0; out->last = 0;
+        if (c.qnext < c.qend) { out->last = MSD_DIR_PENDING; c.pend++; }
+        return;
+    }
+    const MsdDirEnt d = dir[c.e];
+    const uint32_t off = c.k * tile, left = d.pc - off;
+    out->base = d.ps + off;
+    out->valid = left < tile ? left : tile;
+    out->q = d.q;
+    out->last = left <= tile ? 1u : 0u;
+    if (c.e + 1 < c.n) *nq = dir[c.e + 1].q;
+    if (left <= tile) { c.e++; c.k = 0; } else c.k++;
+}
+
+static inline void msd_dir_fill_round(MsdDirEnt *dir, MsdDirCur &c, uint32_t cap, uint32_t batch, const uint32_t *pcnt,
+                                      const uint32_t *pstart) {
+    uint32_t q = c.qnext;
+    const uint32_t hi = c.qend - q < batch ? c.qend : q + batch;
+    for (; q < hi; q++) {
+        if (pcnt[q] == 0) continue;
+        if (c.n == cap) break;
+        dir[c.n].q = q; dir[c.n].ps = pstart[q]; dir[c.n].pc = pcnt[q];
+        c.n++;
+    }
+    c.qnext = q;
+}
+static inline uint32_t msd_dir_refill(MsdDirEnt *dir, MsdDirCur &c, uint32_t cap, uint32_t batch, const uint32_t *pcnt,
+                                      const uint32_t *pstart) {
+    uint32_t rounds = 0;
+    c.e = 0; c.k = 0; c.n = 0; c.pend = 0;
+    while (c.n == 0 && c.qnext < c.qend) {
+        msd_dir_fill_round(dir, c, cap, batch, pcnt, pstart);
+        rounds++;
+    }
+    return rounds;
+}
+static inline uint64_t msd_dir_walk(const uint32_t *pcnt, const uint32_t *pstart, uint32_t q0, uint32_t q1, MsdDirEnt *dir,
+                                    uint32_t cap, uint32_t batch, uint32_t tile, MsdDirTile *out, uint64_t max_out,
+                                    uint32_t *fills, int *bad) {
+    MsdDirCur c = {0, 0, 0, q0, q1, 0};
+    MsdDirTile ring[4];
+    uint32_t nq;
+    uint64_t t = 0;
+    *bad = 0;
+    *fills = msd_dir_refill(dir, c, cap, batch, pcnt, pstart);
+    for (int i = 0; i < 3; i++) msd_dir_next(dir, c, tile, &ring[i], &nq);
+    for (;; t++) {
+        const MsdDirTile ti = ring[t & 3];
+        if (ti.valid == 0) {
+            if (ti.last == MSD_DIR_PENDING) *bad = 1;
+            break;
+        }
+        msd_dir_next(dir, c, tile, &ring[(t + 3) & 3], &nq);
+        const uint32_t dpend = c.pend;
+        if (t < max_out) out[t] = ti;
+        if (dpend == 3 && !ti.last) *bad = 1;
+        if (ti.last && dpend) {
+            *fills += msd_dir_refill(dir, c, cap, batch, pcnt, pstart);
+            for (uint64_t x = t + 4 - dpend; x <= t + 3; x++) msd_dir_next(dir, c, tile, &ring[x & 3], &nq);
+        }
+    }
+    return t;
+}
diff --git a/text-compression_amd/csrc/tc_sa_host.hpp b/text-compression_amd/csrc/tc_sa_host.hpp
--- a/text-compression_amd/csrc/tc_sa_host.hpp
+++ b/text-compression_amd/csrc/tc_sa_host.hpp
@@ -115,6 +115,7 @@
     SA_SLOT_ERR = 62,
     SA_SLOT_MSD_PROF = 64,
     SA_SLOT_MSDK_PROF = 112,
+    SA_SLOT_MSD_DIR = 122,
 };
 static inline u32 sa_slot_lo(const tc_ctx *ctx, int slot) { return (u32)(ctx->h_scalars[slot] & 0xffffffffu); }
 static inline u32 sa_slot_hi(const tc_ctx *ctx, int slot) { return (u32)(ctx->h_scalars[slot] >> 32); }
@@ -388,11 +389,25 @@
         fprintf(stderr, "   level %d, S1 alone per tile: wave 0 %llu, last wave %llu cycles; slowest wave B0 -> before B1 %llu, B0 -> prefetch issued %llu\n", l + 1,
                 (unsigned long long)(h[16 * l + 8] / (h[16 * l + 1] | 1)), (unsigned long long)(h[16 * l + 9] / (h[16 * l + 1] | 1)),
                 (unsigned long long)(h[16 * l + 10] / (h[16 * l + 1] | 1)), (unsigned long long)(h[16 * l + 11] / (h[16 * l + 1] | 1)));
+    for (int l = 0; l < MSD_LEVELS; l++)
+        fprintf(stderr, "   level %d, ends of segments: %llu, %llu cycles each (flush, barriers, next ranges; outside the per-tile stamps)\n", l + 1,
+                (unsigned long long)h[16 * l + 13], (unsigned long long)(h[16 * l + 12] / (h[16 * l + 13] | 1)));
     tc_memset_async(ctx, ctx->d_scalars + SA_SLOT_MSD_PROF, 0, sizeof h);
 }
 #else
 static inline void msd_profile_dump(tc_ctx *) {}
 #endif
+
+static void sa_dbg_msd_dir(tc_ctx *ctx, uint32_t out[2]) {
+    u64 w = 0;
+    out[0] = ctx->msd_dir_used ? 1u : 0u;
+    out[1] = 0;
+    if (ctx->msd_dir_used) {
+        tc_d2h(ctx, &w, ctx->d_scalars + SA_SLOT_MSD_DIR, sizeof w);
+        TC_HIP(ctx, hipStreamSynchronize(ctx->stream));
+        out[1] = (u32)(w & 0xffffffffu);
+    }
+}
 
 static void sa_run_group(SaRun &R, bool init, GroupArgs ga) {
     tc_ctx *ctx = R.ctx;
@@ -579,7 +594,7 @@
         G = (u32)(ctx->num_cus - ctx->reserved_cus) * MSD_BPC;
     if (R.K.msd_grid > 0 && (u32)R.K.msd_grid < G) G = (u32)R.K.msd_grid;
     u32 *maxchild = sa_dev_slot(ctx, SA_SLOT_MAXCHILD);
-    msd_root_kernel<<<1, 1, 0, s>>>(b.msd_pstart[0], b.msd_pcnt[0], N, maxchild);
+    msd_root_kernel<<<1, 1, 0, s>>>(b.msd_pstart[0], b.msd_pcnt[0], N, maxchild, sa_dev_slot(ctx, SA_SLOT_MSD_DIR));
     TC_LAUNCH_CHECK(ctx);
     u64 *kbuf[2] = {b.k0, b.k1};
     u32 *vbuf[2] = {keyonly ? nullptr : b.v0, keyonly ? nullptr : R.sa};
@@ -606,6 +621,8 @@
     const bool split = keyonly && joint && R.K.msd_split != 0 && MSD_LEVELS == 3;
     u32 *khi = reinterpret_cast<u32 *>(b.k0), *klo = khi + msd_split_npad(N);
     ctx->msd_split_used = split ? 1 : 0;
+    const bool dir = joint && R.K.msd_dir != 0;
+    ctx->msd_dir_used = dir ? 1 : 0;
     if (joint) tc_memset_async(ctx, b.msd_joint, 0, (size_t)256 * 256 * 256 * sizeof(u32));
     u32 np = 1;
     for (int l = 0; l < MSD_LEVELS; l++, np *= 256) {
@@ -616,6 +633,7 @@
         ML.aligned = (joint && l == MSD_LEVELS - 1) ? 1 : 0;
         ML.ntot = N; ML.cnt_in = b.msd_joint; ML.flags = counters + 1;
         ML.dbg = ctx->d_scalars + SA_SLOT_MSD_PROF + 16 * l;
+        ML.dirfills = sa_dev_slot(ctx, SA_SLOT_MSD_DIR);
         const u64 *kin = l ? kbuf[(l - 1) & 1] : nullptr;
         const u32 *vin = l ? vbuf[(l - 1) & 1] : nullptr;
         msd_prep_kernel<<<1, 1024, 0, s>>>(ML.pcnt, np, b.msd_tpre[l]);
@@ -633,6 +651,9 @@
         if (split && l <= 1) {
             if (l == 0) msd_partition_split_kernel<true><<<G, MSD_NT, 0, s>>>(ML, khi, klo, nullptr, R.text, kg);
             else msd_partition_split_kernel<false><<<G, MSD_NT, 0, s>>>(ML, khi, klo, kbuf[1], R.text, kg);
+        } else if (dir && ML.aligned) {
+            if (keyonly) msd_partition_dir_kernel<false><<<G, MSD_NT, 0, s>>>(ML, kin, nullptr, kbuf[l & 1], nullptr, kg);
+            else msd_partition_dir_kernel<true><<<G, MSD_NT, 0, s>>>(ML, kin, vin, kbuf[l & 1], vbuf[l & 1], kg);
         } else if (keyonly) {
             if (l == 0) msd_partition_kernel<true, false><<<G, MSD_NT, 0, s>>>(ML, nullptr, nullptr, kbuf[0], nullptr, R.text, kg);
             else msd_partition_kernel<false, false><<<G, MSD_NT, 0, s>>>(ML, kin, nullptr, kbuf[l & 1], nullptr, R.text, kg);
@@ -883,6 +904,7 @@
     }
     if (res == R0_GIVE_WAY) {
         R.ctx->msd_split_used = 0;
+        R.ctx->msd_dir_used = 0;
         Round0Out o = sa_round0_lsd(R, pl);
         res = sa_round0_collect(R, o, pl.keyround, many_ties);
     }
@@ -1139,6 +1161,7 @@
                      ((uintptr_t)b.act[1][0] & 7) == 0;
     sa_trace_buffers(R);
     ctx->msd_split_used = 0;
+    ctx->msd_dir_used = 0;
     if (sa_alphabet(R, counts256_out, primary)) return;
 
     const u32 P_full = R.cfg.P;
diff --git a/text-compression_amd/csrc/tc_sa_plan.hpp b/text-compression_amd/csrc/tc_sa_plan.hpp
--- a/text-compression_amd/csrc/tc_sa_plan.hpp
+++ b/text-compression_amd/csrc/tc_sa_plan.hpp
@@ -22,6 +22,7 @@
     int msd_grid = env_int("TC_MSD_GRID", 0);
     int msd_joint = env_int("TC_SA_MSD_JOINT", 1);
     int msd_split = env_int("TC_MSD_SPLIT", 1);
+    int msd_dir = env_int("TC_MSD_DIR", 1);
     int msd_finish_lut = env_int("TC_MSD_FINISH_LUT", 1);
     int msd_finish_ko = env_int("TC_MSD_FINISH_KO", 1);
     int tier2 = env_int("TC_SA_TIER2", 1);
diff --git a/text-compression_amd/csrc/textcomp.hip b/text-compression_amd/csrc/textcomp.hip
--- a/text-compression_amd/csrc/textcomp.hip
+++ b/text-compression_amd/csrc/textcomp.hip
@@ -613,6 +613,13 @@
     return TC_OK;
 }
 
+int tc_dbg_msd_dir(tc_ctx *ctx, uint32_t out[2]) {
+    TC_API_BEGIN(ctx)
+    if (!out) TC_FAIL(ctx, TC_ERR_ARG, "out is null");
+    sa_dbg_msd_dir(ctx, out);
+    TC_API_END(ctx)
+}
+
 int tc_dbg_dispatch_probe(tc_ctx *ctx, uint32_t grid, uint32_t lds_bytes, uint32_t spin_cycles, uint32_t *out6) {
     TC_API_BEGIN(ctx)
     dbg_dispatch_probe_entry(ctx, grid, lds_bytes, spin_cycles, out6);
diff --git a/text-compression_amd/host/check/msd_dir_walk.cpp b/text-compression_amd/host/check/msd_dir_walk.cpp
--- /dev/null
+++ b/text-compression_amd/host/check/msd_dir_walk.cpp
@@ -0,0 +1,182 @@
+#include <cstdio>
+#include <cstdlib>
+#include <vector>
+
+#include "tc_msd_dir.hpp"
+
+#define EXPECT(cond)                                                              \
+    do {                                                                          \
+        if (!(cond)) {                                                            \
+            std::fprintf(stderr, "%s:%d: failed: %s\n", __FILE__, __LINE__, #cond); \
+            return 1;                                                             \
+        }                                                                         \
+    } while (0)
+
+static const uint32_t TILE = 8192;
+
+struct OldLevel {
+    const uint32_t *pstart, *pcnt, *tpre;
+    uint32_t nparents;
+};
+static uint32_t old_find_parent(const uint32_t *tpre, uint32_t nparents, uint32_t t) {
+    uint32_t lo = 0, hi = nparents;
+    while (hi - lo > 1) {
+        const uint32_t mid = (lo + hi) >> 1;
+        if (tpre[mid] <= t) lo = mid; else hi = mid;
+    }
+    return lo;
+}
+struct OldCur {
+    uint32_t q, tq0, tq1, ps, pc;
+};
+static void old_cur_init(const OldLevel &L, OldCur &c, uint32_t t) {
+    c.q = old_find_parent(L.tpre, L.nparents, t);
+    c.tq0 = L.tpre[c.q]; c.tq1 = L.tpre[c.q + 1]; c.ps = L.pstart[c.q]; c.pc = L.pcnt[c.q];
+}
+static void old_cur_info(const OldLevel &L, OldCur &c, uint32_t t, uint32_t t_end, MsdDirTile *out) {
+    if (t >= t_end) {
+        out->base = 0; out->valid = 0; out->q = 0; out->last = 0;
+        return;
+    }
+    if (t >= c.tq1) {
+        uint32_t q = c.q + 1;
+        while (L.tpre[q + 1] <= t) q++;
+        c.q = q; c.tq0 = L.tpre[q]; c.tq1 = L.tpre[q + 1]; c.ps = L.pstart[q]; c.pc = L.pcnt[q];
+    }
+    const uint32_t off = (t - c.tq0) * TILE;
+    out->base = c.ps + off;
+    out->valid = c.pc - off < TILE ? c.pc - off : TILE;
+    out->q = c.q;
+    out->last = (t + 1 >= t_end || t + 1 >= c.tq1) ? 1u : 0u;
+}
+
+struct Table {
+    std::vector<uint32_t> pcnt, pstart, tpre;
+    explicit Table(const std::vector<uint32_t> &c) : pcnt(c), pstart(c.size()), tpre(c.size() + 1) {
+        uint32_t pos = 0, t = 0;
+        for (size_t q = 0; q < c.size(); q++) {
+            pstart[q] = pos; tpre[q] = t;
+            pos += c[q]; t += (c[q] + TILE - 1) / TILE;
+        }
+        tpre[c.size()] = t;
+    }
+};
+static int compare(const Table &T, uint32_t q0, uint32_t q1, uint32_t cap, uint32_t batch, uint32_t *fills_out) {
+    const OldLevel L = {T.pstart.data(), T.pcnt.data(), T.tpre.data(), (uint32_t)T.pcnt.size()};
+    const uint32_t t0 = T.tpre[q0], t1 = T.tpre[q1];
+    std::vector<MsdDirTile> want;
+    if (t0 < t1) {
+        OldCur c;
+        old_cur_init(L, c, t0);
+        for (uint32_t t = t0; t < t1; t++) {
+            MsdDirTile d;
+            old_cur_info(L, c, t, t1, &d);
+            want.push_back(d);
+        }
+    }
+    std::vector<MsdDirEnt> dir(cap);
+    std::vector<MsdDirTile> got(want.size() + 4);
+    uint32_t fills = 0;
+    int bad = 0;
+    const uint64_t n = msd_dir_walk(T.pcnt.data(), T.pstart.data(), q0, q1, dir.data(), cap, batch, TILE, got.data(), got.size(),
+                                    &fills, &bad);
+    EXPECT(!bad);
+    EXPECT(n == want.size());
+    for (size_t i = 0; i < want.size(); i++) {
+        EXPECT(got[i].base == want[i].base);
+        EXPECT(got[i].valid == want[i].valid);
+        EXPECT(got[i].q == want[i].q);
+        EXPECT(got[i].last == want[i].last);
+    }
+    if (fills_out) *fills_out = fills;
+    return 0;
+}
+static int sweep(const std::vector<uint32_t> &cnt) {
+    const Table T(cnt);
+    const uint32_t np = (uint32_t)cnt.size();
+    const uint32_t caps[] = {1, 2, 3, 128, 1024}, batches[] = {1, 7, 1024};
+    for (uint32_t cap : caps)
+        for (uint32_t batch : batches) {
+            if (compare(T, 0, np, cap, batch, nullptr)) return 1;
+            if (np >= 4 && compare(T, np / 4, np - np / 4, cap, batch, nullptr)) return 1;
+            if (np >= 2 && compare(T, 1, np, cap, batch, nullptr)) return 1;
+        }
+    return 0;
+}
+
+static uint64_t rng_state = 0x9E3779B97F4A7C15ull;
+static uint32_t rnd() {
+    rng_state ^= rng_state << 13; rng_state ^= rng_state >> 7; rng_state ^= rng_state << 17;
+    return (uint32_t)(rng_state >> 32);
+}
+
+int main() {
+    uint32_t fills = 0;
+    EXPECT(!sweep({0}));
+    EXPECT(!sweep(std::vector<uint32_t>(3000, 0)));
+    {
+        const Table T(std::vector<uint32_t>(10, 5));
+        EXPECT(!compare(T, 4, 4, 8, 1024, &fills));
+        EXPECT(fills == 0);
+    }
+    for (uint32_t pc : {1u, 8191u, 8192u, 8193u, 3u * 8192u, 3u * 8192u + 1u, 100000u}) {
+        EXPECT(!sweep({pc}));
+        std::vector<uint32_t> a(2500, 0), b(2500, 0), c(2500, 0);
+        a[0] = pc; b[2499] = pc; c[1234] = pc;
+        EXPECT(!sweep(a)); EXPECT(!sweep(b)); EXPECT(!sweep(c));
+    }
+    {
+        std::vector<uint32_t> a(5000, 0);
+        a[0] = 20000; a[4999] = 7;
+        EXPECT(!sweep(a));
+        const Table T(a);
+        EXPECT(!compare(T, 0, 5000, 1024, 1024, &fills));
+        EXPECT(fills == 1 + 4);
+    }
+    EXPECT(!sweep({1, 8191, 8192, 8193, 3 * 8192, 0, 0, 1, 0, 8193}));
+    EXPECT(!sweep(std::vector<uint32_t>(300, 6)));
+    EXPECT(!sweep(std::vector<uint32_t>(300, 8192)));
+    {
+        std::vector<uint32_t> a;
+        for (int i = 0; i < 400; i++) { a.push_back(1 + i % 3); a.push_back(0); a.push_back(i % 5 == 0 ? 20000 : 0); }
+        EXPECT(!sweep(a));
+    }
+    {
+        const Table T(std::vector<uint32_t>(1000, 9000));
+        EXPECT(!compare(T, 0, 1000, 128, 1024, &fills));
+        EXPECT(fills == 8);
+        EXPECT(!compare(T, 0, 1000, 1, 1024, &fills));
+        EXPECT(fills == 1000);
+        EXPECT(!compare(T, 0, 1000, 1024, 1024, &fills));
+        EXPECT(fills == 1);
+    }
+    {
+        std::vector<uint32_t> a(4096, 0);
+        a[10] = 30000;
+        const Table T(a);
+        EXPECT(!compare(T, 0, 4096, 1024, 1024, &fills));
+        EXPECT(fills == 1 + 3);
+        EXPECT(!sweep(a));
+    }
+    for (int it = 0; it < 3000; it++) {
+        const uint32_t np = 1 + rnd() % 600, dens = 1 + rnd() % 8, big = rnd() % 4;
+        std::vector<uint32_t> a(np);
+        for (uint32_t q = 0; q < np; q++) {
+            if (rnd() % dens) { a[q] = 0; continue; }
+            switch (big ? rnd() % 4 : 0) {
+            case 0: a[q] = 1 + rnd() % 40; break;
+            case 1: a[q] = 8190 + rnd() % 5; break;
+            case 2: a[q] = 1 + rnd() % 70000; break;
+            default: a[q] = TILE * (1 + rnd() % 4); break;
+            }
+        }
+        const Table T(a);
+        const uint32_t x = rnd() % (np + 1), y = rnd() % (np + 1);
+        const uint32_t q0 = x < y ? x : y, q1 = x < y ? y : x;
+        const uint32_t cap = (it & 1) ? 1 + rnd() % 5 : (it & 2) ? 128 : 1024, batch = (it & 4) ? 1024 : 1 + rnd() % 64;
+        EXPECT(!compare(T, q0, q1, cap, batch, nullptr));
+        EXPECT(!compare(T, 0, np, cap, batch, nullptr));
+    }
+    std::printf("ok: directory walk of the aligned MSD level\n");
+    return 0;
+}
```
